# Genie-Kim/PintheMemory

Measured on AMD Instinct MI355X. Metric: train imgs/sec 768x768 bs=8 R50-DeepLabV3+ +mem, higher is better.
Workload: dtype f32

## Files before the change

### include/pinmem_hip.h

```cpp
#ifndef PINMEM_HIP_H
#define PINMEM_HIP_H
#include <stddef.h>
#include <stdint.h>

#ifdef __cplusplus
extern "C" {
#endif

typedef enum pm_status { PM_OK = 0, PM_EINVAL = -1, PM_EWORKSPACE = -2, PM_ELAUNCH = -3, PM_EUNSUPPORTED = -4 } pm_status;

typedef enum pm_dtype { PM_F32 = 0, PM_BF16 = 1 } pm_dtype;
#define PM_TF_ZERO_PAD64 1

typedef struct pm_tensor {
  void* ptr;
  int32_t n, h, w, c;
  int64_t pitch;
  int32_t dtype;
  int32_t flags;
} pm_tensor;

#define PM_ABI_VERSION 400

typedef struct pm_conv_params {
  int32_t struct_size;
  int32_t kh, kw, stride, pad, dil;
  int32_t prec;
  void* wino_v;
  int64_t wino_v_bytes;
  void* wxf;
  int64_t wxf_bytes;
  int32_t wxf_valid;
} pm_conv_params;

typedef struct pm_conv_epilogue {
  int64_t struct_size;
  const float* bias;
  const float* scale;
  const float* shift;
  const float* residual;
  int64_t residual_pitch;
  int32_t relu;
  float* bn_partials;
  int64_t bn_partials_bytes;
} pm_conv_epilogue;

const char* pm_last_error(void);
int pm_version(void);

size_t pm_conv_workspace(const pm_tensor* x, const pm_tensor* y, const pm_conv_params* p, int which );
size_t pm_conv_winograd_v_bytes(const pm_tensor* x, const pm_tensor* y, const pm_conv_params* p);
size_t pm_conv_wxf_bytes(const pm_tensor* x, const pm_tensor* y, const pm_conv_params* p);
size_t pm_conv_wxf_bytes_dgrad(const pm_tensor* dy, const pm_tensor* dx, const pm_conv_params* p);
typedef struct pm_wxf_job {
  const float* w;
  void* wxf;
  int64_t wxf_bytes;
  int32_t cout, kh, kw, cin;
  int32_t dgrad;
  int32_t reserved;
} pm_wxf_job;
int pm_conv_wxf_refresh_bf16(const pm_wxf_job* jobs, int n, void* stream);
int pm_conv_wxf_refresh_f32(const pm_wxf_job* jobs, int n, void* stream);
size_t pm_conv_bn_partials_bytes(const pm_tensor* x, const pm_tensor* y, const pm_conv_params* p);
int pm_conv_fwd(const pm_tensor* x, const float* w_krsc, const pm_tensor* y, const pm_conv_params* p,
                const pm_conv_epilogue* ep, void* ws, size_t ws_bytes, void* stream);
int pm_conv_bwd_data(const pm_tensor* dy, const float* w_krsc, const pm_tensor* dx, const pm_conv_params* p,
                     const pm_tensor* add, void* ws, size_t ws_bytes, void* stream);
int pm_conv_bwd_data_masked(const pm_tensor* dy, const float* w_krsc, const pm_tensor* dx, const pm_conv_params* p,
                            const pm_tensor* add, const uint8_t* add_mask, void* ws, size_t ws_bytes, void* stream);
int pm_conv_bwd_weight(const pm_tensor* x, const pm_tensor* dy, float* dw_krsc, float* dbias, const pm_conv_params* p,
                       void* ws, size_t ws_bytes, void* stream);

typedef struct pm_routing {
  int32_t struct_size;
  int32_t winograd;
  int32_t winograd_fused;
  int32_t conv16;
  int32_t conv16_wide;
  int32_t conv16_persistent;
  int32_t wgrad16;
  int32_t bf16_wgrad;
  int32_t split;
} pm_routing;
int pm_routing_get(pm_routing* out);
int pm_routing_set(const pm_routing* r);


int pm_set_winograd(int mode);
int pm_set_winograd_fused(int on);
int pm_set_conv16(int on);
int pm_set_bf16_wgrad(int on);
int pm_set_wgrad16(int on);
int pm_set_split(int on);

int pm_profile_enable(int on);
int pm_profile_dump(const char* csv_path);
int pm_profile_read(int mode, int bm, int bn, int km, int nst, double* total_ms, double* total_flops, int64_t* launches, int clear);
int pm_profile_read_prec(int mode, int bm, int bn, int km, int nst, int prec, double* total_ms, double* total_flops, int64_t* launches, int clear);
int pm_profile_read_bytes(int mode, int bm, int bn, int km, int nst, int prec, double* total_bytes);

size_t pm_bn_workspace(const pm_tensor* x);
int pm_bn_stats(const pm_tensor* x, float* moments, void* ws, size_t ws_bytes, void* stream);
int pm_bn_stats_finalize(const pm_tensor* x, float eps, float* mean, float* invstd, float* running_mean , float* running_var ,
                         float momentum, void* ws, size_t ws_bytes, void* stream);
int pm_bn_merge(const float* parts, int world, int c, float* moments, void* stream);
int pm_bn_merge_finalize(const float* parts, int world, int c, float eps, float* mean, float* invstd, float* running_mean ,
                         float* running_var , float momentum, void* stream);
int pm_bn_finalize(const float* moments, int c, float eps, float* mean, float* invstd,
                   float* running_mean, float* running_var, float momentum, void* stream);
int pm_bn_apply(const pm_tensor* x, const float* mean, const float* invstd, const float* gamma, const float* beta,
                const pm_tensor* residual , int relu, const pm_tensor* y, void* stream);
int pm_bn_apply_mask(const pm_tensor* x, const float* mean, const float* invstd, const float* gamma, const float* beta,
                     const pm_tensor* residual , int relu, const pm_tensor* y, uint8_t* mask , void* stream);
int pm_bn_bwd_reduce_mask(const pm_tensor* dy, const uint8_t* mask, const pm_tensor* x, const float* mean, const float* invstd,
                          const pm_tensor* gmask , float* sums, void* ws, size_t ws_bytes, void* stream);
int pm_bn_apply_mask_affine(const pm_tensor* x, const float* mean, const float* invstd, const float* gamma, const float* beta,
                            const pm_tensor* r, const float* r_mean, const float* r_invstd, const float* r_gamma, const float* r_beta,
                            int relu, const pm_tensor* y, uint8_t* mask , void* stream);
int pm_bn_bwd_apply_mask(const pm_tensor* dy, const uint8_t* mask, const pm_tensor* x, const float* mean, const float* invstd, const float* gamma,
                         const float* sums, float count, const pm_tensor* dx, void* stream);
int pm_bn_bwd_reduce(const pm_tensor* dy, const pm_tensor* y , const pm_tensor* x, const float* mean, const float* invstd,
                     const float* gamma , const float* beta , int relu, const pm_tensor* gmask ,
                     float* sums, void* ws, size_t ws_bytes, void* stream);
int pm_bn_bwd_apply(const pm_tensor* dy, const pm_tensor* y , const pm_tensor* x, const float* mean, const float* invstd,
                    const float* gamma, const float* beta , const float* sums, float count, int relu, const pm_tensor* dx,
                    const pm_tensor* dres , void* stream);
int pm_bn_partials_finalize(const float* partials, int64_t pixels, int c, float eps, float* mean, float* invstd, float* running_mean ,
                            float* running_var , float momentum, float* moments , void* stream);
int pm_bn_fold(const float* gamma, const float* beta, const float* running_mean, const float* running_var, const float* conv_bias,
               int c, float eps, float* scale, float* shift, void* stream);
int pm_bn_fold_multi(const void* table, const int* cs, const int* offs, int n, int max_c, int total, float eps, float* arena, void* stream);
int pm_relu_bwd(const pm_tensor* dy, const pm_tensor* y, const pm_tensor* dx, void* stream);
int pm_add(const pm_tensor* a, const pm_tensor* b, const pm_tensor* y, void* stream);
int pm_add_n(const pm_tensor* const* xs, int n, const pm_tensor* y, void* stream);
int pm_copy(const pm_tensor* src, const pm_tensor* dst, void* stream);
int pm_scale_shift_act(const pm_tensor* x, const float* scale, const float* shift, const pm_tensor* residual, int relu,
                       const pm_tensor* y, void* stream);

int pm_cast(const pm_tensor* x, const pm_tensor* y, void* stream);

int pm_maxpool3x3s2_fwd(const pm_tensor* x, const pm_tensor* y, uint8_t* argmax, void* stream);
int pm_maxpool3x3s2_bwd(const pm_tensor* dy, const uint8_t* argmax, const pm_tensor* dx, void* stream);
int pm_maxpool3x3s2_bn_relu_fwd(const pm_tensor* x, const float* mean, const float* invstd, const float* gamma, const float* beta, const pm_tensor* y,
                                uint8_t* argmax, void* stream);
int pm_bn_bwd_reduce_pool(const pm_tensor* dy_pooled, const uint8_t* argmax, const pm_tensor* x, const float* mean, const float* invstd, const float* gamma,
                          const float* beta, float* sums, void* ws, size_t ws_bytes, void* stream);
int pm_bn_bwd_apply_pool(const pm_tensor* dy_pooled, const uint8_t* argmax, const pm_tensor* x, const float* mean, const float* invstd, const float* gamma,
                         const float* beta, const float* sums, float count, const pm_tensor* dx, void* stream);
int pm_global_avgpool_fwd(const pm_tensor* x, const pm_tensor* y , void* stream);
int pm_global_avgpool_bwd(const pm_tensor* dy, const pm_tensor* dx, int accumulate, void* stream);

int pm_resize_bilinear_fwd(const pm_tensor* x, const pm_tensor* y, void* stream);
int pm_resize_bilinear_bwd(const pm_tensor* dy, const pm_tensor* dx, int accumulate, void* stream);
size_t pm_resize_bilinear_bwd_workspace(const pm_tensor* dy, const pm_tensor* dx);
int pm_resize_bilinear_bwd_separable(const pm_tensor* dy, const pm_tensor* dx, int accumulate, void* ws, size_t ws_bytes, void* stream);

int pm_resize_bilinear_hp_fwd(const pm_tensor* x, const pm_tensor* y, int flip_w, void* stream);
int pm_softmax_mean_update(const pm_tensor* logits, double* buffer, int counter, void* stream);
int pm_sliding_stitch(const pm_tensor* logits, const int32_t* tiles_xyxy, int ntiles, int H, int W, int flip_w, double* acc, int accumulate, void* stream);
int pm_argmax_f64(const double* buffer, int n, int h, int w, int c, int64_t* out_cls, double* out_prob , void* stream);

int pm_image_u8_to_nhwc4(const uint8_t* img_nhw3, int64_t pixels, const float* mean3, const float* std3, float* out_nhwc4, void* stream);
int pm_labels_u8_to_i64(const uint8_t* lab, int64_t n, int64_t* out, void* stream);

int pm_nchw_to_nhwc(const float* x_nchw, int c_src, const pm_tensor* y, void* stream);
int pm_nhwc_to_nchw(const pm_tensor* x, float* y_nchw, void* stream);
int pm_label_nearest(const int64_t* lab, int n, int H, int W, int64_t* out, int h, int w, void* stream);

size_t pm_upsample_ce_workspace(int n, int H, int W);
int pm_upsample_ce_fwd(const pm_tensor* logits, float inv_temp, const int64_t* labels, int H, int W, float* loss_out,
                       void* ws, size_t ws_bytes, void* stream);
size_t pm_upsample_ce_bwd_workspace(const pm_tensor* logits, int H, int W);
int pm_upsample_ce_bwd(const pm_tensor* logits, float inv_temp, const int64_t* labels, int H, int W, const float* loss_out,
                       const float* gscale, const pm_tensor* dlogits, void* ws, size_t ws_bytes, void* stream);

size_t pm_upsample_ce_field_bytes(const pm_tensor* logits, int H, int W);
int pm_upsample_ce_fwd_field(const pm_tensor* logits, float inv_temp, const int64_t* labels, int H, int W, float* loss_out, float* field,
                             void* ws , size_t ws_bytes, void* stream);
int pm_upsample_ce_bwd_field(const pm_tensor* logits , float inv_temp, int H, int W, const float* loss_out, const float* gscale,
                             const float* field, const pm_tensor* dlogits, void* stream);

size_t pm_upsample_wce_loss_floats(int n);
size_t pm_upsample_wce_workspace(int n, int H, int W);
int pm_upsample_wce_fwd(const pm_tensor* logits, float inv_temp, const int64_t* labels, int H, int W, const float* weights, int64_t weight_stride,
                        int per_image, float* loss_out, void* ws , size_t ws_bytes, void* stream);
int pm_upsample_wce_fwd_field(const pm_tensor* logits, float inv_temp, const int64_t* labels, int H, int W, const float* weights, int64_t weight_stride,
                              int per_image, float* loss_out, float* field, void* ws , size_t ws_bytes, void* stream);
int pm_upsample_wce_bwd_field(const pm_tensor* logits , float inv_temp, int H, int W, int per_image, const float* loss_out,
                              const float* gscale, const float* field, const pm_tensor* dlogits, void* stream);

size_t pm_label_class_weights_workspace(int n);
int pm_label_class_weights(const int64_t* labels, int n, int H, int W, int classes, double upper_bound, int norm, int per_batch, float* weights,
                           void* ws, size_t ws_bytes, void* stream);

size_t pm_upsample_eval_workspace(const pm_tensor* logits, int H, int W);
int pm_upsample_eval(const pm_tensor* logits, float inv_temp, const int64_t* labels, int H, int W, float* loss_out, int64_t* hist, int accumulate,
                     uint8_t* pred , void* ws, size_t ws_bytes, void* stream);

int pm_mem_read_fwd(const pm_tensor* x, const float* mem, int m, const float* gumbel_noise ,
                    const pm_tensor* qr, float* score, float* p_mem, void* stream);
size_t pm_mem_colsoftmax_workspace(int64_t rows, int m);
int pm_mem_colsoftmax(const float* score, const float* noise , int64_t rows, int m, float* p_query,
                      void* ws, size_t ws_bytes, void* stream);
size_t pm_mem_read_fwd_pq_workspace(int64_t rows, int m);
int pm_mem_read_fwd_pq(const pm_tensor* x, const float* mem, int m, const float* gumbel_noise, const float* gumbel_noise_q,
                       const pm_tensor* qr, float* score, float* p_mem, float* p_query, void* ws, size_t ws_bytes, void* stream);
size_t pm_mem_read_bwd_workspace(int64_t rows, int m, int d);
int pm_mem_read_bwd(const pm_tensor* x, const float* mem, int m, const float* p_mem, const pm_tensor* dqr,
                    const float* dscore_extra, const pm_tensor* dx, float* dmem ,
                    void* ws, size_t ws_bytes, void* stream);

size_t pm_mem_write_accum_workspace(const pm_tensor* z, int m);
int pm_mem_write_accum(const pm_tensor* z, const int64_t* labels, int H, int W, int m, int normalize,
                       float* nomden, void* ws, size_t ws_bytes, void* stream);
int pm_mem_write_accum_bwd(const pm_tensor* z, const int64_t* labels, int H, int W, int m, int normalize,
// ... 22 lines not shown
```

### pinthememory_amd/csrc/conv_igemm.hip

```cpp
#include <stdlib.h>
#include <algorithm>
#include <type_traits>
#include <vector>

#include "pm_common.h"

#include "conv_igemm_kernel.h"

namespace {

template <int ZL, bool O16 = false>
__global__ __launch_bounds__(256) void splitk_reduce_vec_kernel(const float* __restrict__ ws, int ksplit, long slab, int M, int Nn,
                                                                float* __restrict__ C, long c_pitch, const float* bias,
                                                                const float* scale, const float* shift, const float* residual,
                                                                long res_pitch, int relu, const unsigned char* res_mask) {
  constexpr int GP = 256 / ZL;
  __shared__ float4 red[ZL > 1 ? ZL : 1][GP];
  const int gl = threadIdx.x % GP, zl = threadIdx.x / GP;
  const long groups = (long)M * Nn / 4;
  for (long g0 = (long)blockIdx.x * GP; g0 < groups; g0 += (long)gridDim.x * GP) {
    const long grp = g0 + gl;
    float4 v = make_float4(0.f, 0.f, 0.f, 0.f);
    if (grp < groups)
#pragma unroll 8
// ... 160 lines not shown
  for (int i = 1; i < 16; ++i) s += sm[i][cl];
  out[c] = s;
}

template <bool O16>
__global__ __launch_bounds__(256) void dgrad_s2_interleave_kernel(const float* __restrict__ tmp, long class_stride, int valid_mask,
                                                                  float* __restrict__ dx, long xp, int N, int H, int W, int C, const float* __restrict__ add,
                                                                  long add_pitch) {
  const int c4n = C / 4;
  const long total = (long)N * H * W * c4n;
  for (long i = (long)blockIdx.x * 256 + threadIdx.x; i < total; i += (long)gridDim.x * 256) {
    const long pix = i / c4n;
    const int c = (int)(i - pix * c4n) * 4;
    const int ix = (int)(pix % W), iy = (int)((pix / W) % H), n = (int)(pix / ((long)W * H));
    const int cy = iy & 1, cx = ix & 1, cls = cy * 2 + cx;
    const int Hc = (H - cy + 1) >> 1, Wc = (W - cx + 1) >> 1;
    float4 v = make_float4(0.f, 0.f, 0.f, 0.f);
    if ((valid_mask >> cls) & 1) v = PM_LD4(tmp + cls * class_stride + ((long)(n * Hc + (iy >> 1)) * Wc + (ix >> 1)) * C + c);
    if constexpr (O16) {
      if (add) {
        const uint2 q = *reinterpret_cast<const uint2*>(reinterpret_cast<const pm_bf16*>(add) + pix * add_pitch + c);
        v.x += __uint_as_float(q.x << 16), v.y += __uint_as_float(q.x & 0xffff0000u), v.z += __uint_as_float(q.y << 16), v.w += __uint_as_float(q.y & 0xffff0000u);
      }
      *reinterpret_cast<uint2*>(reinterpret_cast<pm_bf16*>(dx) + pix * xp + c) = make_uint2(pm_pack_bf16(v.x, v.y), pm_pack_bf16(v.z, v.w));
    } else {
      if (add) {
        const float4 q = PM_LD4(add + pix * add_pitch + c);
        v.x += q.x, v.y += q.y, v.z += q.z, v.w += q.w;
      }
      PM_ST4(dx + pix * xp + c, v);
    }
  }
}

struct S2Class {
  int cy, cx, Hc, Wc, ky0, nky, ksy, kx0, nkx, ksx;
  long M;
};
inline void s2_taps(int c, int pad, int dil, int k, int& k0, int& nk, int& ks) {
  if (dil & 1) {
    k0 = (c + pad) & 1, ks = 2, nk = k0 < k ? (k - k0 + 1) / 2 : 0;
  } else {
    k0 = 0, ks = 1, nk = ((c + pad) & 1) ? 0 : k;
  }
}
inline S2Class s2_class(int cls, const pm_tensor* dx, const pm_conv_params* p) {
  S2Class c;
  c.cy = cls >> 1, c.cx = cls & 1;
  c.Hc = (dx->h - c.cy + 1) >> 1, c.Wc = (dx->w - c.cx + 1) >> 1;
  s2_taps(c.cy, p->pad, p->dil, p->kh, c.ky0, c.nky, c.ksy);
  s2_taps(c.cx, p->pad, p->dil, p->kw, c.kx0, c.nkx, c.ksx);
  c.M = (long)dx->n * c.Hc * c.Wc;
  return c;
}
int s2_interleave(const float* tmp, long class_stride, const bool* valid, const pm_tensor* dx, const pm_tensor* add, hipStream_t st, const char* what) {
  const int valid_mask = valid[0] | (valid[1] << 1) | (valid[2] << 2) | (valid[3] << 3);
  const long total = pm_pixels(dx) * (dx->c / 4);
  auto kernel = pm_is_bf16(dx) ? dgrad_s2_interleave_kernel<true> : dgrad_s2_interleave_kernel<false>;
  hipLaunchKernelGGL(kernel, dim3((int)std::min<long>((total + 255) / 256, 8192)), dim3(256), 0, st, tmp, class_stride, valid_mask, (float*)dx->ptr, (long)dx->pitch,
                     dx->n, dx->h, dx->w, dx->c, add ? (const float*)add->ptr : nullptr, add ? (long)add->pitch : 0l);
  return pm_check_launch(what);
}

struct Plan {
  int bm, bn;
  int tiles_m, tiles_n, ksplit, kper;
  size_t ws_bytes;
};

constexpr long SPLIT_MIN_K = 129;
inline bool split_k_ok(int mode, long K) { return mode == MODE_WGRAD || K >= SPLIT_MIN_K; }
Plan make_plan(int mode, long M, long Nn, long K, bool bf16 = false) {
  Plan best_p{};
  double best = 1e30;
  int bn = Nn > 64 ? 128 : ((Nn > 32 || bf16) ? 64 : 32);
  const bool big = bf16 || (pm_route.split && split_k_ok(mode, K));
  if (mode != MODE_WGRAD && !big && bn == 128) bn = 64;
  const long ksteps = (K + BK - 1) / BK;
  for (int bm = 128; bm >= 64; bm -= 64) {
    if (bm == 64 && bn < 64) continue;
    if (!big && mode != MODE_WGRAD && bn >= 64 && bm == 128) continue;
    if (bm == 64 && mode == MODE_WGRAD && M > 64) continue;
    if (bm == 128 && mode == MODE_WGRAD && M <= 64 && bn >= 64) continue;
    const int tiles_m = pm_cdiv(M, bm), tiles_n = pm_cdiv(Nn, bn);
    const long tiles = (long)tiles_m * tiles_n;
    const double unit_us = 2.0 * (bm / 128.0) * (bn / 128.0) * (bm == 64 ? 1.08 : 1.0);
    const long ks_max = std::max<long>(1, std::min<long>(ksteps / 4, 512));
    for (long ks = 1; ks <= ks_max; ++ks) {
      const long steps_per = (ksteps + ks - 1) / ks;
      if ((ksteps + steps_per - 1) / steps_per != ks) continue;
      const long blocks = tiles * ks;
      const long per_cu = (blocks + 255) / 256;
      double t = (double)per_cu * (double)(steps_per + 2) * unit_us * (per_cu == 1 ? 1.25 : 1.0);
      if (ks > 1) t += 2.0 * (double)ks * (double)M * (double)Nn * 4.0 / 3.0e6 + 6.0;
      if (t < best) {
        best = t;
        best_p.bm = bm, best_p.bn = bn, best_p.tiles_m = tiles_m, best_p.tiles_n = tiles_n;
        best_p.ksplit = (int)ks, best_p.kper = (int)(steps_per * BK);
      }
    }
  }
  best_p.ws_bytes = best_p.ksplit > 1 ? (size_t)best_p.ksplit * M * Nn * sizeof(float) : 0;
  return best_p;
}

template <int MODE, int BM, int BN, int WM, int WN, int KM, int PREC, int NST>
void launch_nst(const ConvK& k, dim3 grid, size_t smem, hipStream_t st) {
  const size_t ep_bytes = (size_t)4 * 32 * (BN / WN + 4) * sizeof(float);
  if constexpr (MODE == MODE_FWD && PREC != 1 && BN >= 64) {
    if (k.stats) {
      static pm_lds_optin optin;
      (void)optin(reinterpret_cast<const void*>(&conv_igemm_kernel<MODE, BM, BN, WM, WN, KM, PREC, NST, true>), 160 * 1024);
      hipLaunchKernelGGL((conv_igemm_kernel<MODE, BM, BN, WM, WN, KM, PREC, NST, true>), grid, dim3(256), std::max(smem / (NST == 1 ? 2 : 1), ep_bytes), st, k);
      return;
    }
  }
  static pm_lds_optin optin;
  (void)optin(reinterpret_cast<const void*>(&conv_igemm_kernel<MODE, BM, BN, WM, WN, KM, PREC, NST>), 160 * 1024);
  hipLaunchKernelGGL((conv_igemm_kernel<MODE, BM, BN, WM, WN, KM, PREC, NST>), grid, dim3(256), std::max(smem / (NST == 1 ? 2 : 1), ep_bytes), st, k);
}
constexpr int NST1_MAX_STEPS = 64;
constexpr bool has_nst1(int mode, int kmode, int bn) { return mode != MODE_WGRAD && kmode == K_FAST && bn >= 64; }
inline int lds_stages(int mode, int kmode, int bn, int kper) { return has_nst1(mode, kmode, bn) && kper <= NST1_MAX_STEPS * BK ? 1 : 2; }
template <int MODE, int BM, int BN, int WM, int WN, int KM, int PREC>
void launch_prec(const ConvK& k, dim3 grid, size_t smem, hipStream_t st) {
  if constexpr (has_nst1(MODE, KM, BN)) {
    if (lds_stages(MODE, KM, BN, k.kper) == 1) return launch_nst<MODE, BM, BN, WM, WN, KM, PREC, 1>(k, grid, smem, st);
  }
  launch_nst<MODE, BM, BN, WM, WN, KM, PREC, 2>(k, grid, smem, st);
}
template <int MODE, int BM, int BN, int WM, int WN, int KM>
void launch_inst(const ConvK& k, dim3 grid, size_t smem, hipStream_t st) {
  if constexpr (MODE == MODE_FWD && KM == K_FAST && BN >= 64) {
    if (k.prec == 2) return launch_prec<MODE, BM, BN, WM, WN, KM, 2>(k, grid, smem, st);
  }
  if constexpr (MODE == MODE_WGRAD && BN >= 64) {
    if (k.prec == 3) return launch_prec<MODE, BM, BN, WM, WN, KM, 3>(k, grid, smem, st);
    if (k.prec == 4) return launch_prec<MODE, BM, BN, WM, WN, KM, 4>(k, grid, smem, st);
  }
  if (k.prec != 0) launch_prec<MODE, BM, BN, WM, WN, KM, 1>(k, grid, smem, st);
  else launch_prec<MODE, BM, BN, WM, WN, KM, 0>(k, grid, smem, st);
}
template <int MODE, int BM, int BN, int WM, int WN>
void launch_one(const ConvK& k, dim3 grid, size_t smem, hipStream_t st) {
  if (k.kmode == K_SMALL) launch_inst<MODE, BM, BN, WM, WN, K_SMALL>(k, grid, smem, st);
  else if (k.kmode == K_FAST && MODE != MODE_WGRAD) launch_inst<MODE, BM, BN, WM, WN, (MODE != MODE_WGRAD ? K_FAST : K_MID)>(k, grid, smem, st);
  else launch_inst<MODE, BM, BN, WM, WN, K_MID>(k, grid, smem, st);
}

struct ProfRec {
  hipEvent_t a, b;
  int mode, bm, bn, km, prec, nst;
  int M, Nn, K, batch, ksplit;
  double flops;
  double bytes;
};
bool g_prof_on = false;
std::vector<ProfRec> g_prof;
struct ProfScope {
  ProfRec rec{};
  hipStream_t st;
  ProfScope(hipStream_t st_, int mode, int bm, int bn, int km, int prec, int nst, long M, long Nn, long K, int batch, int ksplit, double flops, double bytes = 0.0) : st(st_) {
    if (!g_prof_on) return;
    (void)hipEventCreate(&rec.a), (void)hipEventCreate(&rec.b);
    rec.mode = mode, rec.bm = bm, rec.bn = bn, rec.km = km, rec.prec = prec, rec.nst = nst, rec.M = (int)M, rec.Nn = (int)Nn, rec.K = (int)K, rec.batch = batch, rec.ksplit = ksplit;
    rec.flops = flops, rec.bytes = bytes;
    (void)hipEventRecord(rec.a, st);
  }
  void done() {
    if (!g_prof_on) return;
    (void)hipEventRecord(rec.b, st);
    g_prof.push_back(rec);
  }
};

inline bool split_takes(int mode, const Plan& p, const ConvK& k, int batch) {
  return pm_route.split != 0 && p.bn >= 64 && !k.io16 && (batch > 1 || split_k_ok(mode, k.K));
}

template <int MODE>
int launch(const ConvK& k0, const Plan& p, hipStream_t st, int batch = 1, double flops = -1.0) {
  ConvK k = k0;
  k.tiles_m = p.tiles_m;
  k.tiles_n = p.tiles_n;
  k.ksplit = p.ksplit;
  k.kper = p.kper;
  dim3 grid(p.tiles_m * p.tiles_n, batch, p.ksplit);
  if (batch != 1) k.stage_ep = 0;
  if (k.prec == 0 && split_takes(MODE, p, k, batch)) k.prec = 5;
  {
    const int units = batch * p.ksplit, rem = units & 7, ntile = p.tiles_m * p.tiles_n;
    k.batch_xcd = units >= 8 && (rem == 0 || ((rem == 1 || rem == 2 || rem == 4) && ntile % (8 / rem) == 0));
  }
  const int km = (MODE == MODE_WGRAD && k.kmode == K_FAST) ? K_MID : ((k.prec == 5 && MODE != MODE_WGRAD && k.kmode == K_FAST && k.kh * k.kw == 1 && k.stride == 1 && k.pad == 0 && !k.sub) ? K_PW : k.kmode);
  ProfScope prof(st, MODE, p.bm, p.bn, km, k.prec, lds_stages(MODE, k.kmode, p.bn, k.kper), k.M, k.Nn, k.K, batch, p.ksplit,
                 flops >= 0.0 ? flops : 2.0 * (double)k.M * (double)k.Nn * (double)k.K * batch,
                 (double)batch * ((double)k.a_bytes + (double)k.b_bytes + ((k.io16 && p.ksplit == 1) ? 2.0 : 4.0) * (double)k.M * (double)k.Nn * (double)p.ksplit));
  if constexpr (MODE != MODE_WGRAD) {
    if (pm_route.split && (k.prec == 0 || k.prec == 5) && !k.io16 && batch == 1 && p.ksplit == 1 && !k.stats && k.kh * k.kw == 1 && k.stride == 1 && k.pad == 0 && !k.sub) {
      pm_gemm_pw g;
      g.A = k.A, g.B = k.B, g.C = k.C, g.bias = k.bias, g.scale = k.scale, g.shift = k.shift, g.residual = k.residual, g.res_mask = k.res_mask;
      g.a_pitch = MODE == MODE_FWD ? k.x_pitch : k.y_pitch, g.c_pitch = k.c_pitch, g.res_pitch = k.res_pitch;
      g.b_sn = MODE == MODE_FWD ? k.K : 1, g.b_sk = MODE == MODE_FWD ? 1 : k.Nn;
      g.M = k.M, g.Nn = k.Nn, g.K = k.K, g.relu = k.relu;
      if (pm_pwstream_ok(&g)) {
        prof.rec.bm = 32, prof.rec.bn = 64, prof.rec.km = 4, prof.rec.prec = 5, prof.rec.nst = 0;
        const int e = pm_pwstream_launch(&g, st);
        prof.done();
        return e;
      }
    }
  }
  constexpr bool akc = MODE != MODE_WGRAD, bkc = MODE == MODE_FWD;
  if (k.prec == 5) {
    if (int e = pm_conv_split_launch(MODE, p.bm, p.bn, k, grid.x, grid.y, grid.z, pm_conv_split_stage_bytes(MODE, p.bm, p.bn), st)) return e;
    prof.rec.nst = 1;
    prof.done();
    return pm_check_launch("conv_split");
  }
  const bool tr = MODE == MODE_WGRAD && (k.prec == 3 || k.prec == 4) && p.bn >= 64;
  auto smem = [&](int bm, int bn) {
    if (tr) return (size_t)2 * ((k.prec == 4 ? 2 : 1) * BK * (bm + 32) + (k.prec == 4 ? 2 : 1) * BK * (bn + 32)) * 2;
    return (size_t)2 * ((akc ? bm * LDK : BK * bm) + (bkc ? bn * LDK : BK * bn)) * sizeof(float);
  };
  if (p.bm == 64) {
    if (p.bn == 128) launch_one<MODE, 64, 128, 2, 2>(k, grid, smem(64, 128), st);
    else launch_one<MODE, 64, 64, 2, 2>(k, grid, smem(64, 64), st);
  } else if (p.bn == 128) {
    launch_one<MODE, 128, 128, 2, 2>(k, grid, smem(128, 128), st);
  } else if (p.bn == 64) {
    launch_one<MODE, 128, 64, 2, 2>(k, grid, smem(128, 64), st);
  } else {
    launch_one<MODE, 128, 32, 4, 1>(k, grid, smem(128, 32), st);
  }
  prof.done();
  return pm_check_launch("conv_igemm");
}

int check_common(const pm_tensor* x, const pm_tensor* y, const pm_conv_params* p) {
  PM_REQUIRE(x && y && p && x->ptr && y->ptr, PM_EINVAL, "conv: null tensor");
  PM_REQUIRE(p->struct_size == (int32_t)sizeof(pm_conv_params), PM_EINVAL, "conv: pm_conv_params.struct_size %d != %zu -- caller built against another pinmem_hip.h (library ABI %d)",
             p->struct_size, sizeof(pm_conv_params), PM_ABI_VERSION);
  PM_REQUIRE(p->kh >= 1 && p->kw >= 1 && p->dil >= 1 && p->pad >= 0, PM_EINVAL, "conv: bad geometry");
  PM_REQUIRE(p->stride == 1 || p->stride == 2, PM_EUNSUPPORTED, "conv: stride %d unsupported (1 or 2)", p->stride);
  const int ho = (x->h + 2 * p->pad - p->dil * (p->kh - 1) - 1) / p->stride + 1;
  const int wo = (x->w + 2 * p->pad - p->dil * (p->kw - 1) - 1) / p->stride + 1;
  PM_REQUIRE(ho == y->h && wo == y->w && x->n == y->n, PM_EINVAL, "conv: output %dx%d does not match geometry (%dx%d)", y->h, y->w, ho, wo);
  PM_REQUIRE((x->dtype == PM_F32 || x->dtype == PM_BF16) && (y->dtype == PM_F32 || y->dtype == PM_BF16), PM_EUNSUPPORTED, "conv: dtype %d / %d", x->dtype, y->dtype);
  for (const pm_tensor* t : {x, y}) {
    if (pm_is_bf16(t)) PM_REQUIRE(pm_vec8(t), PM_EINVAL, "conv: bf16 tensors must be 16B aligned with pitch %% 8 == 0 and channels %% 8 == 0");
    else PM_REQUIRE(pm_vec_ok(t), PM_EINVAL, "conv: tensors must be 16B aligned with pitch %% 4 == 0");
  }
  PM_REQUIRE(x->c % 4 == 0, PM_EUNSUPPORTED, "conv: Cin %% 4 != 0 unsupported (pad the input channels)");
  PM_REQUIRE((y->c % 4 == 0) || (p->kh * p->kw == 1), PM_EUNSUPPORTED, "conv: Cout %% 4 != 0 only for 1x1");
  PM_REQUIRE(x->pitch >= x->c && y->pitch >= y->c, PM_EINVAL, "conv: pitch < channels");
  PM_REQUIRE(pm_pixels(x) * x->pitch < (1ll << 29) && pm_pixels(y) * y->pitch < (1ll << 29) && (int64_t)y->c * x->c * p->kh * p->kw < (1ll << 29),
             PM_EUNSUPPORTED, "conv: tensor too large for 32-bit byte offsets (2 GiB per tensor)");
  return PM_OK;
}

void fill_geom(ConvK& k, const pm_tensor* x, const pm_tensor* y, const pm_conv_params* p) {
  k.N = x->n, k.H = x->h, k.W = x->w, k.Cin = x->c, k.x_pitch = x->pitch;
  k.Ho = y->h, k.Wo = y->w, k.Cout = y->c, k.y_pitch = y->pitch;
  k.kh = p->kh, k.kw = p->kw, k.stride = p->stride, k.pad = p->pad, k.dil = p->dil;
  k.sshift = p->stride == 2 ? 1 : 0;
  k.prec = p->prec != 0 ? 1 : 0;
  k.T_eff = p->kh * p->kw, k.tk_w = p->kw, k.ky0 = k.kx0 = 0, k.ksy = k.ksx = 1;
  k.sub = k.sub_cy = k.sub_cx = 0, k.Hc = x->h, k.Wc = x->w;
  k.bias = k.scale = k.shift = k.residual = nullptr;
  k.res_pitch = 0, k.res_mask = nullptr, k.relu = 0, k.stats = nullptr, k.io16 = 0;
  k.stage_ep = 1;
  k.spl_prio = 1;
  k.n_group = 8;
  k.batch_xcd = 0;
  k.a_bs = k.b_bs = k.c_bs = 0;
}

struct WinoPlan {
  bool use;
  pm_wino_geom g;
  int Kp, P;
  size_t v_bytes, m_bytes, u_bytes;
  Plan pl;
};
inline bool wino_wgrad_pays(int cin, int cout) { return (long)cin * cout >= 256 * 256; }
WinoPlan wino_plan(const pm_tensor* xin, int cout, const pm_conv_params* p, bool wgrad = false) {
  WinoPlan wp{};
  if (wgrad && !wino_wgrad_pays(xin->c, cout)) return wp;
  if (pm_route.winograd == 0 || p->kh != 3 || p->kw != 3 || p->stride != 1 || p->pad != p->dil || p->prec != 0) return wp;
  const int cin = xin->c;
  if (cin < 128 || cout < 128 || (cout & 3) || (cin & 3)) return wp;
  int m = 0;
  double best_ratio = 0.6;
  for (int cand = pm_route.winograd; cand >= 2; cand -= 2) {
    const pm_wino_geom g = pm_wino_make_geom(xin->n, xin->h, xin->w, p->dil, cand);
    const double cover = (double)(cand * g.TY * p->dil) * (double)(cand * g.TX * p->dil) / ((double)xin->h * xin->w);
    const double ratio = cover * (cand + 2) * (cand + 2) / (9.0 * cand * cand);
    if (ratio <= best_ratio) best_ratio = ratio, m = cand, wp.g = g;
  }
  if (!m) return wp;
  wp.P = (m + 2) * (m + 2);
  wp.Kp = (cin + BK - 1) / BK * BK;
  if (wp.g.tiles * (long)std::max(wp.Kp, cout) * 4 >= (1ll << 31)) return wp;
  wp.v_bytes = pm_align_up((size_t)wp.P * wp.g.tiles * wp.Kp * sizeof(float), 256);
  wp.m_bytes = pm_align_up((size_t)wp.P * wp.g.tiles * cout * sizeof(float), 256);
  wp.u_bytes = pm_align_up((size_t)wp.P * cout * wp.Kp * sizeof(float), 256);
  wp.pl.bm = 128, wp.pl.bn = 128;
  if (pm_cdiv(cout, 128) * 128 > cout * 1.12 && pm_cdiv(cout, 64) * 64 < pm_cdiv(cout, 128) * 128) wp.pl.bn = 64;
  if (wp.g.tiles <= 4608 && !pm_route.split) wp.pl.bm = 64;
  wp.pl.tiles_m = pm_cdiv(wp.g.tiles, wp.pl.bm), wp.pl.tiles_n = pm_cdiv(cout, wp.pl.bn);
  wp.pl.ksplit = 1, wp.pl.kper = wp.Kp, wp.pl.ws_bytes = 0;
  wp.use = true;
  return wp;
}
inline size_t wino_ws(const WinoPlan& wp) { return wp.v_bytes + wp.m_bytes + wp.u_bytes; }

int wino_conv(const pm_tensor* xin, const float* w, int w_cout, int w_cin, bool dgrad, const pm_tensor* yout, const WinoPlan& wp,
              const pm_conv_epilogue& ep, void* ws, hipStream_t st, float* v_keep = nullptr, float* u_ext = nullptr, bool u_valid = false) {
  float* V = v_keep ? v_keep : (float*)ws;
  float* Mo = (float*)((char*)ws + wp.v_bytes);
  float* U = u_ext ? u_ext : (float*)((char*)ws + wp.v_bytes + wp.m_bytes);
  const int cout = yout->c;
  if (int e = pm_wino_input_xf((const float*)xin->ptr, xin->pitch, xin->c, wp.Kp, wp.g, V, st)) return e;
  if (!(u_ext && u_valid))
    if (int e = pm_wino_filter_xf(w, w_cout, w_cin, wp.Kp, dgrad, wp.g.m, U, st)) return e;
  const pm_tensor xv = {V, 1, 1, (int32_t)wp.g.tiles, wp.Kp, wp.Kp};
  const pm_tensor yv = {Mo, 1, 1, (int32_t)wp.g.tiles, cout, cout};
  const pm_conv_params p1 = {(int32_t)sizeof(pm_conv_params), 1, 1, 1, 0, 1, 0};
  ConvK k;
  fill_geom(k, &xv, &yv, &p1);
  k.A = V, k.B = U, k.C = Mo;
  k.M = (int)wp.g.tiles, k.Nn = cout, k.K = wp.Kp;
  k.a_bytes = (unsigned)(wp.g.tiles * wp.Kp * 4), k.b_bytes = (unsigned)((long)cout * wp.Kp * 4), k.kmode = K_FAST;
  k.c_pitch = cout, k.c_split = 0;
  k.a_bs = wp.g.tiles * wp.Kp, k.b_bs = (long)cout * wp.Kp, k.c_bs = wp.g.tiles * cout;
  if (pm_route.winograd_fused && wp.g.m == 4 && wp.Kp % 16 == 0) {
    ProfScope prof(st, 3, 32, 32, 0, 0, 1, wp.g.tiles, cout, wp.Kp, wp.P, 1, 2.0 * wp.P * (double)wp.g.tiles * cout * xin->c);
    const int e = pm_wino_fused_f4(V, U, cout, wp.Kp, wp.g, (float*)yout->ptr, yout->pitch, ep.bias, ep.scale, ep.shift, ep.residual, ep.residual_pitch, ep.relu, st);
    prof.done();
    return e;
  }
  if (int e = launch<MODE_FWD>(k, wp.pl, st, wp.P, 2.0 * wp.P * (double)wp.g.tiles * cout * xin->c)) return e;
  return pm_wino_output_xf(Mo, cout, wp.g, (float*)yout->ptr, yout->pitch, ep.bias, ep.scale, ep.shift, ep.residual, ep.residual_pitch, ep.relu, st);
}

struct WinoWgradPlan {
  Plan pl;
  size_t slab_bytes;
};
WinoWgradPlan wino_wgrad_plan(const WinoPlan& wp, int cout) {
  WinoWgradPlan q{};
  q.pl.bm = 128, q.pl.bn = 128;
  if (pm_cdiv(wp.Kp, 128) * 128 > wp.Kp * 1.12 && pm_cdiv(wp.Kp, 64) * 64 < pm_cdiv(wp.Kp, 128) * 128) q.pl.bn = 64;
  q.pl.tiles_m = pm_cdiv(cout, 128), q.pl.tiles_n = pm_cdiv(wp.Kp, q.pl.bn);
  const long ksteps = (wp.g.tiles + BK - 1) / BK;
  const long per_split = (long)q.pl.tiles_m * q.pl.tiles_n * wp.P;
  long ks = std::max<long>(1, std::min<long>((768 + per_split / 2) / per_split, ksteps / 8));
  const long steps_per = (ksteps + ks - 1) / ks;
  ks = (ksteps + steps_per - 1) / steps_per;
  q.pl.ksplit = (int)ks, q.pl.kper = (int)(steps_per * BK), q.pl.ws_bytes = 0;
  q.slab_bytes = pm_align_up((size_t)ks * wp.P * cout * wp.Kp * sizeof(float), 256);
  return q;
}
inline size_t wino_wgrad_ws(const WinoPlan& wp, const WinoWgradPlan& q) { return wp.v_bytes + wp.m_bytes + q.slab_bytes; }

int wino_wgrad(const pm_tensor* x, const pm_tensor* dy, float* dw, const WinoPlan& wp, const WinoWgradPlan& q, void* ws, hipStream_t st,
               float* v_kept = nullptr) {
  float* V = v_kept ? v_kept : (float*)ws;
  float* Z = (float*)((char*)ws + wp.v_bytes);
  float* slab = (float*)((char*)ws + wp.v_bytes + wp.m_bytes);
  const int cout = dy->c;
  if (!v_kept)
    if (int e = pm_wino_input_xf((const float*)x->ptr, x->pitch, x->c, wp.Kp, wp.g, V, st)) return e;
  if (int e = pm_wino_dy_xf((const float*)dy->ptr, dy->pitch, cout, wp.g, Z, st)) return e;
  const pm_tensor xv = {V, 1, 1, (int32_t)wp.g.tiles, wp.Kp, wp.Kp};
  const pm_tensor zv = {Z, 1, 1, (int32_t)wp.g.tiles, cout, cout};
  const pm_conv_params p1 = {(int32_t)sizeof(pm_conv_params), 1, 1, 1, 0, 1, 0};
  ConvK k;
  fill_geom(k, &xv, &zv, &p1);
  k.A = Z, k.B = V, k.C = slab;
  k.M = cout, k.Nn = wp.Kp, k.K = (int)wp.g.tiles;
  k.a_bytes = (unsigned)(wp.g.tiles * cout * 4), k.b_bytes = (unsigned)(wp.g.tiles * wp.Kp * 4), k.kmode = K_MID;
  k.c_pitch = wp.Kp, k.c_split = (long)wp.P * cout * wp.Kp;
  k.a_bs = wp.g.tiles * cout, k.b_bs = wp.g.tiles * wp.Kp, k.c_bs = (long)cout * wp.Kp;
  if (int e = launch<MODE_WGRAD>(k, q.pl, st, wp.P, 2.0 * wp.P * (double)wp.g.tiles * cout * x->c)) return e;
  return pm_wino_dw_xf(slab, q.pl.ksplit, cout, x->c, wp.Kp, wp.g.m, dw, st);
}

struct Bf16Plan {
  bool use;
  bool c16;
  pm_conv16 k16;
  bool inplace;
  int Cp;
  long M, Nn, Kf;
  size_t xb_bytes, wb_bytes;
  Plan pl;
};
Bf16Plan bf16_plan(const pm_tensor* xin, const pm_tensor* yout, const pm_conv_params* p) {
  Bf16Plan b{};
  if ((p->prec != 2 && !pm_is_bf16(xin) && !pm_is_bf16(yout)) || xin->c < 32) return b;
  b.Cp = (xin->c + 63) / 64 * 64;
  const long T = (long)p->kh * p->kw;
  b.M = pm_pixels(yout), b.Nn = yout->c, b.Kf = T * b.Cp / 2;
  b.inplace = pm_is_bf16(xin) && (xin->c % 64 == 0 || ((xin->flags & PM_TF_ZERO_PAD64) && xin->pitch >= b.Cp));
  const size_t xb = b.inplace ? (size_t)pm_pixels(xin) * xin->pitch * 2 : (size_t)pm_pixels(xin) * b.Cp * 2, wb = (size_t)yout->c * T * b.Cp * 2;
  if (xb >= (1ull << 31) || wb >= (1ull << 31)) return b;
  b.xb_bytes = b.inplace ? 0 : pm_align_up(xb, 256), b.wb_bytes = pm_align_up(wb, 256);
  b.pl = make_plan(MODE_FWD, b.M, b.Nn, b.Kf, true);
  if (b.pl.bn < 64) return b;
  b.use = true;
  constexpr long C16_MIN_M = 256;
  b.c16 = false;
  if (pm_route.conv16 && b.M >= C16_MIN_M && p->stride >= 1) {
    pm_conv16& k = b.k16;
    k = pm_conv16{};
    k.N = xin->n, k.H = xin->h, k.W = xin->w, k.Ho = yout->h, k.Wo = yout->w;
    k.a_pitch = b.inplace ? xin->pitch : b.Cp, k.Cp = b.Cp;
    k.kh = p->kh, k.kw = p->kw, k.stride = p->stride, k.pad = p->pad, k.dil = p->dil;
    k.M = (int)b.M, k.Nn = (int)b.Nn, k.K = (int)(T * b.Cp), k.ksteps = k.K / 64;
    k.c_pitch = yout->pitch, k.c_f32 = pm_is_bf16(yout) ? 0 : 1;
    pm_conv16_plan(&k);
    b.c16 = pm_route.conv16 == 2 || k.wide || k.bm == 64 || k.ksteps_per == 1 || (b.pl.bm == 64 && k.ksteps >= 16);
  }
  return b;
}
inline size_t bf16_ws(const Bf16Plan& b) {
  return b.xb_bytes + b.wb_bytes + std::max(pm_align_up(b.pl.ws_bytes, 256), b.c16 ? pm_conv16_slab_bytes(&b.k16) : (size_t)0);
}

int conv_bf16(const pm_tensor* xin, const float* w, int w_cout, int w_cin, bool rotate, const pm_tensor* yout, const pm_conv_params* pe, const Bf16Plan& b,
              const pm_conv_epilogue& e0, void* ws, hipStream_t st, char* wb_ext = nullptr, bool wb_valid = false) {
  char* xb = b.inplace ? (char*)xin->ptr : (char*)ws;
  char* wb = wb_ext ? wb_ext : (char*)ws + b.xb_bytes;
  float* slab = (float*)((char*)ws + b.xb_bytes + b.wb_bytes);
  const int T = pe->kh * pe->kw;
  if (!b.inplace) {
    if (pm_is_bf16(xin)) {
      if (int e = pm16_pad_rows((const pm_bf16*)xin->ptr, xin->pitch, xin->c, b.Cp, pm_pixels(xin), (pm_bf16*)xb, st)) return e;
    } else if (int e = pm_bf16_cast_rows((const float*)xin->ptr, xin->pitch, xin->c, b.Cp, pm_pixels(xin), xb, st)) return e;
  }
  if (!(wb_ext && wb_valid))
    if (int e = pm_bf16_cast_weights(w, w_cout, T, w_cin, b.Cp, rotate, wb, st)) return e;
  const long xpitch16 = b.inplace ? xin->pitch : b.Cp;
  if (b.c16) {
    const bool o16 = pm_is_bf16(yout);
    const bool ok = (!e0.bn_partials || o16) &&
                    (o16 ? ((yout->c | yout->pitch | (e0.residual ? e0.residual_pitch : 0)) & 7) == 0 && pm_aligned16(yout->ptr) && pm_aligned16(e0.residual)
                         : !(e0.scale || e0.residual || e0.relu));
    if (ok) {
      pm_conv16 k = b.k16;
      k.A = (const pm_bf16*)xb, k.B = (const pm_bf16*)wb;
      const double fl = 2.0 * (double)b.M * (double)b.Nn * (double)T * (double)xin->c * (g_prof_on ? pm_conv16_executed_fraction(&k) : 1.0);
      ProfScope prof(st, k.wide ? 5 : 4, k.bm, k.bn, pm_conv16w_persistent(&k), 5, k.wide ? 3 : (k.ksteps_per == 1 ? 1 : 2), k.M, k.Nn, k.K / 2, 1, k.ksplit, fl);
      int e;
      if (k.ksplit > 1) {
        k.C = slab;
        e = pm_conv16_launch(&k, st);
      } else {
        k.C = yout->ptr;
        k.bias = e0.bias, k.scale = e0.scale, k.shift = e0.shift, k.residual = e0.residual, k.res_pitch = e0.residual_pitch, k.relu = e0.relu;
        k.stats = o16 ? e0.bn_partials : nullptr;
        e = pm_conv16_launch(&k, st);
      }
      prof.done();
      if (e) return e;
      if (k.ksplit > 1)
        return splitk_reduce(slab, k.ksplit, b.M, b.Nn, (float*)yout->ptr, (long)yout->pitch, e0.bias, e0.scale, e0.shift, e0.residual, (long)e0.residual_pitch, e0.relu,
                             st, o16);
      return PM_OK;
    }
  }
  const pm_tensor xv = {xb, xin->n, xin->h, xin->w, b.Cp / 2, xpitch16 / 2};
  ConvK k;
  fill_geom(k, &xv, yout, pe);
  k.prec = 2;
  k.A = (const float*)xb, k.B = (const float*)wb;
  k.M = (int)b.M, k.Nn = (int)b.Nn, k.K = (int)b.Kf;
  k.a_bytes = (unsigned)((size_t)pm_pixels(xin) * xpitch16 * 2), k.b_bytes = (unsigned)((size_t)yout->c * T * b.Cp * 2), k.kmode = K_FAST;
  const double flops = 2.0 * (double)b.M * (double)b.Nn * (double)T * (double)xin->c;
  k.io16 = pm_is_bf16(yout) ? 1 : 0;
  if (b.pl.ksplit > 1) {
    k.C = slab, k.c_pitch = b.Nn, k.c_split = b.M * b.Nn;
    if (int e = launch<MODE_FWD>(k, b.pl, st, 1, flops)) return e;
// ... 68 lines not shown
  PmS2Classes cl = s.cl;
  for (int cls = 0; cls < 4; ++cls) cl.out[cls] = (char*)ws + s.wb_off[cls];
  if (int e = pm_bf16_cast_weights_s2(w, dy->c, p->kh, p->kw, dx->c, dy->c, &cl, st)) return e;
  float* slab = (float*)((char*)ws + s.slab_off);
  for (int cls = 0; cls < 4; ++cls) {
    if (!s.valid[cls]) continue;
    pm_conv16 k = s.k[cls];
    k.A = (const pm_bf16*)dy->ptr, k.B = (const pm_bf16*)((char*)ws + s.wb_off[cls]);
    void* out = (char*)ws + s.out_off[cls];
    ProfScope prof(st, 4, k.bm, k.bn, 0, 5, k.ksteps_per == 1 ? 1 : 2, k.M, k.Nn, k.K / 2, 1, k.ksplit, 2.0 * (double)k.M * (double)k.Nn * (double)k.K);
    k.C = k.ksplit > 1 ? (void*)slab : out;
    const int e = pm_conv16_launch(&k, st);
    prof.done();
    if (e) return e;
    if (k.ksplit > 1)
      if (int e2 = splitk_reduce(slab, k.ksplit, k.M, k.Nn, (float*)out, (long)dx->c, nullptr, nullptr, nullptr, nullptr, 0l, 0, st, false)) return e2;
  }
  return s2_interleave((const float*)((char*)ws + s.out_off[0]), s.class_stride, s.valid, dx, add, st, "dgrad_s2_interleave(native bf16 classes)");
}

struct Bf16WgradPlan {
  bool use;
  long P, M, Nn, Kf;
  size_t dyt_bytes, xt_bytes;
  Plan pl;
};
Bf16WgradPlan bf16_wgrad_plan(const pm_tensor* x, const pm_tensor* dy, const pm_conv_params* p) {
  Bf16WgradPlan b{};
  if (p->prec != 2 || !pm_route.bf16_wgrad || x->c < 32 || dy->c < 32) return b;
  b.P = pm_pixels(dy);
  if (b.P % 64) return b;
  const long T = (long)p->kh * p->kw;
  b.M = dy->c, b.Nn = T * x->c, b.Kf = b.P / 2;
  const size_t dyt = (size_t)dy->c * b.P * 2, xt = (size_t)T * x->c * b.P * 2;
  if (dyt >= (1ull << 31) || xt >= (1ull << 31)) return b;
  b.dyt_bytes = pm_align_up(dyt, 256), b.xt_bytes = pm_align_up(xt, 256);
  b.pl = make_plan(MODE_FWD, b.M, b.Nn, b.Kf, true);
  if (b.pl.bn < 64) return b;
  b.use = true;
  return b;
}
inline size_t bf16_wgrad_ws(const Bf16WgradPlan& b) { return b.dyt_bytes + b.xt_bytes + pm_align_up(b.pl.ws_bytes, 256); }

int conv_wgrad_bf16(const pm_tensor* x, const pm_tensor* dy, float* dw, const pm_conv_params* p, const Bf16WgradPlan& b, void* ws, hipStream_t st) {
  char* dyt = (char*)ws;
  char* xt = dyt + b.dyt_bytes;
  float* slab = (float*)(xt + b.xt_bytes);
  if (int e = pm_bf16_transpose_taps((const float*)dy->ptr, dy->pitch, dy->c, dy->n, dy->h, dy->w, dy->h, dy->w, 1, 1, 1, 0, 1, dyt, st)) return e;
  if (int e = pm_bf16_transpose_taps((const float*)x->ptr, x->pitch, x->c, x->n, x->h, x->w, dy->h, dy->w, p->kh, p->kw, p->stride, p->pad, p->dil, xt, st)) return e;
  const int Pf = (int)(b.P / 2);
  const pm_tensor av = {dyt, 1, 1, (int32_t)b.M, Pf, Pf};
  const pm_tensor cv = {dw, 1, 1, (int32_t)b.M, (int32_t)b.Nn, b.Nn};
  const pm_conv_params p1 = {(int32_t)sizeof(pm_conv_params), 1, 1, 1, 0, 1, 2};
  ConvK k;
  fill_geom(k, &av, &cv, &p1);
  k.prec = 2;
  k.A = (const float*)dyt, k.B = (const float*)xt;
  k.M = (int)b.M, k.Nn = (int)b.Nn, k.K = (int)b.Kf;
  k.a_bytes = (unsigned)((size_t)b.M * b.P * 2), k.b_bytes = (unsigned)((size_t)b.Nn * b.P * 2), k.kmode = K_FAST;
  const double flops = 2.0 * (double)b.M * (double)b.Nn * (double)b.P;
  if (b.pl.ksplit > 1) {
    k.C = slab, k.c_pitch = b.Nn, k.c_split = b.M * b.Nn;
    if (int e = launch<MODE_FWD>(k, b.pl, st, 1, flops)) return e;
    return splitk_reduce(slab, b.pl.ksplit, b.M, b.Nn, dw, b.Nn, nullptr, nullptr, nullptr, nullptr, 0l, 0, st);
  }
  k.C = dw, k.c_pitch = b.Nn, k.c_split = 0;
  return launch<MODE_FWD>(k, b.pl, st, 1, flops);
}

void gemm_dims(int which, const pm_tensor* x, const pm_tensor* y, const pm_conv_params* p, long& M, long& Nn, long& K) {
  const long T = (long)p->kh * p->kw;
  if (which == MODE_FWD) M = pm_pixels(y), Nn = y->c, K = T * x->c;
  else if (which == MODE_DGRAD) M = pm_pixels(x), Nn = x->c, K = T * y->c;
  else M = y->c, Nn = T * x->c, K = pm_pixels(y);
}

struct S2ParityPlan {
  S2Class c[4];
  Plan pl[4];
  bool valid[4];
  size_t tmp_bytes, slab_bytes;
};
S2ParityPlan s2_parity_plan(const pm_tensor* dy, const pm_tensor* dx, const pm_conv_params* p) {
  S2ParityPlan s{};
  for (int cls = 0; cls < 4; ++cls) {
    const S2Class& c = s.c[cls] = s2_class(cls, dx, p);
    s.tmp_bytes = std::max(s.tmp_bytes, (size_t)c.M * dx->c * sizeof(float));
    s.valid[cls] = c.M > 0 && c.nky * c.nkx > 0;
    if (!s.valid[cls]) continue;
    s.pl[cls] = make_plan(MODE_DGRAD, c.M, dx->c, (long)c.nky * c.nkx * dy->c, p->prec != 0);
    s.slab_bytes = std::max(s.slab_bytes, s.pl[cls].ws_bytes);
  }
  s.tmp_bytes = pm_align_up(s.tmp_bytes, 256);
  return s;
}

struct W16Plan {
  bool use;
  pm_wgrad16 k;
};
W16Plan wgrad16_plan(const pm_tensor* x, const pm_tensor* dy, const pm_conv_params* p, long M, long Nn, long K, int max_ksplit) {
  W16Plan q{};
  pm_wgrad16& w16 = q.k;
  w16.X = (const pm_bf16*)x->ptr, w16.DY = (const pm_bf16*)dy->ptr;
  w16.N = x->n, w16.H = x->h, w16.W = x->w, w16.Ho = dy->h, w16.Wo = dy->w;
  w16.x_pitch = x->pitch, w16.dy_pitch = dy->pitch, w16.Cin = x->c, w16.Cout = dy->c;
  w16.kh = p->kh, w16.kw = p->kw, w16.stride = p->stride, w16.pad = p->pad, w16.dil = p->dil;
  w16.M = (int)M, w16.Nn = (int)Nn, w16.P = (int)K, w16.kper = 64, w16.c_split = M * Nn;
  q.use = K < (1l << 30) && pm_wgrad16_plan(&w16);
  if (!q.use) return q;
  const long tiles = (long)w16.tiles_m * w16.tiles_n, steps = (K + 63) / 64;
  int best_ks = 1;
  double best = 1e30;
  for (int ks = 1; ks <= max_ksplit; ++ks) {
    const long per = (steps + ks - 1) / ks, kse = (steps + per - 1) / per;
    const long rounds = (tiles * kse + 255) / 256;
    const double cost = (double)rounds * (per + 6) + (kse > 1 ? (double)kse * M * Nn * 8.0 / 4e12 / 1.0e-6 : 0.0);
    if (cost < best) best = cost, best_ks = (int)kse;
  }
  const long per = (steps + best_ks - 1) / best_ks;
  w16.kper = (int)per * 64, w16.ksplit = (int)((steps + per - 1) / per);
  return q;
}

enum RouteKind {
  R_DIRECT,
  R_WINO,
  R_BF16,
  R_S2_NATIVE,
  R_S2_PARITY,
  R_WINO_WGRAD,
  R_BF16_WGRAD,
  R_DIRECT_WGRAD,
};
struct ConvRoute {
  RouteKind kind;
  Plan pl;
  WinoPlan wino;
  WinoWgradPlan wino_w;
  Bf16Plan b16;
  pm_conv_params pe;
  S2Native s2n;
  S2ParityPlan s2p;
  Bf16WgradPlan b16w;
  W16Plan w16;
  bool native16;
  size_t ws_bytes;
  size_t class_off, slab_off;
  size_t bias_off;
  size_t x32_off, dy32_off;
  size_t v_keep_bytes;
  size_t wxf_bytes;
  size_t bn_bytes;
};

ConvRoute route_conv(int which, const pm_tensor* x, const pm_tensor* y, const pm_conv_params* p) {
  ConvRoute r{};
  long M, Nn, K;
  gemm_dims(which, x, y, p, M, Nn, K);
  if (which == MODE_FWD) {
    if ((r.wino = wino_plan(x, y->c, p)).use) {
      r.kind = R_WINO, r.ws_bytes = wino_ws(r.wino), r.wxf_bytes = r.wino.u_bytes;
      r.v_keep_bytes = wino_wgrad_pays(x->c, y->c) ? r.wino.v_bytes : 0;
    } else if (p->prec == 2 && (r.b16 = bf16_plan(x, y, p)).use) {
      r.kind = R_BF16, r.pe = *p, r.ws_bytes = bf16_ws(r.b16), r.wxf_bytes = r.b16.wb_bytes;
    } else {
      r.kind = R_DIRECT, r.pl = make_plan(MODE_FWD, M, Nn, K, p->prec != 0), r.ws_bytes = pm_align_up(r.pl.ws_bytes, 256);
    }
    bool bn;
    if (pm_is_bf16(y)) bn = pm_vec8(y) && r.kind == R_BF16 && (r.b16.c16 ? (r.b16.k16.ksplit == 1 && !r.b16.k16.wide) : r.b16.pl.ksplit == 1);
    else if (pm_is_bf16(x) || (y->c & 3) || (y->pitch & 3) || !pm_aligned16(y->ptr)) bn = false;
    else bn = r.kind == R_BF16 ? r.b16.pl.ksplit == 1 : (r.kind == R_DIRECT && p->prec == 0 && r.pl.ksplit == 1 && r.pl.bn >= 64);
    r.bn_bytes = bn ? pm_align_up((size_t)pm_cdiv(pm_pixels(y), 32) * y->c * 2 * sizeof(float), 256) : 0;
  } else if (which == MODE_DGRAD) {
    if (p->stride == 2) {
      if ((r.s2n = s2_native_plan(y, x, p)).ok) {
        r.kind = R_S2_NATIVE, r.ws_bytes = r.s2n.total;
      } else {
        r.kind = R_S2_PARITY, r.s2p = s2_parity_plan(y, x, p);
        r.class_off = 0, r.slab_off = 4 * r.s2p.tmp_bytes;
        r.dy32_off = pm_align_up(r.slab_off + r.s2p.slab_bytes + 256, 256);
        r.ws_bytes = r.dy32_off + upcast_bytes(y);
      }
    } else if (dgrad_bf16_ok(p) && (r.pe = dgrad_as_fwd(p), r.b16 = bf16_plan(y, x, &r.pe)).use) {
      r.kind = R_BF16, r.ws_bytes = bf16_ws(r.b16), r.wxf_bytes = r.b16.wb_bytes;
    } else if ((r.wino = wino_plan(y, x->c, p)).use) {
      r.kind = R_WINO, r.ws_bytes = wino_ws(r.wino);
    } else {
      r.kind = R_DIRECT, r.pl = make_plan(MODE_DGRAD, M, Nn, K, p->prec != 0), r.ws_bytes = pm_align_up(r.pl.ws_bytes, 256);
    }
  } else {
    const bool tier = pm_is_bf16(x) || pm_is_bf16(y);
    r.native16 = pm_is_bf16(x) && pm_is_bf16(y) && y->c >= 32;
    size_t own;
    if (!tier && (r.b16w = bf16_wgrad_plan(x, y, p)).use) {
      r.kind = R_BF16_WGRAD, own = bf16_wgrad_ws(r.b16w);
    } else if (!tier && (r.wino = wino_plan(x, y->c, p, true)).use) {
      r.kind = R_WINO_WGRAD, r.wino_w = wino_wgrad_plan(r.wino, y->c), own = wino_wgrad_ws(r.wino, r.wino_w);
    } else {
      r.kind = R_DIRECT_WGRAD, r.pl = make_plan(MODE_WGRAD, M, Nn, K, p->prec != 0), own = r.pl.ws_bytes;
      if (r.native16) {
        r.pl.kper = (r.pl.kper + 63) / 64 * 64;
        r.pl.ksplit = (int)((K + r.pl.kper - 1) / r.pl.kper);
        r.w16 = wgrad16_plan(x, y, p, M, Nn, K, r.pl.ksplit);
      }
    }
    r.bias_off = pm_align_up(own, 256);
    r.ws_bytes = r.bias_off + pm_align_up((size_t)pm_cdiv(pm_pixels(y), colsum_rows(pm_pixels(y), y->c)) * y->c * sizeof(float), 256) + upcast_bytes(x) + upcast_bytes(y);
    r.x32_off = r.dy32_off = r.ws_bytes;
    if (!r.native16) r.x32_off -= upcast_bytes(x);
    r.dy32_off = r.x32_off - upcast_bytes(y);
  }
  return r;
}

int dgrad_s2_parity(const pm_tensor* dy0, const float* w, const pm_tensor* dx, const pm_conv_params* p, const pm_tensor* add, const ConvRoute& r, void* ws, hipStream_t st) {
  pm_tensor dy32;
  if (int e = upcast(dy0, (char*)ws + r.dy32_off, &dy32, st)) return e;
  const pm_tensor* dy = &dy32;
  float* tmp = (float*)((char*)ws + r.class_off);
  float* slab = (float*)((char*)ws + r.slab_off);
  for (int cls = 0; cls < 4; ++cls) {
    if (!r.s2p.valid[cls]) continue;
    const S2Class& c = r.s2p.c[cls];
    const Plan& pl = r.s2p.pl[cls];
    ConvK k;
    fill_geom(k, dx, dy, p);
    k.A = (const float*)dy->ptr, k.B = w;
    k.M = (int)c.M, k.Nn = dx->c, k.K = c.nky * c.nkx * dy->c;
    k.a_bytes = (unsigned)(pm_pixels(dy) * dy->pitch * 4), k.b_bytes = (unsigned)((long)dy->c * p->kh * p->kw * dx->c * 4);
    k.kmode = dy->c >= BK ? K_MID : K_SMALL;
    k.T_eff = c.nky * c.nkx, k.tk_w = c.nkx, k.ky0 = c.ky0, k.kx0 = c.kx0, k.ksy = c.ksy, k.ksx = c.ksx;
    k.sub = 1, k.sub_cy = c.cy, k.sub_cx = c.cx, k.Hc = c.Hc, k.Wc = c.Wc;
    float* out = (float*)((char*)tmp + cls * r.s2p.tmp_bytes);
    if (pl.ksplit > 1) {
      k.C = slab, k.c_pitch = dx->c, k.c_split = c.M * dx->c;
      if (int e = launch<MODE_DGRAD>(k, pl, st)) return e;
      if (int e = splitk_reduce(slab, pl.ksplit, c.M, dx->c, out, (long)dx->c, nullptr, nullptr, nullptr, nullptr, 0l, 0, st)) return e;
    } else {
      k.C = out, k.c_pitch = dx->c, k.c_split = 0;
      if (int e = launch<MODE_DGRAD>(k, pl, st)) return e;
    }
  }
  return s2_interleave(tmp, (long)(r.s2p.tmp_bytes / sizeof(float)), r.s2p.valid, dx, add, st, "dgrad_s2_interleave");
}

template <int MODE>
int conv_direct(const pm_tensor* x, const pm_tensor* y, const float* w, const pm_conv_params* p, const Plan& pl, const pm_conv_epilogue& e, void* ws, hipStream_t st,
                const unsigned char* res_mask = nullptr) {
  const pm_tensor *xin = MODE == MODE_FWD ? x : y, *out = MODE == MODE_FWD ? y : x;
  long M, Nn, K;
  gemm_dims(MODE, x, y, p, M, Nn, K);
  ConvK k;
  fill_geom(k, x, y, p);
  k.io16 = pm_is_bf16(out) ? 1 : 0;
  k.A = (const float*)xin->ptr, k.B = w;
  k.M = (int)M, k.Nn = (int)Nn, k.K = (int)K;
  k.a_bytes = (unsigned)(pm_pixels(xin) * xin->pitch * 4), k.b_bytes = (unsigned)((long)y->c * p->kh * p->kw * x->c * 4);
  k.kmode = (xin->c % BK == 0 && (MODE == MODE_FWD || p->stride == 1)) ? 0 : (xin->c >= BK ? 1 : 2);
  if (pl.ksplit > 1) {
    k.C = (float*)ws, k.c_pitch = Nn, k.c_split = M * Nn;
    if (int err = launch<MODE>(k, pl, st)) return err;
    return splitk_reduce((const float*)ws, pl.ksplit, M, Nn, (float*)out->ptr, (long)out->pitch, e.bias, e.scale, e.shift, e.residual, (long)e.residual_pitch, e.relu, st, k.io16 != 0,
                         res_mask);
  }
  k.C = (float*)out->ptr, k.c_pitch = out->pitch, k.c_split = 0;
  k.bias = e.bias, k.scale = e.scale, k.shift = e.shift, k.residual = e.residual, k.res_pitch = e.residual_pitch, k.res_mask = res_mask, k.relu = e.relu;
  k.stats = e.bn_partials;
  return launch<MODE>(k, pl, st);
}

int conv_wgrad_direct(const pm_tensor* x, const pm_tensor* dy, float* dw, const pm_conv_params* p, const ConvRoute& r, void* ws, hipStream_t st) {
  long M, Nn, K;
  gemm_dims(MODE_WGRAD, x, dy, p, M, Nn, K);
  if (r.w16.use) {
    pm_wgrad16 w16 = r.w16.k;
    w16.C = w16.ksplit > 1 ? (float*)ws : dw;
    ProfScope prof(st, MODE_WGRAD, w16.bm, w16.bn, 2, 4, 3, M, Nn, K, 1, w16.ksplit, 2.0 * (double)M * (double)Nn * (double)K);
    const int e = pm_wgrad16_launch(&w16, st);
    prof.done();
    if (e || w16.ksplit == 1) return e;
    return splitk_reduce((const float*)ws, w16.ksplit, M, Nn, dw, (long)Nn, nullptr, nullptr, nullptr, nullptr, 0l, 0, st);
  }
  ConvK k;
  fill_geom(k, x, dy, p);
  if (p->prec == 2) k.prec = 3;
  if (r.native16) {
    PM_REQUIRE(x->c % 8 == 0 && dy->c % 8 == 0 && r.pl.bn >= 64, PM_EUNSUPPORTED, "conv_bwd_weight(bf16): channels %% 8 != 0 or a tile narrower than 64");
    k.prec = 4;
  }
  const int esz = r.native16 ? 2 : 4;
  k.A = (const float*)dy->ptr, k.B = (const float*)x->ptr;
  k.M = (int)M, k.Nn = (int)Nn, k.K = (int)K;
  k.a_bytes = (unsigned)(pm_pixels(dy) * dy->pitch * esz), k.b_bytes = (unsigned)(pm_pixels(x) * x->pitch * esz), k.kmode = dy->w >= (r.native16 ? 2 * BK : BK) ? 1 : 2;
  k.C = r.pl.ksplit > 1 ? (float*)ws : dw, k.c_pitch = Nn, k.c_split = r.pl.ksplit > 1 ? M * Nn : 0;
  if (int e = launch<MODE_WGRAD>(k, r.pl, st)) return e;
  if (r.pl.ksplit == 1) return PM_OK;
  return splitk_reduce((const float*)ws, r.pl.ksplit, M, Nn, dw, (long)Nn, nullptr, nullptr, nullptr, nullptr, 0l, 0, st);
}

}

static pm_routing routing_from_env() {
  auto env = [](const char* name, int dflt) { const char* e = getenv(name); return e ? atoi(e) : dflt; };
  return pm_routing{
      (int32_t)sizeof(pm_routing),
      4,
      env("PM_WINO_FUSED", 0),
      env("PM_CONV16", 1),
      env("PM_C16W", 1),
      env("PM_C16P", 1),
      env("PM_WGRAD16", 1),
      0,
      env("PM_SPLIT", 1),
  };
}
const pm_routing pm_route_defaults = routing_from_env();
pm_routing pm_route = pm_route_defaults;
extern "C" int pm_routing_get(pm_routing* out) {
  PM_REQUIRE(out && out->struct_size == (int32_t)sizeof(pm_routing), PM_EINVAL, "pm_routing_get: struct_size %d != %zu (library ABI %d)", out ? out->struct_size : -1,
             sizeof(pm_routing), PM_ABI_VERSION);
  *out = pm_route;
  return PM_OK;
}
extern "C" int pm_routing_set(const pm_routing* r) {
  PM_REQUIRE(r && r->struct_size == (int32_t)sizeof(pm_routing), PM_EINVAL, "pm_routing_set: struct_size %d != %zu (library ABI %d)", r ? r->struct_size : -1, sizeof(pm_routing),
             PM_ABI_VERSION);
  PM_REQUIRE(r->winograd == 0 || r->winograd == 2 || r->winograd == 4, PM_EINVAL, "pm_routing_set: winograd %d (0, 2 or 4)", r->winograd);
  PM_REQUIRE(r->conv16 >= 0 && r->conv16 <= 2 && r->conv16_wide >= 0 && r->conv16_wide <= 3, PM_EINVAL, "pm_routing_set: conv16 %d / conv16_wide %d", r->conv16, r->conv16_wide);
  pm_route = *r;
  return PM_OK;
}
extern "C" int pm_set_winograd(int mode) {
  PM_REQUIRE(mode == 0 || mode == 2 || mode == 4, PM_EINVAL, "pm_set_winograd: mode %d (0 off, 2 F(2x2,3x3), 4 prefer F(4x4,3x3))", mode);
  pm_route.winograd = mode;
  return PM_OK;
}
extern "C" int pm_set_conv16(int on) {
  PM_REQUIRE(on >= 0 && on <= 8, PM_EINVAL, "pm_set_conv16: %d (0 register-staged, 1 per shape, 2 LDS-DMA everywhere / narrow tiles only, 3 LDS-DMA everywhere / wide tiles "
             "wherever the shape allows, 4 per shape without the wide kernel, 5 / 6 = 1 (the streaming 1x1 kernel left the library in round 6), 7 as 3 with the 256 x 256 tile, "
             "8 as 3 with one block per tile instead of the persistent ring)", on);
  pm_route.conv16 = (on == 3 || on == 7 || on == 8) ? 2 : ((on == 4 || on == 5 || on == 6) ? 1 : on);
  pm_route.conv16_wide = (on == 3 || on == 8) ? 2 : (on == 7 ? 3 : ((on == 2 || on == 4) ? 0 : pm_route_defaults.conv16_wide));
  pm_route.conv16_persistent = on == 8 ? 0 : (on == 3 ? 1 : pm_route_defaults.conv16_persistent);
  return PM_OK;
}
extern "C" int pm_set_winograd_fused(int on) {
  pm_route.winograd_fused = on != 0;
  return PM_OK;
}
extern "C" int pm_set_wgrad16(int on) {
  pm_route.wgrad16 = on != 0;
  return PM_OK;
}
extern "C" int pm_set_split(int on) {
  pm_route.split = on ? 1 : 0;
  return PM_OK;
}
extern "C" int pm_set_bf16_wgrad(int on) {
  pm_route.bf16_wgrad = on != 0;
  return PM_OK;
}
extern "C" int pm_profile_enable(int on) {
  g_prof_on = on != 0;
  return PM_OK;
}
extern "C" int pm_profile_read_prec(int mode, int bm, int bn, int km, int nst, int prec, double* total_ms, double* total_flops, int64_t* launches, int clear);
extern "C" int pm_profile_read(int mode, int bm, int bn, int km, int nst, double* total_ms, double* total_flops, int64_t* launches, int clear) {
  return pm_profile_read_prec(mode, bm, bn, km, nst, -1, total_ms, total_flops, launches, clear);
}
extern "C" int pm_profile_read_prec(int mode, int bm, int bn, int km, int nst, int prec, double* total_ms, double* total_flops, int64_t* launches, int clear) {
  double ms = 0.0, fl = 0.0;
  int64_t n = 0;
  for (const ProfRec& r : g_prof) {
    if ((mode >= 0 && r.mode != mode) || (bm >= 0 && r.bm != bm) || (bn >= 0 && r.bn != bn) || (km >= 0 && r.km != km) || (nst >= 0 && r.nst != nst) ||
        (prec >= 0 && r.prec != prec))
      continue;
    float t = 0.f;
    if (hipEventSynchronize(r.b) != hipSuccess || hipEventElapsedTime(&t, r.a, r.b) != hipSuccess) continue;
    ms += t, fl += r.flops, ++n;
  }
  if (clear) {
    for (const ProfRec& r : g_prof) (void)hipEventDestroy(r.a), (void)hipEventDestroy(r.b);
    g_prof.clear();
  }
  if (total_ms) *total_ms = ms;
  if (total_flops) *total_flops = fl;
  if (launches) *launches = n;
  return PM_OK;
}

extern "C" int pm_profile_read_bytes(int mode, int bm, int bn, int km, int nst, int prec, double* total_bytes) {
  double b = 0.0;
  for (const ProfRec& r : g_prof) {
    if ((mode >= 0 && r.mode != mode) || (bm >= 0 && r.bm != bm) || (bn >= 0 && r.bn != bn) || (km >= 0 && r.km != km) || (nst >= 0 && r.nst != nst) ||
        (prec >= 0 && r.prec != prec))
      continue;
    b += r.bytes;
  }
  if (total_bytes) *total_bytes = b;
  return PM_OK;
}

extern "C" int pm_profile_dump(const char* path) {
  PM_REQUIRE(path, PM_EINVAL, "pm_profile_dump: null path");
  FILE* f = fopen(path, "w");
  PM_REQUIRE(f, PM_EINVAL, "pm_profile_dump: cannot open %s", path);
  fprintf(f, "mode,bm,bn,km,nst,prec,M,N,K,batch,ksplit,ms,gflop\n");
  for (const ProfRec& r : g_prof) {
    float t = 0.f;
    if (hipEventSynchronize(r.b) != hipSuccess || hipEventElapsedTime(&t, r.a, r.b) != hipSuccess) continue;
    fprintf(f, "%d,%d,%d,%d,%d,%d,%d,%d,%d,%d,%d,%.5f,%.4f\n", r.mode, r.bm, r.bn, r.km, r.nst, r.prec, r.M, r.Nn, r.K, r.batch, r.ksplit, t, r.flops * 1e-9);
  }
  fclose(f);
  return PM_OK;
}

extern "C" size_t pm_conv_workspace(const pm_tensor* x, const pm_tensor* y, const pm_conv_params* p0, int which) {
  const pm_conv_params tp = tier_params(p0, x, y);
  return route_conv(which, x, y, &tp).ws_bytes;
}
extern "C" size_t pm_conv_winograd_v_bytes(const pm_tensor* x, const pm_tensor* y, const pm_conv_params* p0) {
  if (!x || !y || !p0) return 0;
  const pm_conv_params tp = tier_params(p0, x, y);
  return route_conv(MODE_FWD, x, y, &tp).v_keep_bytes;
}
extern "C" size_t pm_conv_wxf_bytes(const pm_tensor* x, const pm_tensor* y, const pm_conv_params* p0) {
  if (!x || !y || !p0) return 0;
  const pm_conv_params tp = tier_params(p0, x, y);
  return route_conv(MODE_FWD, x, y, &tp).wxf_bytes;
}
extern "C" size_t pm_conv_wxf_bytes_dgrad(const pm_tensor* dy, const pm_tensor* dx, const pm_conv_params* p0) {
  if (!dy || !dx || !p0) return 0;
  const pm_conv_params tp = tier_params(p0, dy, dx);
  return route_conv(MODE_DGRAD, dx, dy, &tp).wxf_bytes;
}
extern "C" size_t pm_conv_bn_partials_bytes(const pm_tensor* x, const pm_tensor* y, const pm_conv_params* p0) {
  if (!x || !y || !p0 || check_common(x, y, p0) != PM_OK) return 0;
  const pm_conv_params tp = tier_params(p0, x, y);
  return route_conv(MODE_FWD, x, y, &tp).bn_bytes;
}

extern "C" int pm_conv_wxf_refresh_f32(const pm_wxf_job* jobs, int n, void* stream) {
  PM_REQUIRE(n >= 0 && (jobs || n == 0), PM_EINVAL, "conv_wxf_refresh_f32: bad job table");
  std::vector<const float*> w(n);
  std::vector<float*> U(n);
  std::vector<int> cout(n), cin(n), kp(n), m(n);
  for (int i = 0; i < n; ++i) {
    const pm_wxf_job& q = jobs[i];
    PM_REQUIRE(q.w && q.wxf && q.cout > 0 && q.cin > 0 && q.kh == 3 && q.kw == 3 && q.dgrad == 0, PM_EINVAL,
               "conv_wxf_refresh_f32: job %d: forward transforms of 3x3 filters only", i);
    PM_REQUIRE(pm_aligned16(q.wxf), PM_EINVAL, "conv_wxf_refresh_f32: job %d: buffer must be 16-byte aligned", i);
    const int Kp = (q.cin + BK - 1) / BK * BK;
    const size_t u4 = pm_align_up((size_t)36 * q.cout * Kp * sizeof(float), 256), u2 = pm_align_up((size_t)16 * q.cout * Kp * sizeof(float), 256);
    PM_REQUIRE((size_t)q.wxf_bytes == u4 || (size_t)q.wxf_bytes == u2, PM_EINVAL, "conv_wxf_refresh_f32: job %d: %ld bytes is neither the F(4x4) nor the F(2x2) transform of %d x %d",
               i, (long)q.wxf_bytes, q.cout, q.cin);
    w[i] = q.w, U[i] = (float*)q.wxf, cout[i] = q.cout, cin[i] = q.cin, kp[i] = Kp, m[i] = (size_t)q.wxf_bytes == u4 ? 4 : 2;
  }
  return pm_wino_filter_xf_multi(w.data(), U.data(), cout.data(), cin.data(), kp.data(), m.data(), n, (hipStream_t)stream);
}

extern "C" int pm_conv_fwd(const pm_tensor* x, const float* w, const pm_tensor* y, const pm_conv_params* p0,
                           const pm_conv_epilogue* ep, void* ws, size_t ws_bytes, void* stream) {
  if (int e = check_common(x, y, p0)) return e;
  const pm_conv_params tp = tier_params(p0, x, y);
  const pm_conv_params* p = &tp;
  PM_REQUIRE(!ep || ep->struct_size == (int64_t)sizeof(pm_conv_epilogue), PM_EINVAL,
             "conv_fwd: pm_conv_epilogue.struct_size %ld != %zu -- caller built against another pinmem_hip.h (library ABI %d)", ep ? (long)ep->struct_size : 0l,
             sizeof(pm_conv_epilogue), PM_ABI_VERSION);
  PM_REQUIRE(w && pm_aligned16(w), PM_EINVAL, "conv_fwd: weight null or unaligned");
  pm_conv_epilogue e0 = {(int64_t)sizeof(pm_conv_epilogue), nullptr, nullptr, nullptr, nullptr, 0, 0};
  if (ep) e0 = *ep;
  PM_REQUIRE((e0.scale == nullptr) == (e0.shift == nullptr), PM_EINVAL, "conv_fwd: scale and shift go together");
  const ConvRoute r = route_conv(MODE_FWD, x, y, p);
  if (e0.bn_partials) {
    PM_REQUIRE(!e0.relu && !e0.residual, PM_EINVAL, "conv_fwd: bn_partials are the statistics of the convolution output (no residual / ReLU)");
    PM_REQUIRE(r.bn_bytes != 0 && (size_t)e0.bn_partials_bytes >= r.bn_bytes, PM_EINVAL, "conv_fwd: this call cannot emit bn_partials (ask pm_conv_bn_partials_bytes): %zu needed", r.bn_bytes);
  }
  PM_REQUIRE(ws_bytes >= r.ws_bytes && (ws || r.ws_bytes == 0), PM_EWORKSPACE, "conv_fwd: workspace %zu < %zu", ws_bytes, r.ws_bytes);
  hipStream_t st = (hipStream_t)stream;
  switch (r.kind) {
    case R_WINO: {
      float* keep = (p->wino_v && (size_t)p->wino_v_bytes >= r.wino.v_bytes) ? (float*)p->wino_v : nullptr;
      float* uext = (p->wxf && (size_t)p->wxf_bytes >= r.wino.u_bytes) ? (float*)p->wxf : nullptr;
      return wino_conv(x, w, y->c, x->c, false, y, r.wino, e0, ws, st, keep, uext, p->wxf_valid != 0);
    }
    case R_BF16: {
      char* wext = (p->wxf && (size_t)p->wxf_bytes >= r.b16.wb_bytes) ? (char*)p->wxf : nullptr;
      return conv_bf16(x, w, y->c, x->c, false, y, &r.pe, r.b16, e0, ws, st, wext, p->wxf_valid != 0);
    }
    default:
      PM_REQUIRE(pm_is_f32(x), PM_EUNSUPPORTED, "conv_fwd: a bf16 input needs at least 32 channels (got %d)", x->c);
      return conv_direct<MODE_FWD>(x, y, w, p, r.pl, e0, ws, st);
  }
}

extern "C" int pm_conv_bwd_data(const pm_tensor* dy, const float* w, const pm_tensor* dx, const pm_conv_params* p0, const pm_tensor* add,
                                void* ws, size_t ws_bytes, void* stream) {
  return pm_conv_bwd_data_masked(dy, w, dx, p0, add, nullptr, ws, ws_bytes, stream);
}

extern "C" int pm_conv_bwd_data_masked(const pm_tensor* dy, const float* w, const pm_tensor* dx, const pm_conv_params* p0, const pm_tensor* add,
                                       const uint8_t* add_mask, void* ws, size_t ws_bytes, void* stream) {
  if (int e = check_common(dx, dy, p0)) return e;
  const pm_conv_params tp = tier_params(p0, dy, dx);
  const pm_conv_params* p = &tp;
  PM_REQUIRE(!add || (add->ptr && pm_same_shape(add, dx) && add->dtype == dx->dtype), PM_EINVAL, "conv_bwd_data: `add` must match dx (shape and dtype)");
  PM_REQUIRE(!add || !pm_is_bf16(add) || pm_vec8(add), PM_EINVAL, "conv_bwd_data: bf16 `add` must be 16B aligned with pitch %% 8 == 0");
  PM_REQUIRE(w && pm_aligned16(w), PM_EINVAL, "conv_bwd_data: weight null or unaligned");
  const ConvRoute r = route_conv(MODE_DGRAD, dx, dy, p);
  PM_REQUIRE(ws_bytes >= r.ws_bytes && (ws || r.ws_bytes == 0), PM_EWORKSPACE, "conv_bwd_data: workspace %zu < %zu", ws_bytes, r.ws_bytes);
  if (add_mask) {
    PM_REQUIRE(add && pm_is_f32(add) && pm_is_f32(dy) && pm_vec4(add) && pm_vec4(dx), PM_EINVAL, "conv_bwd_data: a masked `add` is an fp32 tensor with 16-byte rows and c %% 4 == 0");
    PM_REQUIRE(r.kind == R_DIRECT, PM_EUNSUPPORTED,
               "conv_bwd_data: a masked `add` is served by the fp32 implicit-GEMM route only (this call routes to %s)",
               r.kind == R_WINO ? "Winograd" : (r.kind == R_BF16 ? "the bf16 kernels" : "the stride-2 class kernels"));
  }
  hipStream_t st = (hipStream_t)stream;
  const pm_conv_epilogue e1 = {(int64_t)sizeof(pm_conv_epilogue), nullptr, nullptr, nullptr, add ? (const float*)add->ptr : nullptr, add ? add->pitch : 0, 0};
  switch (r.kind) {
    case R_S2_NATIVE: return dgrad_s2_bf16(dy, w, dx, p, add, r.s2n, ws, st);
    case R_S2_PARITY: return dgrad_s2_parity(dy, w, dx, p, add, r, ws, st);
    case R_BF16: {
      char* wext = (p->wxf && (size_t)p->wxf_bytes >= r.b16.wb_bytes) ? (char*)p->wxf : nullptr;
      return conv_bf16(dy, w, dy->c, dx->c, true, dx, &r.pe, r.b16, e1, ws, st, wext, p->wxf_valid != 0);
    }
    case R_WINO: return wino_conv(dy, w, dy->c, dx->c, true, dx, r.wino, e1, ws, st);
    default:
      PM_REQUIRE(pm_is_f32(dy), PM_EUNSUPPORTED, "conv_bwd_data: a bf16 dy needs at least 32 channels and a stride-1 geometry the forward form covers");
      return conv_direct<MODE_DGRAD>(dx, dy, w, p, r.pl, e1, ws, st, add_mask);
  }
}

extern "C" int pm_conv_bwd_weight(const pm_tensor* x0, const pm_tensor* dy0, float* dw, float* dbias, const pm_conv_params* p0, void* ws,
                                  size_t ws_bytes, void* stream) {
  if (int e = check_common(x0, dy0, p0)) return e;
  const pm_conv_params tp = tier_params(p0, x0, dy0);
  const pm_conv_params* p = &tp;
  PM_REQUIRE(dw && pm_aligned16(dw), PM_EINVAL, "conv_bwd_weight: dw null or unaligned");
  const ConvRoute r = route_conv(MODE_WGRAD, x0, dy0, p);
  PM_REQUIRE(ws && ws_bytes >= r.ws_bytes, PM_EWORKSPACE, "conv_bwd_weight: workspace %zu < %zu", ws_bytes, r.ws_bytes);
  hipStream_t st = (hipStream_t)stream;
  const pm_tensor *x = x0, *dy = dy0;
  pm_tensor x32, dy32;
  if (!r.native16 && pm_is_bf16(x0)) {
    if (int e = upcast(x0, (char*)ws + r.x32_off, &x32, st)) return e;
    x = &x32;
  }
  if (pm_is_bf16(dy0) && (!r.native16 || dbias)) {
    if (int e = upcast(dy0, (char*)ws + r.dy32_off, &dy32, st)) return e;
    if (!r.native16) dy = &dy32;
  }
  int e;
  switch (r.kind) {
    case R_BF16_WGRAD: e = conv_wgrad_bf16(x, dy, dw, p, r.b16w, ws, st); break;
    case R_WINO_WGRAD: e = wino_wgrad(x, dy, dw, r.wino, r.wino_w, ws, st, (p->wino_v && (size_t)p->wino_v_bytes >= r.wino.v_bytes) ? (float*)p->wino_v : nullptr); break;
    default: e = conv_wgrad_direct(x, dy, dw, p, r, ws, st);
  }
  if (e || !dbias) return e;
  const pm_tensor* dyb = pm_is_bf16(dy0) ? &dy32 : dy0;
  const long P = pm_pixels(dyb);
  const int rpb = colsum_rows(P, dyb->c), nb = pm_cdiv(P, rpb);
  float* part = (float*)((char*)ws + r.bias_off);
  if (dyb->pitch == ((dyb->c + 3) & ~3) && dyb->pitch <= 64 && pm_aligned16(dyb->ptr))
    hipLaunchKernelGGL(colsum_partial_narrow_kernel, dim3(nb), dim3(256), 0, st, (const float*)dyb->ptr, (int)(dyb->pitch / 4), P, dyb->c, rpb, part);
  else
    hipLaunchKernelGGL(colsum_partial_kernel, dim3(nb, pm_cdiv(dyb->c, 64)), dim3(256), 0, st, (const float*)dyb->ptr, (long)dyb->pitch, P, dyb->c, rpb, part);
  hipLaunchKernelGGL(colsum_final_kernel, dim3(pm_cdiv(dyb->c, 64)), dim3(1024), 0, st, (const float*)part, nb, dyb->c, dbias);
  return pm_check_launch("conv_bias_grad");
}
```

### pinthememory_amd/csrc/conv_igemm_kernel.h

```cpp
#pragma once
#include <stdint.h>
#include <type_traits>

#include "pm_common.h"

typedef float f32x16 __attribute__((ext_vector_type(16)));
typedef __bf16 bf16x8 __attribute__((ext_vector_type(8)));

struct ConvK {
  const float* A;
  const float* B;
  float* C;
  int N, H, W, Cin;
  int Ho, Wo, Cout;
  long x_pitch, y_pitch;
  int kh, kw, stride, pad, dil, sshift;
  int M, Nn, K;
  int ksplit;
  int kper;
  long c_pitch;
  long c_split;
  long a_bs, b_bs, c_bs;
  int tiles_m, tiles_n;
  unsigned a_bytes, b_bytes;
  int kmode;
  int prec;
  int T_eff, tk_w, ky0, kx0, ksy, ksx;
  int sub, sub_cy, sub_cx, Hc, Wc;
  const float* bias;
  const float* scale;
  const float* shift;
  const float* residual;
  long res_pitch;
  const unsigned char* res_mask;
  int relu;
  float* stats;
  int io16;
  int stage_ep;
  int n_group;
  int batch_xcd;
  int spl_prio;
};

int pm_conv_split_launch(int mode, int bm, int bn, const ConvK& k, unsigned gx, unsigned gy, unsigned gz, size_t smem, hipStream_t st);
size_t pm_conv_split_stage_bytes(int mode, int bm, int bn);

namespace {

enum { MODE_FWD = 0, MODE_DGRAD = 1, MODE_WGRAD = 2 };
constexpr int BK = 32;
constexpr int LDK = 36;


typedef float v4f __attribute__((ext_vector_type(4)));
constexpr int OOB = 0x7fffffff;

__device__ __forceinline__ float4 bload(__amdgpu_buffer_rsrc_t r, int off) {
  const v4f v = __builtin_bit_cast(v4f, __builtin_amdgcn_raw_buffer_load_b128(r, off, 0, 0));
  return make_float4(v.x, v.y, v.z, v.w);
}

__device__ __forceinline__ int xcd_remap(int bid, int nwg) {
  const int q = nwg >> 3, r = nwg & 7, xcd = bid & 7, idx = bid >> 3;
  const int base = xcd < r ? xcd * (q + 1) : r * (q + 1) + (xcd - r) * q;
  return base + idx;
}

enum { K_FAST = 0, K_MID = 1, K_SMALL = 2, K_PW = 3 };

template <int MODE, int BM, int BN, int WM, int WN, int KM, int PREC, int NST, bool STATS = false>
__global__ __launch_bounds__(256, 2) void conv_igemm_kernel(const ConvK a) {
  constexpr bool A_KC = (MODE != MODE_WGRAD);
  constexpr bool B_KC = (MODE == MODE_FWD);
  constexpr bool FAST = (KM == K_FAST || KM == K_PW) && (MODE != MODE_WGRAD);
  constexpr bool PW = (KM == K_PW) && (MODE != MODE_WGRAD);
  constexpr int TM = BM / WM / 32, TN = BN / WN / 32;
  constexpr bool TR = (PREC == 3 || PREC == 4);
  constexpr bool NAT16 = (PREC == 4);
  constexpr bool SPL = (PREC == 5);
  constexpr int LD5 = 52;
  constexpr int KX = NAT16 ? 2 : 1, BKW = BK * KX;
  static_assert(!TR || MODE == MODE_WGRAD, "PREC 3 / 4 are the weight-gradient forms");
  constexpr int LDA_T = BM + 32, LDB_T = BN + 32;
  constexpr int PLANE_A = BK * LDA_T / 2, PLANE_B = BK * LDB_T / 2;
  constexpr int A_FLOATS = SPL ? (A_KC ? BM * LD5 : 3 * PLANE_A) : (A_KC ? BM * LDK : (TR ? BKW * LDA_T / 2 : BK * BM));
  constexpr int B_FLOATS = SPL ? (B_KC ? BN * LD5 : 3 * PLANE_B) : (B_KC ? BN * LDK : (TR ? BKW * LDB_T / 2 : BK * BN));
  constexpr int STAGE = A_FLOATS + B_FLOATS;
  constexpr int A_N = BM / 32, B_N = BN / 32;
  static_assert(WM * WN == 4 && TM >= 1 && TN >= 1 && BK == 32, "bad tile config");

  extern __shared__ __align__(16) float smem[];
  if constexpr (PREC == 5) {
    if (a.spl_prio && (__builtin_amdgcn_s_getreg(0x1804) & 1)) __builtin_amdgcn_s_setprio(2);
  }

  const int t = threadIdx.x;
  const int lane = t & 63, wave = t >> 6;
  const int wm = wave / WN, wn = wave % WN;
  const int half = lane >> 5, l31 = lane & 31;
  const int g = t & 7, r = t >> 3;

  const int ntile = a.tiles_m * a.tiles_n;
  int lid, by, z;
  if (a.batch_xcd) {
    const int L = blockIdx.x + ntile * (blockIdx.y + gridDim.y * blockIdx.z), xcd = L & 7, idx = L >> 3;
    const int units = (int)(gridDim.y * gridDim.z), whole = units >> 3, rem = units & 7;
    int u;
    if (idx < whole * ntile) {
      u = xcd + 8 * (idx / ntile), lid = idx % ntile;
    } else {
      const int share = 8 / rem, per = ntile / share;
      u = whole * 8 + xcd / share, lid = (xcd % share) * per + (idx - whole * ntile);
    }
    by = u % (int)gridDim.y, z = u / (int)gridDim.y;
  } else {
    lid = xcd_remap(blockIdx.x, ntile), by = blockIdx.y, z = blockIdx.z;
  }
  int tile_m, tile_n;
  if (a.n_group > 0 && a.tiles_n > a.n_group) {
    const int gsz = a.tiles_m * a.n_group, grp = lid / gsz, rem = lid - grp * gsz;
    const int gw = min(a.n_group, a.tiles_n - grp * a.n_group);
    tile_m = rem / gw, tile_n = grp * a.n_group + rem % gw;
  } else {
    tile_m = lid / a.tiles_n, tile_n = lid % a.tiles_n;
  }
  const int m0 = tile_m * BM, n0 = tile_n * BN;
  const int k_begin = z * a.kper;
  const int k_end = min(a.K, k_begin + a.kper);
  const int nk = (k_end - k_begin + BKW - 1) / BKW;
  const int T = a.T_eff;
  const int Treal = a.kh * a.kw;

  const __amdgpu_buffer_rsrc_t rA = __builtin_amdgcn_make_buffer_rsrc(const_cast<float*>(a.A + by * a.a_bs), 0, (int)a.a_bytes, 0x00020000);
  const __amdgpu_buffer_rsrc_t rB = __builtin_amdgcn_make_buffer_rsrc(const_cast<float*>(a.B + by * a.b_bs), 0, (int)a.b_bytes, 0x00020000);
  const int xp4 = (int)a.x_pitch * (NAT16 ? 2 : 4), yp4 = (int)a.y_pitch * (NAT16 ? 2 : 4);
  constexpr int A_NL = NAT16 ? (A_N + 1) / 2 : A_N, B_NL = NAT16 ? (B_N + 1) / 2 : B_N;
  constexpr int EPL = NAT16 ? 8 : 4;

  int u_ch = 0, u_tap = 0, u_ky = 0, u_kx = 0;
  int a_ch = 0, a_tap = 0, a_ky = 0, a_kx = 0;
  int b_co = 0, b_tap = 0;
  int p_ox = 0, p_oy = 0, p_img = 0;
  int q_ox = 0, q_oy = 0, q_img = 0;
  int a_base[A_N], a_y0[A_N], a_x0[A_N];
  int a_col4[A_N];
  int b_base[B_N];
  int b_dy[B_N], b_dx[B_N];

  if constexpr (MODE == MODE_FWD || MODE == MODE_DGRAD) {
    const int rh = (MODE == MODE_FWD) ? a.Ho : (a.sub ? a.Hc : a.H), rw = (MODE == MODE_FWD) ? a.Wo : (a.sub ? a.Wc : a.W);
    const int cdim = (MODE == MODE_FWD) ? a.Cin : a.Cout;
    const bool pointwise = FAST && a.kh * a.kw == 1 && a.stride == 1 && a.pad == 0 && !a.sub;
#pragma unroll
    for (int i = 0; i < A_N; ++i) {
      const int m = m0 + r + 32 * i;
      if (PW) {
        a_y0[i] = a_x0[i] = 0;
        a_base[i] = m < a.M ? m * (MODE == MODE_FWD ? xp4 : yp4) + g * 16 : OOB;
      } else if (pointwise) {
        a_y0[i] = a_x0[i] = m < a.M ? 0 : -(1 << 28);
        a_base[i] = m < a.M ? m * (MODE == MODE_FWD ? xp4 : yp4) + (FAST ? g * 16 : 0) : 0;
      } else if (m < a.M) {
        const int img = m / (rh * rw), rem = m - img * (rh * rw);
        const int py = rem / rw, px = rem - py * rw;
        if constexpr (MODE == MODE_FWD) {
          a_y0[i] = py * a.stride - a.pad;
          a_x0[i] = px * a.stride - a.pad;
          a_base[i] = (img * a.H * a.W + a_y0[i] * a.W + a_x0[i]) * xp4 + (FAST ? g * 16 : 0);
        } else {
          a_y0[i] = (a.sub ? 2 * py + a.sub_cy : py) + a.pad;
          a_x0[i] = (a.sub ? 2 * px + a.sub_cx : px) + a.pad;
          a_base[i] = FAST ? ((img * a.Ho + a_y0[i]) * a.Wo + a_x0[i]) * yp4 + g * 16 : img * a.Ho * a.Wo;
        }
      } else {
        a_base[i] = 0;
        a_y0[i] = -(1 << 28);
        a_x0[i] = -(1 << 28);
      }
    }
    if constexpr (FAST) {
      u_tap = __builtin_amdgcn_readfirstlane(k_begin / cdim);
      u_ch = k_begin - u_tap * cdim;
      u_ky = u_tap / a.kw;
      u_kx = u_tap - u_ky * a.kw;
    } else {
      const int k = k_begin + g * 4;
      a_tap = k / cdim;
      a_ch = k - a_tap * cdim;
      a_ky = a_tap / a.tk_w;
      a_kx = a_tap - a_ky * a.tk_w;
    }
  } else {
#pragma unroll
    for (int j = 0; j < A_NL; ++j) {
      const int col = m0 + (g + 8 * j) * EPL;
      a_col4[j] = col < a.Cout ? col * (NAT16 ? 2 : 4) : OOB;
    }
  }
  if constexpr (MODE == MODE_FWD) {
#pragma unroll
    for (int i = 0; i < B_N; ++i) {
      const int row = n0 + r + 32 * i;
      b_base[i] = row < a.Cout ? row * a.K * 4 + g * 16 : OOB;
    }
  } else if constexpr (MODE == MODE_DGRAD) {
#pragma unroll
    for (int j = 0; j < B_N; ++j) {
      const int col = n0 + (g + 8 * j) * 4;
      b_base[j] = col < a.Cin ? col * 4 + (FAST ? r * Treal * a.Cin * 4 : 0) : OOB;
    }
    if constexpr (!FAST) {
      const int k = k_begin + r;
      b_tap = k / a.Cout;
      b_co = k - b_tap * a.Cout;
    }
  } else {
#pragma unroll
    for (int j = 0; j < B_NL; ++j) {
      const int n = n0 + (g + 8 * j) * EPL;
      const int tap = n < a.Nn ? n / a.Cin : 0;
      const int ky = tap / a.kw, kx = tap - ky * a.kw;
      b_dy[j] = ky * a.dil - a.pad;
      b_dx[j] = kx * a.dil - a.pad;
      b_base[j] = n < a.Nn ? (b_dy[j] * a.W + b_dx[j]) * xp4 + (n - tap * a.Cin) * (NAT16 ? 2 : 4) : OOB;
    }
    const int p = k_begin + r;
    p_img = p / (a.Ho * a.Wo);
    const int rem = p - p_img * (a.Ho * a.Wo);
    p_oy = rem / a.Wo;
    p_ox = rem - p_oy * a.Wo;
    if constexpr (KX == 2) {
      const int q = p + 32;
      q_img = q / (a.Ho * a.Wo);
      const int rq = q - q_img * (a.Ho * a.Wo);
      q_oy = rq / a.Wo;
      q_ox = rq - q_oy * a.Wo;
    }
  }

  float4 ra[A_N], rb[B_N];

  auto load_tiles = [&](int kt, int which = 0) {
    const int kbase = k_begin + kt * BKW;
    const bool doA = which != 2, doB = which != 1;
    if constexpr (PW) {
      const unsigned beyond = 0x80000000u;
      const bool tok = u_tap < T;
      if constexpr (MODE == MODE_FWD) {
        const unsigned toff = (unsigned)(u_ch * 4) + (tok ? 0u : beyond), kb4 = kbase < k_end ? (unsigned)(kbase * 4) : beyond;
        if (doA)
#pragma unroll
        for (int i = 0; i < A_N; ++i) ra[i] = bload(rA, (int)((unsigned)a_base[i] + toff));
        if (doB)
#pragma unroll
        for (int i = 0; i < B_N; ++i) rb[i] = bload(rB, (int)((unsigned)b_base[i] + kb4));
      } else {
        const unsigned toff = (unsigned)(u_ch * 4) + (tok ? 0u : beyond), uoff = tok ? (unsigned)((u_ch * Treal + u_tap) * a.Cin * 4) : beyond;
        if (doA)
#pragma unroll
        for (int i = 0; i < A_N; ++i) ra[i] = bload(rA, (int)((unsigned)a_base[i] + toff));
        if (doB)
#pragma unroll
        for (int j = 0; j < B_N; ++j) rb[j] = bload(rB, (int)((unsigned)b_base[j] + uoff));
      }
    } else if constexpr (MODE == MODE_FWD) {
      const int ky = FAST ? u_ky : a_ky, kx = FAST ? u_kx : a_kx, tap = FAST ? u_tap : a_tap, ch = FAST ? u_ch : a_ch;
      const int dy = ky * a.dil, dx = kx * a.dil;
      const int toff = (dy * a.W + dx) * xp4 + ch * 4;
      const bool tok = tap < T;
      if (doA)
#pragma unroll
      for (int i = 0; i < A_N; ++i) {
        const bool ok = ((unsigned)(a_y0[i] + dy) < (unsigned)a.H) & ((unsigned)(a_x0[i] + dx) < (unsigned)a.W) & tok;
        const int off = a_base[i] + toff;
        ra[i] = bload(rA, ok ? off : OOB);
      }
      const bool kok = FAST ? (kbase < k_end) : (kbase + g * 4 < k_end);
      if (doB)
#pragma unroll
      for (int i = 0; i < B_N; ++i) {
        const int off = b_base[i] + kbase * 4;
        rb[i] = bload(rB, (kok & (b_base[i] != OOB)) ? off : OOB);
      }
    } else if constexpr (MODE == MODE_DGRAD) {
      if constexpr (FAST) {
        const int dy = u_ky * a.dil, dx = u_kx * a.dil;
        const int toff = (dy * a.Wo + dx) * yp4 - u_ch * 4;
        const bool tok = u_tap < T;
        if (doA)
#pragma unroll
        for (int i = 0; i < A_N; ++i) {
          const bool ok = ((unsigned)(a_y0[i] - dy) < (unsigned)a.Ho) & ((unsigned)(a_x0[i] - dx) < (unsigned)a.Wo) & tok;
          const int off = a_base[i] - toff;
          ra[i] = bload(rA, ok ? off : OOB);
        }
        const int uoff = (u_ch * Treal + u_tap) * a.Cin * 4;
        if (doB)
#pragma unroll
        for (int j = 0; j < B_N; ++j) {
          const int off = b_base[j] + uoff;
          rb[j] = bload(rB, (tok & (b_base[j] != OOB)) ? off : OOB);
        }
      } else {
        const int dy = (a.ky0 + a.ksy * a_ky) * a.dil, dx = (a.kx0 + a.ksx * a_kx) * a.dil, smask = a.stride - 1;
        const bool kok = a_tap < T;
        if (doA)
#pragma unroll
        for (int i = 0; i < A_N; ++i) {
          const int ty = a_y0[i] - dy, tx = a_x0[i] - dx;
          const int oy = ty >> a.sshift, ox = tx >> a.sshift;
          const bool ok = kok & ((ty | tx) >= 0) & (((ty | tx) & smask) == 0) & (oy < a.Ho) & (ox < a.Wo);
          const int off = (a_base[i] + oy * a.Wo + ox) * yp4 + a_ch * 4;
          ra[i] = bload(rA, ok ? off : OOB);
        }
        const bool rok = (b_tap < T) & (kbase + r < k_end);
        const int b_tky = b_tap / a.tk_w, b_tkx = b_tap - b_tky * a.tk_w;
        const int roff = (b_co * Treal + (a.ky0 + a.ksy * b_tky) * a.kw + a.kx0 + a.ksx * b_tkx) * a.Cin * 4;
        if (doB)
#pragma unroll
        for (int j = 0; j < B_N; ++j) {
          const int off = roff + b_base[j];
          rb[j] = bload(rB, (rok & (b_base[j] != OOB)) ? off : OOB);
        }
      }
    } else {
#pragma unroll
      for (int kk = 0; kk < KX; ++kk) {
        const int p = kbase + r + 32 * kk;
        const bool pok = p < k_end;
        const int poff = p * yp4;
        if (doA)
#pragma unroll
        for (int j = 0; j < A_NL; ++j) {
          const int off = poff + a_col4[j];
          ra[kk * A_NL + j] = bload(rA, (pok & (a_col4[j] != OOB)) ? off : OOB);
        }
        const int by = (kk ? q_oy : p_oy) * a.stride, bx = (kk ? q_ox : p_ox) * a.stride;
        const int rowbase = (((kk ? q_img : p_img) * a.H + by) * a.W + bx) * xp4;
        if (doB)
#pragma unroll
        for (int j = 0; j < B_NL; ++j) {
          const bool ok = pok & (b_base[j] != OOB) & ((unsigned)(by + b_dy[j]) < (unsigned)a.H) & ((unsigned)(bx + b_dx[j]) < (unsigned)a.W);
          const int off = rowbase + b_base[j];
          rb[kk * B_NL + j] = bload(rB, ok ? off : OOB);
        }
      }
    }
  };

  auto advance = [&]() {
    if constexpr (MODE == MODE_FWD || MODE == MODE_DGRAD) {
      const int cdim = (MODE == MODE_FWD) ? a.Cin : a.Cout;
      if constexpr (FAST) {
        u_ch += BK;
        if (u_ch >= cdim) {
          u_ch = 0;
          ++u_tap;
          if (++u_kx == a.kw) u_kx = 0, ++u_ky;
        }
      } else {
        a_ch += BK;
        if constexpr (KM == K_SMALL) {
          while (a_ch >= cdim) {
            a_ch -= cdim;
            ++a_tap;
            if (++a_kx == a.tk_w) a_kx = 0, ++a_ky;
          }
        } else {
          const bool wrap = a_ch >= cdim;
          a_ch -= wrap ? cdim : 0;
          a_tap += wrap ? 1 : 0;
          const bool roww = wrap & (a_kx + 1 == a.tk_w);
          a_kx = roww ? 0 : a_kx + (wrap ? 1 : 0);
          a_ky += roww ? 1 : 0;
        }
        if constexpr (MODE == MODE_DGRAD) {
          b_co += BK;
          if constexpr (KM == K_SMALL) {
            while (b_co >= a.Cout) b_co -= a.Cout, ++b_tap;
          } else {
            const bool wrap = b_co >= a.Cout;
            b_co -= wrap ? a.Cout : 0;
            b_tap += wrap ? 1 : 0;
          }
        }
      }
    } else {
      auto step = [&](int& ox, int& oy, int& img) {
        ox += BKW;
        if constexpr (KM == K_SMALL) {
          while (ox >= a.Wo) {
            ox -= a.Wo;
            if (++oy == a.Ho) oy = 0, ++img;
          }
        } else {
          const bool wrap = ox >= a.Wo;
          ox -= wrap ? a.Wo : 0;
          const bool imgw = wrap & (oy + 1 == a.Ho);
          oy = imgw ? 0 : oy + (wrap ? 1 : 0);
          img += imgw ? 1 : 0;
        }
      };
      step(p_ox, p_oy, p_img);
      if constexpr (KX == 2) step(q_ox, q_oy, q_img);
    }
  };

  auto pack4 = [](const float4& v) {
    typedef __bf16 bf16x4 __attribute__((ext_vector_type(4)));
    bf16x4 o;
    o[0] = (__bf16)v.x, o[1] = (__bf16)v.y, o[2] = (__bf16)v.z, o[3] = (__bf16)v.w;
    return __builtin_bit_cast(float2, o);
  };
  auto split4 = [](const float4& v, float2& h, float2& m, float2& l) {
    const unsigned u0 = __float_as_uint(v.x), u1 = __float_as_uint(v.y), u2 = __float_as_uint(v.z), u3 = __float_as_uint(v.w);
    h.x = __uint_as_float(__builtin_amdgcn_perm(u1, u0, 0x07060302)), h.y = __uint_as_float(__builtin_amdgcn_perm(u3, u2, 0x07060302));
    const float r0 = v.x - __uint_as_float(u0 & 0xffff0000u), r1 = v.y - __uint_as_float(u1 & 0xffff0000u);
    const float r2 = v.z - __uint_as_float(u2 & 0xffff0000u), r3 = v.w - __uint_as_float(u3 & 0xffff0000u);
    const unsigned q0 = __float_as_uint(r0), q1 = __float_as_uint(r1), q2 = __float_as_uint(r2), q3 = __float_as_uint(r3);
    m.x = __uint_as_float(__builtin_amdgcn_perm(q1, q0, 0x07060302)), m.y = __uint_as_float(__builtin_amdgcn_perm(q3, q2, 0x07060302));
    const float s0 = r0 - __uint_as_float(q0 & 0xffff0000u), s1 = r1 - __uint_as_float(q1 & 0xffff0000u);
    const float s2 = r2 - __uint_as_float(q2 & 0xffff0000u), s3 = r3 - __uint_as_float(q3 & 0xffff0000u);
    l.x = __uint_as_float(__builtin_amdgcn_perm(__float_as_uint(s1), __float_as_uint(s0), 0x07060302));
    l.y = __uint_as_float(__builtin_amdgcn_perm(__float_as_uint(s3), __float_as_uint(s2), 0x07060302));
  };
  float2 sa[SPL ? A_N : 1][3], sb[SPL ? B_N : 1][3];
  auto split_a = [&]() {
    if constexpr (SPL) {
#pragma unroll
      for (int i = 0; i < A_N; ++i) split4(ra[i], sa[i][0], sa[i][1], sa[i][2]);
    }
  };
  auto split_b = [&]() {
    if constexpr (SPL) {
#pragma unroll
      for (int i = 0; i < B_N; ++i) split4(rb[i], sb[i][0], sb[i][1], sb[i][2]);
    }
  };
  auto write_planes = [&](int buf) {
    if constexpr (SPL) {
      float* As = smem + buf * STAGE;
      float* Bs = As + A_FLOATS;
#pragma unroll
      for (int i = 0; i < A_N; ++i) {
        if constexpr (A_KC) {
          float* d = As + (r + 32 * i) * LD5 + g * 2;
          *reinterpret_cast<float2*>(d) = sa[i][0], *reinterpret_cast<float2*>(d + 16) = sa[i][1], *reinterpret_cast<float2*>(d + 32) = sa[i][2];
        } else {
          float* d = As + (r * LDA_T + (g + 8 * i) * 4) / 2;
          *reinterpret_cast<float2*>(d) = sa[i][0], *reinterpret_cast<float2*>(d + PLANE_A) = sa[i][1], *reinterpret_cast<float2*>(d + 2 * PLANE_A) = sa[i][2];
        }
      }
#pragma unroll
      for (int i = 0; i < B_N; ++i) {
        if constexpr (B_KC) {
          float* d = Bs + (r + 32 * i) * LD5 + g * 2;
          *reinterpret_cast<float2*>(d) = sb[i][0], *reinterpret_cast<float2*>(d + 16) = sb[i][1], *reinterpret_cast<float2*>(d + 32) = sb[i][2];
        } else {
          float* d = Bs + (r * LDB_T + (g + 8 * i) * 4) / 2;
          *reinterpret_cast<float2*>(d) = sb[i][0], *reinterpret_cast<float2*>(d + PLANE_B) = sb[i][1], *reinterpret_cast<float2*>(d + 2 * PLANE_B) = sb[i][2];
        }
      }
    }
  };
  auto store_tiles = [&](int buf) {
    float* As = smem + buf * STAGE;
    float* Bs = As + A_FLOATS;
    if constexpr (SPL) {
      split_a();
      split_b();
      write_planes(buf);
      return;
    }
    if constexpr (NAT16) {
#pragma unroll
      for (int kk = 0; kk < KX; ++kk) {
#pragma unroll
        for (int i = 0; i < A_NL; ++i)
          *reinterpret_cast<float4*>(reinterpret_cast<char*>(As) + ((r + 32 * kk) * LDA_T + (g + 8 * i) * 8) * 2) = ra[kk * A_NL + i];
#pragma unroll
        for (int i = 0; i < B_NL; ++i)
          *reinterpret_cast<float4*>(reinterpret_cast<char*>(Bs) + ((r + 32 * kk) * LDB_T + (g + 8 * i) * 8) * 2) = rb[kk * B_NL + i];
      }
      return;
    }
#pragma unroll
    for (int i = 0; i < A_NL; ++i) {
      if constexpr (A_KC) *reinterpret_cast<float4*>(As + (r + 32 * i) * LDK + g * 4) = ra[i];
      else if constexpr (NAT16) *reinterpret_cast<float4*>(reinterpret_cast<char*>(As) + (r * LDA_T + (g + 8 * i) * 8) * 2) = ra[i];
      else if constexpr (TR) *reinterpret_cast<float2*>(reinterpret_cast<char*>(As) + (r * LDA_T + (g + 8 * i) * 4) * 2) = pack4(ra[i]);
      else *reinterpret_cast<float4*>(As + r * BM + (g + 8 * i) * 4) = ra[i];
    }
#pragma unroll
    for (int i = 0; i < B_NL; ++i) {
      if constexpr (B_KC) *reinterpret_cast<float4*>(Bs + (r + 32 * i) * LDK + g * 4) = rb[i];
      else if constexpr (NAT16) *reinterpret_cast<float4*>(reinterpret_cast<char*>(Bs) + (r * LDB_T + (g + 8 * i) * 8) * 2) = rb[i];
      else if constexpr (TR) *reinterpret_cast<float2*>(reinterpret_cast<char*>(Bs) + (r * LDB_T + (g + 8 * i) * 4) * 2) = pack4(rb[i]);
      else *reinterpret_cast<float4*>(Bs + r * BN + (g + 8 * i) * 4) = rb[i];
    }
  };

  f32x16 acc[TM][TN];
#pragma unroll
  for (int i = 0; i < TM; ++i)
#pragma unroll
    for (int j = 0; j < TN; ++j)
#pragma unroll
      for (int q = 0; q < 16; ++q) acc[i][j][q] = 0.f;

  auto compute_kg = [&](int buf, int kg) {
    const float* As = smem + buf * STAGE;
    const float* Bs = As + A_FLOATS;
    if constexpr (TR) {
      if (kg & 1) return;
      typedef short s16x4 __attribute__((ext_vector_type(4)));
      typedef short s16x8 __attribute__((ext_vector_type(8)));
      const int krow = (kg >> 1) * 16 + half * 8 + ((lane & 15) >> 2);
      const int cofs = ((lane >> 4) & 1) * 16 + (lane & 3) * 4;
      auto frag = [&](const float* T, int ld, int col0) {
        const short* base = reinterpret_cast<const short*>(T) + krow * ld + col0 + cofs;
        const s16x4 lo = __builtin_amdgcn_ds_read_tr16_b64_v4i16((__attribute__((address_space(3))) s16x4*)(base));
        const s16x4 hi = __builtin_amdgcn_ds_read_tr16_b64_v4i16((__attribute__((address_space(3))) s16x4*)(base + 4 * ld));
        const s16x8 v = {lo[0], lo[1], lo[2], lo[3], hi[0], hi[1], hi[2], hi[3]};
        return __builtin_bit_cast(bf16x8, v);
      };
      bf16x8 fa[TM], fb[TN];
#pragma unroll
      for (int i = 0; i < TM; ++i) fa[i] = frag(As, LDA_T, wm * (BM / WM) + i * 32);
#pragma unroll
      for (int i = 0; i < TN; ++i) fb[i] = frag(Bs, LDB_T, wn * (BN / WN) + i * 32);
#pragma unroll
      for (int i = 0; i < TM; ++i)
#pragma unroll
        for (int n = 0; n < TN; ++n)
          acc[i][n] = __builtin_amdgcn_mfma_f32_32x32x16_bf16(fa[i], fb[n], acc[i][n], 0, 0, 0);
    } else if constexpr (SPL) {
      if (kg & 1) return;
      typedef short s16x4 __attribute__((ext_vector_type(4)));
      typedef short s16x8 __attribute__((ext_vector_type(8)));
      const int krow = (kg >> 1) * 16 + half * 8 + ((lane & 15) >> 2);
      const int cofs = ((lane >> 4) & 1) * 16 + (lane & 3) * 4;
      auto frag_t = [&](const float* T, int ld, int col0) {
        const short* base = reinterpret_cast<const short*>(T) + krow * ld + col0 + cofs;
        const s16x4 lo = __builtin_amdgcn_ds_read_tr16_b64_v4i16((__attribute__((address_space(3))) s16x4*)(base));
        const s16x4 hi = __builtin_amdgcn_ds_read_tr16_b64_v4i16((__attribute__((address_space(3))) s16x4*)(base + 4 * ld));
        const s16x8 v = {lo[0], lo[1], lo[2], lo[3], hi[0], hi[1], hi[2], hi[3]};
        return __builtin_bit_cast(bf16x8, v);
      };
      const int kk = (kg >> 1) * 8 + half * 4;
      bf16x8 fa[3][TM], fb[3][TN];
#pragma unroll
      for (int p = 0; p < 3; ++p) {
#pragma unroll
        for (int i = 0; i < TM; ++i) {
          if constexpr (A_KC) fa[p][i] = __builtin_bit_cast(bf16x8, *reinterpret_cast<const float4*>(As + (wm * (BM / WM) + i * 32 + l31) * LD5 + p * 16 + kk));
          else fa[p][i] = frag_t(As + p * PLANE_A, LDA_T, wm * (BM / WM) + i * 32);
        }
#pragma unroll
        for (int i = 0; i < TN; ++i) {
          if constexpr (B_KC) fb[p][i] = __builtin_bit_cast(bf16x8, *reinterpret_cast<const float4*>(Bs + (wn * (BN / WN) + i * 32 + l31) * LD5 + p * 16 + kk));
          else fb[p][i] = frag_t(Bs + p * PLANE_B, LDB_T, wn * (BN / WN) + i * 32);
        }
      }
#define PM_SPL_PROD(PA, PB)                                                                                  \
  _Pragma("unroll") for (int i = 0; i < TM; ++i) _Pragma("unroll") for (int n = 0; n < TN; ++n) acc[i][n] = \
      __builtin_amdgcn_mfma_f32_32x32x16_bf16(fa[PA][i], fb[PB][n], acc[i][n], 0, 0, 0);
      PM_SPL_PROD(2, 0) PM_SPL_PROD(0, 2) PM_SPL_PROD(1, 1) PM_SPL_PROD(1, 0) PM_SPL_PROD(0, 1) PM_SPL_PROD(0, 0)
#undef PM_SPL_PROD
    } else if constexpr (PREC == 2) {
      static_assert(A_KC && B_KC, "bf16 tiles need k-contiguous operands (forward form)");
      const int kk = kg * 8 + half * 4;
      bf16x8 fa[TM], fb[TN];
#pragma unroll
      for (int i = 0; i < TM; ++i) fa[i] = __builtin_bit_cast(bf16x8, *reinterpret_cast<const float4*>(As + (wm * (BM / WM) + i * 32 + l31) * LDK + kk));
#pragma unroll
      for (int i = 0; i < TN; ++i) fb[i] = __builtin_bit_cast(bf16x8, *reinterpret_cast<const float4*>(Bs + (wn * (BN / WN) + i * 32 + l31) * LDK + kk));
#pragma unroll
      for (int i = 0; i < TM; ++i)
#pragma unroll
        for (int n = 0; n < TN; ++n)
          acc[i][n] = __builtin_amdgcn_mfma_f32_32x32x16_bf16(fa[i], fb[n], acc[i][n], 0, 0, 0);
    } else if constexpr (PREC == 0) {
      const int kk = kg * 8 + half * 4;
      float fa[TM][4], fb[TN][4];
#pragma unroll
      for (int i = 0; i < TM; ++i) {
        const int row = wm * (BM / WM) + i * 32 + l31;
        if constexpr (A_KC) {
          const float4 v = *reinterpret_cast<const float4*>(As + row * LDK + kk);
          fa[i][0] = v.x, fa[i][1] = v.y, fa[i][2] = v.z, fa[i][3] = v.w;
        } else {
#pragma unroll
          for (int j = 0; j < 4; ++j) fa[i][j] = As[(kk + j) * BM + row];
        }
      }
#pragma unroll
      for (int i = 0; i < TN; ++i) {
        const int col = wn * (BN / WN) + i * 32 + l31;
        if constexpr (B_KC) {
          const float4 v = *reinterpret_cast<const float4*>(Bs + col * LDK + kk);
          fb[i][0] = v.x, fb[i][1] = v.y, fb[i][2] = v.z, fb[i][3] = v.w;
        } else {
#pragma unroll
          for (int j = 0; j < 4; ++j) fb[i][j] = Bs[(kk + j) * BN + col];
        }
      }
#pragma unroll
      for (int j = 0; j < 4; ++j)
#pragma unroll
        for (int i = 0; i < TM; ++i)
#pragma unroll
          for (int n = 0; n < TN; ++n)
            acc[i][n] = __builtin_amdgcn_mfma_f32_32x32x2f32(fa[i][j], fb[n][j], acc[i][n], 0, 0, 0);
    } else {
      if (kg & 1) return;
      const int kk = (kg >> 1) * 16 + half * 8;
      bf16x8 fa[TM], fb[TN];
#pragma unroll
      for (int i = 0; i < TM; ++i) {
        const int row = wm * (BM / WM) + i * 32 + l31;
        float v[8];
        if constexpr (A_KC) {
          const float4 p = *reinterpret_cast<const float4*>(As + row * LDK + kk), q = *reinterpret_cast<const float4*>(As + row * LDK + kk + 4);
          v[0] = p.x, v[1] = p.y, v[2] = p.z, v[3] = p.w, v[4] = q.x, v[5] = q.y, v[6] = q.z, v[7] = q.w;
        } else {
#pragma unroll
          for (int j = 0; j < 8; ++j) v[j] = As[(kk + j) * BM + row];
        }
#pragma unroll
        for (int j = 0; j < 8; ++j) fa[i][j] = (__bf16)v[j];
      }
#pragma unroll
      for (int i = 0; i < TN; ++i) {
        const int col = wn * (BN / WN) + i * 32 + l31;
        float v[8];
        if constexpr (B_KC) {
          const float4 p = *reinterpret_cast<const float4*>(Bs + col * LDK + kk), q = *reinterpret_cast<const float4*>(Bs + col * LDK + kk + 4);
          v[0] = p.x, v[1] = p.y, v[2] = p.z, v[3] = p.w, v[4] = q.x, v[5] = q.y, v[6] = q.z, v[7] = q.w;
        } else {
#pragma unroll
          for (int j = 0; j < 8; ++j) v[j] = Bs[(kk + j) * BN + col];
        }
#pragma unroll
        for (int j = 0; j < 8; ++j) fb[i][j] = (__bf16)v[j];
      }
#pragma unroll
      for (int i = 0; i < TM; ++i)
#pragma unroll
        for (int n = 0; n < TN; ++n)
          acc[i][n] = __builtin_amdgcn_mfma_f32_32x32x16_bf16(fa[i], fb[n], acc[i][n], 0, 0, 0);
    }
  };
  auto compute = [&](int buf) {
#pragma unroll
    for (int kg = 0; kg < BKW / 8; ++kg) compute_kg(buf, kg);
  };

  if constexpr (SPL && NST == 1) {
    if (nk > 0) {
      load_tiles(0);
      advance();
      split_a(), split_b();
      write_planes(0);
      __syncthreads();
      load_tiles(1);
      advance();
      constexpr int NDS = 3 * (TM * (A_KC ? 1 : 2) + TN * (B_KC ? 1 : 2));
      constexpr int NMF = 6 * TM * TN;
      for (int kt = 0; kt < nk; ++kt) {
        compute_kg(0, 0);
        split_a();
        load_tiles(kt + 2, 1);
        __builtin_amdgcn_sched_group_barrier(0x100, NDS, 0);
#pragma unroll
        for (int q = 0; q < NMF; ++q) {
          __builtin_amdgcn_sched_group_barrier(0x008, 1, 0);
          __builtin_amdgcn_sched_group_barrier(0x006, 5, 0);
        }
        __builtin_amdgcn_sched_barrier(0);
        compute_kg(0, 2);
        split_b();
        load_tiles(kt + 2, 2);
        __builtin_amdgcn_sched_group_barrier(0x100, NDS, 0);
#pragma unroll
        for (int q = 0; q < NMF; ++q) {
          __builtin_amdgcn_sched_group_barrier(0x008, 1, 0);
          __builtin_amdgcn_sched_group_barrier(0x006, 5, 0);
        }
        __builtin_amdgcn_sched_barrier(0);
        __syncthreads();
        write_planes(0);
        __syncthreads();
        advance();
      }
    }
  } else if constexpr (NST == 1) {
    if (nk > 0) {
      load_tiles(0);
      advance();
      store_tiles(0);
      __syncthreads();
      for (int kt = 0; kt < nk - 1; ++kt) {
        load_tiles(kt + 1);
        __builtin_amdgcn_sched_barrier(0);
        advance();
        compute(0);
        __syncthreads();
        store_tiles(0);
        __syncthreads();
      }
      compute(0);
    }
  } else if (nk > 0) {
    load_tiles(0);
    advance();
    store_tiles(0);
    __syncthreads();
    for (int kt = 0; kt < nk - 1; ++kt) {
      compute_kg(kt & 1, 0);
      load_tiles(kt + 1);
      advance();
      __builtin_amdgcn_sched_group_barrier(0x100, TM + TN + (A_KC ? 0 : 3 * TM) + (B_KC ? 0 : 3 * TN), 0);
#define PM_SG(I)                                                                   \
      if constexpr ((A_NL + B_NL) * KX > I) {                                                \
        __builtin_amdgcn_sched_group_barrier(0x008, 2, 0);   \
        __builtin_amdgcn_sched_group_barrier(0x006, 8, 0);   \
        __builtin_amdgcn_sched_group_barrier(0x020, 1, 0);   \
      }
      PM_SG(0) PM_SG(1) PM_SG(2) PM_SG(3) PM_SG(4) PM_SG(5) PM_SG(6) PM_SG(7)
#undef PM_SG
      __builtin_amdgcn_sched_barrier(0);
#pragma unroll
      for (int kg = 1; kg < BKW / 8; ++kg) compute_kg(kt & 1, kg);
      store_tiles((kt + 1) & 1);
      __syncthreads();
    }
    compute((nk - 1) & 1);
  }

  float* Cb = a.C + by * a.c_bs + (a.ksplit > 1 ? (long)z * a.c_split : 0);
  const bool plain = a.ksplit > 1 || !(a.bias || a.scale || a.residual || a.relu);
  const bool full = m0 + BM <= a.M && n0 + BN <= a.Nn;
  const int rbase = m0 + wm * (BM / WM) + 4 * half, cbase = n0 + wn * (BN / WN) + l31;
  const bool out16 = a.io16 && a.ksplit == 1;
  if (out16 && ((a.c_pitch | a.Nn | (a.residual ? a.res_pitch : 0)) & 7) == 0 &&
      ((reinterpret_cast<uintptr_t>(a.C) | reinterpret_cast<uintptr_t>(a.residual)) & 15) == 0) {
    constexpr int WC = BN / WN, LDC = WC + 4, LPR = WC / 8, RPI = 64 / LPR;
    static_assert(32 % RPI == 0, "row segments must tile the 32-row slab");
    __syncthreads();
    float* Ws = smem + wave * 32 * LDC;
    const int rr0 = lane / LPR, cc = (lane % LPR) * 8;
    const int col = n0 + wn * WC + cc;
    const bool cok = col < a.Nn;
    const bool aff = a.bias || a.scale, res = a.residual != nullptr, relu = a.relu != 0;
    float bi[8], sc[8], sh[8];
#pragma unroll
    for (int e = 0; e < 8; ++e) bi[e] = 0.f, sc[e] = 1.f, sh[e] = 0.f;
    if (aff && cok) {
#pragma unroll
      for (int e = 0; e < 8; ++e) {
        if (a.bias) bi[e] = a.bias[col + e];
        if (a.scale) sc[e] = a.scale[col + e], sh[e] = a.shift[col + e];
      }
    }
    pm_bf16* C16 = reinterpret_cast<pm_bf16*>(a.C) + by * a.c_bs;
    const pm_bf16* R16 = reinterpret_cast<const pm_bf16*>(a.residual);
#pragma unroll
    for (int i = 0; i < TM; ++i) {
#pragma unroll
      for (int n = 0; n < TN; ++n)
#pragma unroll
        for (int q = 0; q < 16; ++q) Ws[((q & 3) + 8 * (q >> 2) + 4 * half) * LDC + n * 32 + l31] = acc[i][n][q];
#pragma unroll
      for (int r0 = 0; r0 < 32; r0 += RPI) {
        const int rr = r0 + rr0;
        const long row = m0 + wm * (BM / WM) + i * 32 + rr;
        const float4 v0 = *reinterpret_cast<const float4*>(Ws + rr * LDC + cc), v1 = *reinterpret_cast<const float4*>(Ws + rr * LDC + cc + 4);
        float v[8] = {v0.x, v0.y, v0.z, v0.w, v1.x, v1.y, v1.z, v1.w};
        if (row < a.M && cok) {
          if (aff) {
#pragma unroll
            for (int e = 0; e < 8; ++e) v[e] = (v[e] + bi[e]) * sc[e] + sh[e];
          }
          if (res) {
            float q[8];
            pm_ld8(R16 + row * a.res_pitch + col, q);
#pragma unroll
            for (int e = 0; e < 8; ++e) v[e] += q[e];
          }
          if (relu) {
#pragma unroll
            for (int e = 0; e < 8; ++e) v[e] = fmaxf(v[e], 0.f);
          }
          pm_st8(C16 + row * a.c_pitch + col, v);
        }
      }
      if constexpr (STATS) {
        if (a.stats) pm_slab_stats16<LDC, LPR, RPI>(Ws, rr0, cc, (long)m0 + wm * (BM / WM) + i * 32, a.M, a.Nn, col, cok, bi, sc, sh, a.stats);
      }
    }
    return;
  }
  if (out16) {
    pm_bf16* C16 = reinterpret_cast<pm_bf16*>(a.C) + by * a.c_bs;
    const pm_bf16* R16 = reinterpret_cast<const pm_bf16*>(a.residual);
#pragma unroll
    for (int i = 0; i < TM; ++i)
#pragma unroll
      for (int n = 0; n < TN; ++n) {
        const int col = cbase + n * 32;
        const bool cok = col < a.Nn;
        float bi = 0.f, sc = 1.f, sh = 0.f;
        if (cok) {
          if (a.bias) bi = a.bias[col];
          if (a.scale) sc = a.scale[col], sh = a.shift[col];
        }
#pragma unroll
        for (int q = 0; q < 16; ++q) {
          const int row = rbase + i * 32 + (q & 3) + 8 * (q >> 2);
          if (row < a.M && cok) {
            float v = (acc[i][n][q] + bi) * sc + sh;
            if (R16) v += pm_bf16_to_f32(R16[(long)row * a.res_pitch + col]);
            if (a.relu) v = fmaxf(v, 0.f);
            C16[(long)row * a.c_pitch + col] = pm_f32_to_bf16(v);
          }
        }
      }
    return;
  }
  const bool vec = a.stage_ep && ((a.c_pitch | a.Nn | (a.residual ? a.res_pitch : 0)) & 3) == 0 &&
                   ((reinterpret_cast<uintptr_t>(Cb) | reinterpret_cast<uintptr_t>(a.residual)) & 15) == 0;
  if (vec) {
    constexpr int WC = BN / WN, LDC = WC + 4, LPR = WC / 4, RPI = 64 / LPR;
    static_assert(32 % RPI == 0, "row segments must tile the 32-row slab");
    __syncthreads();
    float* Ws = smem + wave * 32 * LDC;
    const int rr0 = lane / LPR, cc = (lane % LPR) * 4;
    const int col = n0 + wn * WC + cc;
    const bool cok = col < a.Nn;
    const bool aff = !plain && (a.bias || a.scale), res = !plain && a.residual, relu = !plain && a.relu;
    float bi[4] = {0.f, 0.f, 0.f, 0.f}, sc[4] = {1.f, 1.f, 1.f, 1.f}, sh[4] = {0.f, 0.f, 0.f, 0.f};
    if (aff && cok) {
#pragma unroll
      for (int e = 0; e < 4; ++e) {
// ... 138 lines not shown
```

### pinthememory_amd/csrc/conv_split.hip

```cpp
#include <stdlib.h>
#include <algorithm>

#include "conv_igemm_kernel.h"

namespace {

template <int MODE, int BM, int BN, int KM>
void launch_split(const ConvK& k, dim3 grid, size_t smem, hipStream_t st) {
  const size_t ep_bytes = (size_t)4 * 32 * (BN / 2 + 4) * sizeof(float);
  const size_t bytes = std::max(smem, ep_bytes);
  if constexpr (MODE == MODE_FWD) {
    if (k.stats) {
      static pm_lds_optin optin;
      (void)optin(reinterpret_cast<const void*>(&conv_igemm_kernel<MODE, BM, BN, 2, 2, KM, 5, 1, true>), 160 * 1024);
      hipLaunchKernelGGL((conv_igemm_kernel<MODE, BM, BN, 2, 2, KM, 5, 1, true>), grid, dim3(256), bytes, st, k);
      return;
    }
  }
  static pm_lds_optin optin;
  (void)optin(reinterpret_cast<const void*>(&conv_igemm_kernel<MODE, BM, BN, 2, 2, KM, 5, 1>), 160 * 1024);
  hipLaunchKernelGGL((conv_igemm_kernel<MODE, BM, BN, 2, 2, KM, 5, 1>), grid, dim3(256), bytes, st, k);
}

template <int MODE, int BM, int BN>
void launch_km(const ConvK& k, dim3 grid, size_t smem, hipStream_t st) {
  if (k.kmode == K_SMALL) return launch_split<MODE, BM, BN, K_SMALL>(k, grid, smem, st);
  if constexpr (MODE != MODE_WGRAD) {
    if (k.kmode == K_FAST && k.kh * k.kw == 1 && k.stride == 1 && k.pad == 0 && !k.sub) return launch_split<MODE, BM, BN, K_PW>(k, grid, smem, st);
    if (k.kmode == K_FAST) return launch_split<MODE, BM, BN, K_FAST>(k, grid, smem, st);
  }
  launch_split<MODE, BM, BN, K_MID>(k, grid, smem, st);
}

template <int MODE>
int launch_tile(int bm, int bn, const ConvK& k, dim3 grid, size_t smem, hipStream_t st) {
  if (bm == 128 && bn == 128) launch_km<MODE, 128, 128>(k, grid, smem, st);
  else if (bm == 128 && bn == 64) launch_km<MODE, 128, 64>(k, grid, smem, st);
  else if (bm == 64 && bn == 128) launch_km<MODE, 64, 128>(k, grid, smem, st);
  else if (bm == 64 && bn == 64) launch_km<MODE, 64, 64>(k, grid, smem, st);
  else {
    pm_set_error("conv_split: no %d x %d tile", bm, bn);
    return PM_EUNSUPPORTED;
  }
  return PM_OK;
}

}

size_t pm_conv_split_stage_bytes(int mode, int bm, int bn) {
  const bool akc = mode != MODE_WGRAD, bkc = mode == MODE_FWD;
  const size_t a = akc ? (size_t)bm * 52 * 4 : (size_t)3 * BK * (bm + 32) * 2;
  const size_t b = bkc ? (size_t)bn * 52 * 4 : (size_t)3 * BK * (bn + 32) * 2;
  return a + b;
}

int pm_conv_split_launch(int mode, int bm, int bn, const ConvK& k, unsigned gx, unsigned gy, unsigned gz, size_t smem, hipStream_t st) {
  const dim3 grid(gx, gy, gz);
  if (mode == MODE_FWD) return launch_tile<MODE_FWD>(bm, bn, k, grid, smem, st);
  if (mode == MODE_DGRAD) return launch_tile<MODE_DGRAD>(bm, bn, k, grid, smem, st);
  return launch_tile<MODE_WGRAD>(bm, bn, k, grid, smem, st);
}
```

### pinthememory_amd/hip/kernels.py

```python
import ctypes
from ctypes import byref

import os
import weakref

import torch

from . import lib as L
from .lib import PmConvEpilogue, PmConvParams, check, ptr, stream, tdesc, workspace


def _lib():
    return L.load()


CONV_PREC = 0
ACT_DTYPE = torch.float32


def set_conv_precision(name):
    global CONV_PREC, ACT_DTYPE
    CONV_PREC = {'f32': 0, 'fp32': 0, 'bf16': 2, 'bf16_operands': 2, 'bf16_staged': 1}[name]
    ACT_DTYPE = torch.bfloat16 if name == 'bf16' else torch.float32


def _act_dtype(like):
    return like.dtype if like.dtype in (torch.float32, torch.bfloat16) else torch.float32


def new(shape, like, pitch_pad=False, zero_pad=True, dtype=None):
    n, h, w, c = shape
    dtype = _act_dtype(like) if dtype is None else dtype
    if dtype == torch.bfloat16:
        if c % 64:
            base = torch.empty((n, h, w, (c + 63) // 64 * 64), dtype=dtype, device=like.device)
            base[..., c:].zero_()
            L.register_zero_pad(base, c, base.shape[3])
            return base[..., :c]
        return torch.empty((n, h, w, c), dtype=dtype, device=like.device)
    if c % 4 and pitch_pad:
        cp = (c + 3) // 4 * 4
        alloc = torch.zeros if zero_pad else torch.empty
        return alloc((n, h, w, cp), dtype=torch.float32, device=like.device)[..., :c]
    return torch.empty((n, h, w, c), dtype=torch.float32, device=like.device)


def cast(x, dtype):
    if x.dtype == dtype:
        return x
    y = torch.empty(x.shape, dtype=dtype, device=x.device)
    check(_lib().pm_cast(byref(tdesc(x)), byref(tdesc(y)), stream()), 'pm_cast')
    return y


def conv_out_hw(h, w, k, stride, pad, dil):
    return (h + 2 * pad - dil * (k - 1) - 1) // stride + 1, (w + 2 * pad - dil * (k - 1) - 1) // stride + 1


def krsc(w):
    v = w.permute(0, 2, 3, 1)
    return v if v.is_contiguous() else v.contiguous()


KEEP_WINOGRAD_V = os.environ.get('PM_KEEP_V', '1') == '1'


BN_EPILOGUE = os.environ.get('PM_BN_EPILOGUE', '0') == '1'
BN_EPILOGUE16 = os.environ.get('PM_BN_EPILOGUE16', '0') == '1'
BN_EP16_MIN_BYTES = int(float(os.environ.get('PM_BN_EP16_MIN_MB', '0')) * (1 << 20))
BN_EP_MIN_BYTES = int(float(os.environ.get('PM_BN_EP_MIN_MB', '0')) * (1 << 20))


KEEP_WINOGRAD_U = {'0': False, '1': True}.get(os.environ.get('PM_KEEP_U', ''))

_U_OWNERS = {}
_U_CACHE_MAX = 256
_U_CACHE_BYTES = int(os.environ.get('PM_KEEP_U_MB', '2048')) << 20


def register_filter_owners(params):
    for p in params:
        if isinstance(p, torch.nn.Parameter) and p.is_leaf and p.is_cuda and p.dim() == 4 and p.dtype == torch.float32:
            _U_OWNERS[p.data_ptr()] = weakref.ref(p)


def unregister_filter_owners(params=None):
    ptrs = None if params is None else {p.data_ptr() for p in params}
    for k in [k for k in _U_OWNERS if ptrs is None or k in ptrs]:
        del _U_OWNERS[k]
    _U_CACHE.drop_if(lambda ent: ptrs is None or ent.ptr in ptrs)


def _filter_owner(w_krsc):
    ref = _U_OWNERS.get(w_krsc.data_ptr())
    p = ref() if ref is not None else None
    if p is None:
        if ref is not None:
            del _U_OWNERS[w_krsc.data_ptr()]
        return None
    return p if (p.data_ptr() == w_krsc.data_ptr() and p.numel() == w_krsc.numel() and p.is_leaf) else None


class _KeptFilter:
    __slots__ = ('ptr', 'shape', 'nbytes', 'device', 'prec', 'dgrad', 'owner', 'version', 'buf', 'event', 'stream', 'used')


class _FilterCache(dict):
    def __init__(self):
        self.nbytes = 0
        self.streams = {}

    def _stream(self):
        raw = stream()
        cur = self.streams.get(raw)
        if cur is None:
            cur = self.streams[raw] = L.stream_obj()
        return raw, cur

    def _drop(self, key):
        ent = self.pop(key)
        self.nbytes -= ent.nbytes
        if ent.buf.is_cuda:
            for s in self.streams.values():
                ent.buf.record_stream(s)

    def drop_if(self, pred):
        for key in [k for k, ent in self.items() if pred(ent)]:
            self._drop(key)

    def clear(self):
        self.drop_if(lambda ent: True)

    def lookup(self, p, w_krsc, nbu, dgrad=False):
        if KEEP_WINOGRAD_U is False or not nbu:
            return None
        registered = _filter_owner(w_krsc)
        if registered is None and KEEP_WINOGRAD_U is not True:
            return None
        owner = w_krsc if registered is None else registered
        key = (w_krsc.data_ptr(), tuple(w_krsc.shape), nbu, w_krsc.device.index, p.prec, dgrad)
        ent = self.get(key)
        if ent is not None and ent.owner() is not owner:
            self._drop(key)
            ent = None
        if ent is None:
            self.drop_if(lambda e: e.owner() is None)
            while self and (len(self) >= _U_CACHE_MAX or self.nbytes + nbu > _U_CACHE_BYTES):
                self._drop(next(iter(self)))
            ent = _KeptFilter()
            ent.ptr, ent.shape, ent.nbytes, ent.device, ent.prec, ent.dgrad = key
            ent.owner = (lambda: w_krsc) if registered is None else weakref.ref(registered)
            ent.version, ent.buf, ent.event, ent.stream = -1, torch.empty(nbu // 4, dtype=torch.float32, device=w_krsc.device), None, None
            self.nbytes += nbu
        else:
            del self[key]
        self[key] = ent
        ent.used = True
        version = owner._version
        valid = ent.version == version
        if not valid:
            ent.version = -1
        p.wxf, p.wxf_bytes, p.wxf_valid = ent.buf.data_ptr(), nbu, 1 if valid else 0
        raw, cur = self._stream()
        if valid and ent.event is not None and ent.stream != raw:
            cur.wait_event(ent.event)
        return None if valid else (ent, version)

    def commit(self, *pending):
        raw, cur = self._stream()
        event = cur.record_event()
        for ent, version in pending:
            ent.version, ent.event, ent.stream = version, event, raw

    def forget_events(self):
        for ent in self.values():
            ent.event = ent.stream = None


_U_CACHE = _FilterCache()
clear_filters, forget_filter_events = _U_CACHE.clear, _U_CACHE.forget_events

_REFRESH = {2: ('pm_conv_wxf_refresh_bf16', False), 0: ('pm_conv_wxf_refresh_f32', True)}


def refresh_filters():
    if KEEP_WINOGRAD_U is False or not _U_CACHE or CONV_PREC not in _REFRESH:
        return 0
    entry_point, forward_3x3_only = _REFRESH[CONV_PREC]
    dev = torch.cuda.current_device()
    todo = []
    for ent in _U_CACHE.values():
        if ent.prec != CONV_PREC or ent.device != dev or not ent.used:
            continue
        cout, kh, kw, cin = ent.shape
        if forward_3x3_only and (ent.dgrad or kh != 3 or kw != 3):
            continue
        ent.used = False
        owner = ent.owner()
        if owner is None or owner.data_ptr() != ent.ptr or ent.version == owner._version or not ent.buf.is_cuda:
            continue
        todo.append((ent, owner._version))
    if not todo:
        return 0
    jobs = (L.PmWxfJob * len(todo))()
    for j, (ent, version) in zip(jobs, todo):
        cout, kh, kw, cin = ent.shape
        j.w, j.wxf, j.wxf_bytes, j.cout, j.kh, j.kw, j.cin, j.dgrad = ent.ptr, ent.buf.data_ptr(), ent.nbytes, cout, kh, kw, cin, 1 if ent.dgrad else 0
        ent.version = -1
    check(getattr(_lib(), entry_point)(jobs, len(todo), stream()), entry_point)
    _U_CACHE.commit(*todo)
    return len(todo)


_SIZES = {}
_GEN = [0]


def _sizes(key, fn):
    v = _SIZES.get(key)
    if v is None:
        if len(_SIZES) > 8192:
            _SIZES.clear()
        v = _SIZES[key] = fn()
    return v


_XFORM_COUNT = [0, False]


def filter_transform_count(enable=None):
    if enable is not None:
        _XFORM_COUNT[1] = bool(enable)
    return _XFORM_COUNT[0]


def conv_fwd(x, w_krsc, stride, pad, dil, bias=None, scale=None, shift=None, residual=None, relu=False, out=None, keep_v=None, bn_partials=None, out_dtype=None):
    cout, kh, kw, cin = w_krsc.shape
    n, h, w_, c = x.shape
    assert c == cin, 'conv: Cin mismatch %d vs %d' % (c, cin)
    ho, wo = conv_out_hw(h, w_, kh, stride, pad, dil)
    y = out if out is not None else new((n, ho, wo, cout), x, pitch_pad=True, dtype=out_dtype if out_dtype is not None else ACT_DTYPE)
    assert residual is None or residual.dtype == y.dtype, 'conv_fwd: the fused residual has the dtype of the output'
    xd, yd = tdesc(x), tdesc(y)
    p = L.conv_params(kh, kw, stride, pad, dil, CONV_PREC)
    lib = _lib()
    nbv, nbu, nb, npb = _sizes(('f', x.shape, x.stride(), x.dtype, xd.flags, w_krsc.shape, y.stride(), y.dtype, stride, pad, dil, CONV_PREC, _GEN[0]),
                               lambda: (lib.pm_conv_winograd_v_bytes(byref(xd), byref(yd), byref(p)), lib.pm_conv_wxf_bytes(byref(xd), byref(yd), byref(p)),
                                        lib.pm_conv_workspace(byref(xd), byref(yd), byref(p), 0), lib.pm_conv_bn_partials_bytes(byref(xd), byref(yd), byref(p))))
    if keep_v is not None:
        nbv = nbv if KEEP_WINOGRAD_V else 0
        v = torch.empty(nbv // 4, dtype=torch.float32, device=x.device) if nbv else None
        keep_v.append(v)
        if v is not None:
            p.wino_v, p.wino_v_bytes = v.data_ptr(), nbv
    u_ent = None
    if (kh == 3 and CONV_PREC == 0) or CONV_PREC == 2:
        u_ent = _U_CACHE.lookup(p, w_krsc, nbu)
    if _XFORM_COUNT[1] and p.wxf_valid == 0 and nbu:
        _XFORM_COUNT[0] += 1
    ws = workspace(nb, x.device) if nb else None
    part = None
    if bn_partials is not None:
        ep16 = BN_EPILOGUE16 or (BN_EP16_MIN_BYTES > 0 and y.numel() * 2 >= BN_EP16_MIN_BYTES)
        ep32 = BN_EPILOGUE or (BN_EP_MIN_BYTES > 0 and y.numel() * 4 >= BN_EP_MIN_BYTES)
        npb = npb if ((ep16 if y.dtype == torch.bfloat16 else ep32) and residual is None and not relu and scale is None) else 0
        part = torch.empty(npb // 4, dtype=torch.float32, device=x.device) if npb else None
        bn_partials.append(part)
    ep = None
    if bias is not None or scale is not None or residual is not None or relu or part is not None:
        rd = tdesc(residual) if residual is not None else None
        ep = L.conv_epilogue(ptr(bias), ptr(scale), ptr(shift), rd.ptr if rd else None, rd.pitch if rd else 0, 1 if relu else 0, ptr(part),
                            part.numel() * 4 if part is not None else 0)
    check(lib.pm_conv_fwd(byref(xd), w_krsc.data_ptr(), byref(yd), byref(p), byref(ep) if ep else None, ptr(ws), nb, stream()), 'pm_conv_fwd')
    if u_ent is not None:
        _U_CACHE.commit(u_ent)
    return y


def conv_bwd_data(dy, w_krsc, x_shape, stride, pad, dil, add=None, dtype=None, add_mask=None):
    cout, kh, kw, cin = w_krsc.shape
    dx = new(x_shape, dy, dtype=dtype)
    dyd, dxd = tdesc(dy), tdesc(dx)
    p = L.conv_params(kh, kw, stride, pad, dil, CONV_PREC)
    lib = _lib()
    nb, nbu = _sizes(('d', dy.shape, dy.stride(), dy.dtype, dyd.flags, w_krsc.shape, dx.shape, dx.stride(), dx.dtype, stride, pad, dil, CONV_PREC, _GEN[0]),
                     lambda: (lib.pm_conv_workspace(byref(dxd), byref(dyd), byref(p), 1), lib.pm_conv_wxf_bytes_dgrad(byref(dyd), byref(dxd), byref(p))))
    ws = workspace(nb, dy.device) if nb else None
    ad = tdesc(add) if add is not None else None
    u_ent = _U_CACHE.lookup(p, w_krsc, nbu, dgrad=True) if CONV_PREC == 2 else None
    if add_mask is not None:
        check(lib.pm_conv_bwd_data_masked(byref(dyd), w_krsc.data_ptr(), byref(dxd), byref(p), byref(ad), add_mask.data_ptr(), ptr(ws), nb, stream()), 'pm_conv_bwd_data_masked')
    else:
        check(lib.pm_conv_bwd_data(byref(dyd), w_krsc.data_ptr(), byref(dxd), byref(p), byref(ad) if ad else None, ptr(ws), nb, stream()), 'pm_conv_bwd_data')
    if u_ent is not None:
        _U_CACHE.commit(u_ent)
    return dx


def conv_bwd_weight(x, dy, w_shape_krsc, stride, pad, dil, want_bias=False, wino_v=None, on_stream=None):
    cout, kh, kw, cin = w_shape_krsc
    dw = torch.empty(w_shape_krsc, dtype=torch.float32, device=x.device)
    db = torch.empty(cout, dtype=torch.float32, device=x.device) if want_bias else None
    xd, dyd = tdesc(x), tdesc(dy)
    p = L.conv_params(kh, kw, stride, pad, dil, CONV_PREC)
    if wino_v is not None:
        p.wino_v, p.wino_v_bytes = wino_v.data_ptr(), wino_v.numel() * 4
    lib = _lib()
    nb = _sizes(('w', x.shape, x.stride(), x.dtype, dy.shape, dy.stride(), dy.dtype, w_shape_krsc, stride, pad, dil, CONV_PREC, wino_v is not None, _GEN[0]),
                lambda: lib.pm_conv_workspace(byref(xd), byref(dyd), byref(p), 2))
    raw = stream() if on_stream is None else on_stream.cuda_stream
    ws = workspace(nb, x.device, on_stream)
    check(lib.pm_conv_bwd_weight(byref(xd), byref(dyd), dw.data_ptr(), ptr(db), byref(p), ptr(ws), nb, raw), 'pm_conv_bwd_weight')
    return dw, db


def bn_stats(x):
    c = x.shape[3]
    mom = torch.empty(3 * c, dtype=torch.float32, device=x.device)
    xd = tdesc(x)
    lib = _lib()
    nb = _sizes(('bn', x.shape, x.dtype), lambda: lib.pm_bn_workspace(byref(xd)))
    ws = workspace(nb, x.device)
    check(lib.pm_bn_stats(byref(xd), mom.data_ptr(), ptr(ws), nb, stream()), 'pm_bn_stats')
    return mom


def bn_stats_finalize(x, eps, running_mean=None, running_var=None, momentum=0.1):
    c = x.shape[3]
    mean = torch.empty(c, dtype=torch.float32, device=x.device)
    invstd = torch.empty_like(mean)
    xd = tdesc(x)
    lib = _lib()
    nb = _sizes(('bn', x.shape, x.dtype), lambda: lib.pm_bn_workspace(byref(xd)))
    ws = workspace(nb, x.device)
    check(lib.pm_bn_stats_finalize(byref(xd), eps, mean.data_ptr(), invstd.data_ptr(), ptr(running_mean), ptr(running_var), momentum, ptr(ws), nb, stream()),
          'pm_bn_stats_finalize')
    return mean, invstd


def bn_partials_finalize(part, pixels, c, eps, running_mean=None, running_var=None, momentum=0.1):
    mean = torch.empty(c, dtype=torch.float32, device=part.device)
    invstd = torch.empty_like(mean)
    check(_lib().pm_bn_partials_finalize(part.data_ptr(), pixels, c, eps, mean.data_ptr(), invstd.data_ptr(), ptr(running_mean), ptr(running_var), momentum, None,
                                         stream()), 'pm_bn_partials_finalize')
    return mean, invstd


def bn_partials_moments(part, pixels, c):
    mom = torch.empty(3 * c, dtype=torch.float32, device=part.device)
    check(_lib().pm_bn_partials_finalize(part.data_ptr(), pixels, c, 0.0, None, None, None, None, 0.0, mom.data_ptr(), stream()), 'pm_bn_partials_finalize')
    return mom


def bn_merge(parts, world, c):
    out = torch.empty(3 * c, dtype=torch.float32, device=parts.device)
    check(_lib().pm_bn_merge(parts.data_ptr(), world, c, out.data_ptr(), stream()), 'pm_bn_merge')
    return out


def bn_merge_finalize(parts, world, c, eps, running_mean=None, running_var=None, momentum=0.1):
    mean = torch.empty(c, dtype=torch.float32, device=parts.device)
    invstd = torch.empty_like(mean)
    check(_lib().pm_bn_merge_finalize(parts.data_ptr(), world, c, eps, mean.data_ptr(), invstd.data_ptr(), ptr(running_mean), ptr(running_var), momentum,
                                      stream()), 'pm_bn_merge_finalize')
    return mean, invstd


def bn_finalize(moments, c, eps, running_mean=None, running_var=None, momentum=0.1):
    mean = torch.empty(c, dtype=torch.float32, device=moments.device)
    invstd = torch.empty_like(mean)
    check(_lib().pm_bn_finalize(moments.data_ptr(), c, eps, mean.data_ptr(), invstd.data_ptr(), ptr(running_mean), ptr(running_var), momentum, stream()),
          'pm_bn_finalize')
    return mean, invstd


def bn_fold_multi(table, cs, offs, n, max_c, total, eps):
    arena = torch.empty(2 * total, dtype=torch.float32, device=table.device)
    check(_lib().pm_bn_fold_multi(table.data_ptr(), cs.data_ptr(), offs.data_ptr(), n, max_c, total, eps, arena.data_ptr(), stream()), 'pm_bn_fold_multi')
    return arena


def bn_fold(gamma, beta, running_mean, running_var, eps, conv_bias=None):
    c = gamma.numel()
    scale = torch.empty(c, dtype=torch.float32, device=gamma.device)
    shift = torch.empty_like(scale)
    check(_lib().pm_bn_fold(gamma.data_ptr(), beta.data_ptr(), running_mean.data_ptr(), running_var.data_ptr(), ptr(conv_bias), c, eps, scale.data_ptr(),
                            shift.data_ptr(), stream()), 'pm_bn_fold')
    return scale, shift


def bn_apply(x, mean, invstd, gamma, beta, residual=None, relu=False, out=None, want_mask=False):
    y = out if out is not None else torch.empty_like(x, memory_format=torch.contiguous_format)
    rd = tdesc(residual) if residual is not None else None
    grp = 8 if x.dtype == torch.bfloat16 else 4
    mask = torch.empty((x.shape[0] * x.shape[1] * x.shape[2], x.shape[3] // grp), dtype=torch.uint8, device=x.device) if want_mask else None
    check(_lib().pm_bn_apply_mask(byref(tdesc(x)), mean.data_ptr(), invstd.data_ptr(), gamma.data_ptr(), beta.data_ptr(), byref(rd) if rd else None,
                                  1 if relu else 0, byref(tdesc(y)), ptr(mask), stream()), 'pm_bn_apply_mask')
    return (y, mask) if want_mask else y


def bn_apply_res_affine(x, mean, invstd, gamma, beta, r, r_mean, r_invstd, r_gamma, r_beta, relu=False, want_mask=False):
    y = torch.empty_like(x, memory_format=torch.contiguous_format)
    mask = torch.empty((x.shape[0] * x.shape[1] * x.shape[2], x.shape[3] // 4), dtype=torch.uint8, device=x.device) if want_mask else None
    check(_lib().pm_bn_apply_mask_affine(byref(tdesc(x)), mean.data_ptr(), invstd.data_ptr(), gamma.data_ptr(), beta.data_ptr(), byref(tdesc(r)), r_mean.data_ptr(),
                                         r_invstd.data_ptr(), r_gamma.data_ptr(), r_beta.data_ptr(), 1 if relu else 0, byref(tdesc(y)), ptr(mask), stream()),
          'pm_bn_apply_mask_affine')
    return (y, mask) if want_mask else y


def bn_bwd_apply_mask(dy, mask, x, mean, invstd, gamma, sums, count):
    dx = torch.empty(x.shape, dtype=x.dtype, device=x.device)
    check(_lib().pm_bn_bwd_apply_mask(byref(tdesc(dy)), mask.data_ptr(), byref(tdesc(x)), mean.data_ptr(), invstd.data_ptr(), gamma.data_ptr(), sums.data_ptr(),
                                      float(count), byref(tdesc(dx)), stream()), 'pm_bn_bwd_apply_mask')
    return dx


def bn_bwd_reduce_mask(dy, mask, x, mean, invstd, want_gmask=True, with_count=False):
    c = x.shape[3]
    sums = torch.empty(2 * c + (1 if with_count else 0), dtype=torch.float32, device=x.device)
    if with_count:
        sums[2 * c:].fill_(float(x.shape[0] * x.shape[1] * x.shape[2]))
    xd = tdesc(x)
    lib = _lib()
    nb = _sizes(('bn', x.shape, x.dtype), lambda: lib.pm_bn_workspace(byref(xd)))
    ws = workspace(nb, x.device)
    gm = torch.empty(x.shape, dtype=x.dtype, device=x.device) if want_gmask else None
    gd = tdesc(gm) if want_gmask else None
    check(lib.pm_bn_bwd_reduce_mask(byref(tdesc(dy)), mask.data_ptr(), byref(xd), mean.data_ptr(), invstd.data_ptr(), byref(gd) if gd else None,
                                    sums.data_ptr(), ptr(ws), nb, stream()), 'pm_bn_bwd_reduce_mask')
    return sums, gm


def scale_shift_act(x, scale, shift, residual=None, relu=False):
    y = torch.empty(x.shape, dtype=torch.float32, device=x.device)
    rd = tdesc(residual) if residual is not None else None
    check(_lib().pm_scale_shift_act(byref(tdesc(x)), scale.data_ptr(), shift.data_ptr(), byref(rd) if rd else None, 1 if relu else 0, byref(tdesc(y)), stream()),
          'pm_scale_shift_act')
    return y


def bn_bwd_reduce(dy, y, x, mean, invstd, relu, gamma=None, beta=None, want_gmask=False, with_count=False):
    relu = int(relu)
    c = x.shape[3]
    sums = torch.empty(2 * c + (1 if with_count else 0), dtype=torch.float32, device=x.device)
    if with_count:
        sums[2 * c:].fill_(float(x.shape[0] * x.shape[1] * x.shape[2]))
    xd = tdesc(x)
    lib = _lib()
# ... 496 lines not shown
```

### pinthememory_amd/hip/lib.py

```python
import ctypes
import os
from ctypes import POINTER, byref, c_char_p, c_float, c_int, c_int32, c_int64, c_size_t, c_void_p

import torch

_HERE = os.path.dirname(os.path.dirname(os.path.abspath(__file__)))
LIB_PATH = os.environ.get('PM_LIB') or os.path.join(_HERE, 'libpinmem_hip.so')


class PmTensor(ctypes.Structure):
    _fields_ = [('ptr', c_void_p), ('n', c_int32), ('h', c_int32), ('w', c_int32), ('c', c_int32), ('pitch', c_int64), ('dtype', c_int32), ('flags', c_int32)]


PM_F32, PM_BF16 = 0, 1
PM_TF_ZERO_PAD64 = 1


class PmSgdEntry(ctypes.Structure):
    _fields_ = [('param', c_void_p), ('grad', c_void_p), ('momentum_buffer', c_void_p), ('numel', c_int64)]


class PmWxfJob(ctypes.Structure):
    _fields_ = [('w', c_void_p), ('wxf', c_void_p), ('wxf_bytes', c_int64), ('cout', c_int32), ('kh', c_int32), ('kw', c_int32), ('cin', c_int32),
                ('dgrad', c_int32), ('reserved', c_int32)]


class PmConvParams(ctypes.Structure):
    _fields_ = [('struct_size', c_int32), ('kh', c_int32), ('kw', c_int32), ('stride', c_int32), ('pad', c_int32), ('dil', c_int32), ('prec', c_int32),
                ('wino_v', c_void_p), ('wino_v_bytes', c_int64),
                ('wxf', c_void_p), ('wxf_bytes', c_int64), ('wxf_valid', c_int32)]


class PmRouting(ctypes.Structure):
    _fields_ = [('struct_size', c_int32), ('winograd', c_int32), ('winograd_fused', c_int32), ('conv16', c_int32), ('conv16_wide', c_int32),
                ('conv16_persistent', c_int32), ('wgrad16', c_int32), ('bf16_wgrad', c_int32), ('split', c_int32)]


class PmConvEpilogue(ctypes.Structure):
    _fields_ = [('struct_size', c_int64), ('bias', c_void_p), ('scale', c_void_p), ('shift', c_void_p), ('residual', c_void_p),
                ('residual_pitch', c_int64), ('relu', c_int32), ('bn_partials', c_void_p), ('bn_partials_bytes', c_int64)]


def conv_params(kh, kw, stride, pad, dil, prec=0):
    return PmConvParams(ctypes.sizeof(PmConvParams), kh, kw, stride, pad, dil, prec)


def conv_epilogue(*fields):
    return PmConvEpilogue(ctypes.sizeof(PmConvEpilogue), *fields)


ABI_VERSION = 400


class PinmemError(RuntimeError):
    pass


_T, _P, _E = POINTER(PmTensor), POINTER(PmConvParams), POINTER(PmConvEpilogue)
_vp, _sz, _i, _f, _i64 = c_void_p, c_size_t, c_int, c_float, c_int64

SIGNATURES = {
    'pm_last_error': (c_char_p, []),
    'pm_version': (c_int, []),
    'pm_conv_winograd_v_bytes': (_sz, [_T, _T, _P]),
    'pm_conv_wxf_bytes': (_sz, [_T, _T, _P]),
    'pm_conv_wxf_bytes_dgrad': (_sz, [_T, _T, _P]),
    'pm_conv_wxf_refresh_bf16': (_i, [_vp, _i, _vp]),
    'pm_conv_wxf_refresh_f32': (_i, [_vp, _i, _vp]),
    'pm_conv_workspace': (_sz, [_T, _T, _P, _i]),
    'pm_conv_fwd': (_i, [_T, _vp, _T, _P, _E, _vp, _sz, _vp]),
    'pm_conv_bwd_data': (_i, [_T, _vp, _T, _P, _T, _vp, _sz, _vp]),
    'pm_conv_bwd_data_masked': (_i, [_T, _vp, _T, _P, _T, _vp, _vp, _sz, _vp]),
    'pm_conv_bwd_weight': (_i, [_T, _T, _vp, _vp, _P, _vp, _sz, _vp]),
    'pm_set_winograd': (_i, [_i]),
    'pm_set_winograd_fused': (_i, [_i]),
    'pm_set_conv16': (_i, [_i]),
    'pm_profile_enable': (_i, [_i]),
    'pm_profile_dump': (_i, [ctypes.c_char_p]),
    'pm_profile_read': (_i, [_i, _i, _i, _i, _i, POINTER(ctypes.c_double), POINTER(ctypes.c_double), POINTER(c_int64), _i]),
    'pm_profile_read_prec': (_i, [_i, _i, _i, _i, _i, _i, POINTER(ctypes.c_double), POINTER(ctypes.c_double), POINTER(c_int64), _i]),
    'pm_profile_read_bytes': (_i, [_i, _i, _i, _i, _i, _i, POINTER(ctypes.c_double)]),
    'pm_bn_workspace': (_sz, [_T]),
    'pm_bn_stats': (_i, [_T, _vp, _vp, _sz, _vp]),
    'pm_bn_merge': (_i, [_vp, _i, _i, _vp, _vp]),
    'pm_bn_merge_finalize': (_i, [_vp, _i, _i, _f, _vp, _vp, _vp, _vp, _f, _vp]),
    'pm_bn_finalize': (_i, [_vp, _i, _f, _vp, _vp, _vp, _vp, _f, _vp]),
    'pm_bn_stats_finalize': (_i, [_T, _f, _vp, _vp, _vp, _vp, _f, _vp, _sz, _vp]),
    'pm_bn_fold': (_i, [_vp, _vp, _vp, _vp, _vp, _i, _f, _vp, _vp, _vp]),
    'pm_bn_fold_multi': (_i, [_vp, _vp, _vp, _i, _i, _i, _f, _vp, _vp]),
    'pm_bn_apply': (_i, [_T, _vp, _vp, _vp, _vp, _T, _i, _T, _vp]),
    'pm_bn_apply_mask': (_i, [_T, _vp, _vp, _vp, _vp, _T, _i, _T, _vp, _vp]),
    'pm_bn_bwd_reduce_mask': (_i, [_T, _vp, _T, _vp, _vp, _T, _vp, _vp, _sz, _vp]),
    'pm_bn_apply_mask_affine': (_i, [_T, _vp, _vp, _vp, _vp, _T, _vp, _vp, _vp, _vp, _i, _T, _vp, _vp]),
    'pm_bn_bwd_apply_mask': (_i, [_T, _vp, _T, _vp, _vp, _vp, _vp, _f, _T, _vp]),
    'pm_bn_bwd_reduce': (_i, [_T, _T, _T, _vp, _vp, _vp, _vp, _i, _T, _vp, _vp, _sz, _vp]),
    'pm_bn_bwd_apply': (_i, [_T, _T, _T, _vp, _vp, _vp, _vp, _vp, _f, _i, _T, _T, _vp]),
    'pm_relu_bwd': (_i, [_T, _T, _T, _vp]),
    'pm_add': (_i, [_T, _T, _T, _vp]),
    'pm_add_n': (_i, [POINTER(_T), _i, _T, _vp]),
    'pm_copy': (_i, [_T, _T, _vp]),
    'pm_scale_shift_act': (_i, [_T, _vp, _vp, _T, _i, _T, _vp]),
    'pm_maxpool3x3s2_fwd': (_i, [_T, _T, _vp, _vp]),
    'pm_maxpool3x3s2_bwd': (_i, [_T, _vp, _T, _vp]),
    'pm_maxpool3x3s2_bn_relu_fwd': (_i, [_T, _vp, _vp, _vp, _vp, _T, _vp, _vp]),
    'pm_bn_bwd_reduce_pool': (_i, [_T, _vp, _T, _vp, _vp, _vp, _vp, _vp, _vp, _sz, _vp]),
    'pm_bn_bwd_apply_pool': (_i, [_T, _vp, _T, _vp, _vp, _vp, _vp, _vp, _f, _T, _vp]),
    'pm_global_avgpool_fwd': (_i, [_T, _T, _vp]),
    'pm_global_avgpool_bwd': (_i, [_T, _T, _i, _vp]),
    'pm_resize_bilinear_fwd': (_i, [_T, _T, _vp]),
    'pm_resize_bilinear_bwd': (_i, [_T, _T, _i, _vp]),
    'pm_resize_bilinear_bwd_workspace': (_sz, [_T, _T]),
    'pm_resize_bilinear_bwd_separable': (_i, [_T, _T, _i, _vp, _sz, _vp]),
    'pm_resize_bilinear_hp_fwd': (_i, [_T, _T, _i, _vp]),
    'pm_softmax_mean_update': (_i, [_T, _vp, _i, _vp]),
    'pm_sliding_stitch': (_i, [_T, _vp, _i, _i, _i, _i, _vp, _i, _vp]),
    'pm_argmax_f64': (_i, [_vp, _i, _i, _i, _i, _vp, _vp, _vp]),
    'pm_image_u8_to_nhwc4': (_i, [_vp, _i64, POINTER(c_float), POINTER(c_float), _vp, _vp]),
    'pm_labels_u8_to_i64': (_i, [_vp, _i64, _vp, _vp]),
    'pm_nchw_to_nhwc': (_i, [_vp, _i, _T, _vp]),
    'pm_nhwc_to_nchw': (_i, [_T, _vp, _vp]),
    'pm_label_nearest': (_i, [_vp, _i, _i, _i, _vp, _i, _i, _vp]),
    'pm_upsample_ce_workspace': (_sz, [_i, _i, _i]),
    'pm_upsample_ce_fwd': (_i, [_T, _f, _vp, _i, _i, _vp, _vp, _sz, _vp]),
    'pm_upsample_ce_bwd_workspace': (_sz, [_T, _i, _i]),
    'pm_upsample_ce_bwd': (_i, [_T, _f, _vp, _i, _i, _vp, _vp, _T, _vp, _sz, _vp]),
    'pm_upsample_ce_field_bytes': (_sz, [_T, _i, _i]),
    'pm_upsample_ce_fwd_field': (_i, [_T, _f, _vp, _i, _i, _vp, _vp, _vp, _sz, _vp]),
    'pm_upsample_ce_bwd_field': (_i, [_T, _f, _i, _i, _vp, _vp, _vp, _T, _vp]),
    'pm_upsample_wce_loss_floats': (_sz, [_i]),
    'pm_upsample_wce_workspace': (_sz, [_i, _i, _i]),
    'pm_upsample_wce_fwd': (_i, [_T, _f, _vp, _i, _i, _vp, _i64, _i, _vp, _vp, _sz, _vp]),
    'pm_upsample_wce_fwd_field': (_i, [_T, _f, _vp, _i, _i, _vp, _i64, _i, _vp, _vp, _vp, _sz, _vp]),
    'pm_upsample_wce_bwd_field': (_i, [_T, _f, _i, _i, _i, _vp, _vp, _vp, _T, _vp]),
    'pm_label_class_weights_workspace': (_sz, [_i]),
    'pm_label_class_weights': (_i, [_vp, _i, _i, _i, _i, ctypes.c_double, _i, _i, _vp, _vp, _sz, _vp]),
    'pm_upsample_eval_workspace': (_sz, [_T, _i, _i]),
    'pm_upsample_eval': (_i, [_T, _f, _vp, _i, _i, _vp, _vp, _i, _vp, _vp, _sz, _vp]),
    'pm_mem_read_fwd': (_i, [_T, _vp, _i, _vp, _T, _vp, _vp, _vp]),
    'pm_mem_read_fwd_pq_workspace': (_sz, [_i64, _i]),
    'pm_mem_read_fwd_pq': (_i, [_T, _vp, _i, _vp, _vp, _T, _vp, _vp, _vp, _vp, _sz, _vp]),
    'pm_mem_colsoftmax_workspace': (_sz, [_i64, _i]),
    'pm_mem_colsoftmax': (_i, [_vp, _vp, _i64, _i, _vp, _vp, _sz, _vp]),
    'pm_mem_read_bwd_workspace': (_sz, [_i64, _i, _i]),
    'pm_mem_read_bwd': (_i, [_T, _vp, _i, _vp, _T, _vp, _T, _vp, _vp, _sz, _vp]),
    'pm_mem_write_accum_workspace': (_sz, [_T, _i]),
    'pm_mem_write_accum': (_i, [_T, _vp, _i, _i, _i, _i, _vp, _vp, _sz, _vp]),
    'pm_mem_write_accum_bwd': (_i, [_T, _vp, _i, _i, _i, _i, _vp, _T, _vp]),
    'pm_mem_write_update': (_i, [_vp, _vp, _i, _i, _f, _vp, _vp, _vp]),
    'pm_mem_write_update_bwd': (_i, [_vp, _vp, _i, _i, _f, _vp, _vp, _vp, _vp]),
    'pm_sgd_momentum': (_i, [_vp, _vp, _vp, _i64, _f, _f, _f, _i, _vp]),
    'pm_set_bf16_wgrad': (_i, [_i]),
    'pm_set_wgrad16': (_i, [_i]),
    'pm_set_split': (_i, [_i]),
    'pm_routing_get': (_i, [POINTER(PmRouting)]),
    'pm_routing_set': (_i, [POINTER(PmRouting)]),
    'pm_conv_bn_partials_bytes': (_sz, [_T, _T, POINTER(PmConvParams)]),
    'pm_bn_partials_finalize': (_i, [_vp, _i64, _i, _f, _vp, _vp, _vp, _vp, _f, _vp, _vp]),
    'pm_sgd_momentum_multi': (_i, [_vp, _i, _f, _f, _f, _vp]),
    'pm_sgd_momentum_multi_dev': (_i, [_vp, _i, _f, _vp, _f, _f, _vp]),
    'pm_cast': (_i, [_T, _T, _vp]),
}

_lib = None


def load():
    global _lib
    if _lib is not None:
        return _lib
    if not os.environ.get('PM_LIB'):
        from .. import build as _build
        _build.build()
    lib = ctypes.CDLL(LIB_PATH)
    for name, (res, args) in SIGNATURES.items():
        fn = getattr(lib, name)
        fn.restype, fn.argtypes = res, args
    if lib.pm_version() != ABI_VERSION:
        raise PinmemError('%s reports ABI %d, this binding is written against %d (include/pinmem_hip.h)' % (LIB_PATH, lib.pm_version(), ABI_VERSION))
    _lib = lib
    return lib


def check(code, what=''):
    if code != 0:
        raise PinmemError('%s failed (%d): %s' % (what, code, load().pm_last_error().decode()))


_raw_stream = torch._C._cuda_getCurrentRawStream
_cur_device = torch._C._cuda_getDevice


def stream():
    return _raw_stream(_cur_device())


_ZERO_PAD = {}


def register_zero_pad(base, c, pitch):
    import weakref
    if len(_ZERO_PAD) > 64:
        for k in [k for k, v in _ZERO_PAD.items() if v[0]() is None]:
            del _ZERO_PAD[k]
    _ZERO_PAD[base.data_ptr()] = (weakref.ref(base), c, pitch)


_TD = {}


def tdesc(t):
    key = (t.shape, t.stride(), t.dtype)
    m = _TD.get(key)
    if m is None:
        assert t.dim() == 4 and t.dtype in (torch.float32, torch.bfloat16) and t.is_cuda, 'expected a CUDA fp32 / bf16 NHWC tensor, got %s %s' % (tuple(t.shape), t.dtype)
        n, h, w, c = t.shape
        sn, sh, sw, sc = t.stride()
        pitch = sw if w > 1 else (sh if h > 1 else (sn if n > 1 else c))
        assert (sc == 1 or c == 1) and pitch >= c, 'channels must be innermost: shape %s stride %s' % (tuple(t.shape), t.stride())
        assert (h == 1 or w == 1 or sh == w * pitch) and (n == 1 or h * w == 1 or sn == h * w * pitch), \
            'not an NHWC view: shape %s stride %s' % (tuple(t.shape), t.stride())
        if len(_TD) > 4096:
# ... 40 lines not shown
```

Baseline: 154.8.

## Cache pre-split packed weight planes for the split-precision conv path

Adds a packed 6-byte-per-element weight format (split planes) that is computed once per weight version and cached, so split-precision (prec 5) forward and data-gradient kernels load pre-split B operands instead of splitting fp32 weights on the fly in every tile. A new pack kernel, size queries, ABI fields and a Python cache with lazy refresh after optimizer steps are added. This trades extra weight-memory traffic (1.5x bytes) and cache bookkeeping for fewer per-tile conversion instructions in the kernel's B-load path.

```diff
diff --git a/include/pinmem_hip.h b/include/pinmem_hip.h
--- a/include/pinmem_hip.h
+++ b/include/pinmem_hip.h
@@ -20,7 +20,7 @@
   int32_t flags;
 } pm_tensor;
 
-#define PM_ABI_VERSION 400
+#define PM_ABI_VERSION 410
 
 typedef struct pm_conv_params {
   int32_t struct_size;
@@ -31,6 +31,9 @@
   void* wxf;
   int64_t wxf_bytes;
   int32_t wxf_valid;
+  const void* wsplit;
+  int64_t wsplit_bytes;
+  int32_t wsplit_valid;
 } pm_conv_params;
 
 typedef struct pm_conv_epilogue {
@@ -62,6 +65,14 @@
 } pm_wxf_job;
 int pm_conv_wxf_refresh_bf16(const pm_wxf_job* jobs, int n, void* stream);
 int pm_conv_wxf_refresh_f32(const pm_wxf_job* jobs, int n, void* stream);
+typedef struct pm_split_job {
+  const float* src;
+  void* dst;
+  int64_t count;
+} pm_split_job;
+int pm_split_pack_multi(const pm_split_job* jobs, int n, void* stream);
+size_t pm_conv_wsplit_bytes(const pm_tensor* x, const pm_tensor* y, const pm_conv_params* p, int32_t* src_is_wxf);
+size_t pm_conv_wsplit_bytes_dgrad(const pm_tensor* dy, const pm_tensor* dx, const pm_conv_params* p, int32_t* src_is_wxf);
 size_t pm_conv_bn_partials_bytes(const pm_tensor* x, const pm_tensor* y, const pm_conv_params* p);
 int pm_conv_fwd(const pm_tensor* x, const float* w_krsc, const pm_tensor* y, const pm_conv_params* p,
                 const pm_conv_epilogue* ep, void* ws, size_t ws_bytes, void* stream);
diff --git a/pinthememory_amd/csrc/conv_igemm.hip b/pinthememory_amd/csrc/conv_igemm.hip
--- a/pinthememory_amd/csrc/conv_igemm.hip
+++ b/pinthememory_amd/csrc/conv_igemm.hip
@@ -336,6 +336,7 @@
   hipEvent_t a, b;
   int mode, bm, bn, km, prec, nst;
   int M, Nn, K, batch, ksplit;
+  int wsplit;
   double flops;
   double bytes;
 };
@@ -357,6 +358,10 @@
     g_prof.push_back(rec);
   }
 };
+
+inline bool packed_b_ok(int mode, int kmode, unsigned b_bytes) {
+  return mode != MODE_WGRAD && kmode == K_FAST && (double)b_bytes * 1.5 < 2147483000.0 && (b_bytes & 15u) == 0;
+}
 
 inline bool split_takes(int mode, const Plan& p, const ConvK& k, int batch) {
   return pm_route.split != 0 && p.bn >= 64 && !k.io16 && (batch > 1 || split_k_ok(mode, k.K));
@@ -397,6 +402,8 @@
   }
   constexpr bool akc = MODE != MODE_WGRAD, bkc = MODE == MODE_FWD;
   if (k.prec == 5) {
+    if (!packed_b_ok(MODE, k.kmode, k.b_bytes)) k.Bp = nullptr;
+    prof.rec.wsplit = k.Bp ? 1 : 0;
     if (int e = pm_conv_split_launch(MODE, p.bm, p.bn, k, grid.x, grid.y, grid.z, pm_conv_split_stage_bytes(MODE, p.bm, p.bn), st)) return e;
     prof.rec.nst = 1;
     prof.done();
@@ -458,6 +465,7 @@
   k.n_group = 8;
   k.batch_xcd = 0;
   k.a_bs = k.b_bs = k.c_bs = 0;
+  k.Bp = nullptr;
 }
 
 struct WinoPlan {
@@ -500,7 +508,7 @@
 inline size_t wino_ws(const WinoPlan& wp) { return wp.v_bytes + wp.m_bytes + wp.u_bytes; }
 
 int wino_conv(const pm_tensor* xin, const float* w, int w_cout, int w_cin, bool dgrad, const pm_tensor* yout, const WinoPlan& wp,
-              const pm_conv_epilogue& ep, void* ws, hipStream_t st, float* v_keep = nullptr, float* u_ext = nullptr, bool u_valid = false) {
+              const pm_conv_epilogue& ep, void* ws, hipStream_t st, float* v_keep = nullptr, float* u_ext = nullptr, bool u_valid = false, const void* u_packed = nullptr) {
   float* V = v_keep ? v_keep : (float*)ws;
   float* Mo = (float*)((char*)ws + wp.v_bytes);
   float* U = u_ext ? u_ext : (float*)((char*)ws + wp.v_bytes + wp.m_bytes);
@@ -514,6 +522,7 @@
   ConvK k;
   fill_geom(k, &xv, &yv, &p1);
   k.A = V, k.B = U, k.C = Mo;
+  if (u_ext && u_valid) k.Bp = u_packed;
   k.M = (int)wp.g.tiles, k.Nn = cout, k.K = wp.Kp;
   k.a_bytes = (unsigned)(wp.g.tiles * wp.Kp * 4), k.b_bytes = (unsigned)((long)cout * wp.Kp * 4), k.kmode = K_FAST;
   k.c_pitch = cout, k.c_split = 0;
@@ -888,7 +897,24 @@
   size_t v_keep_bytes;
   size_t wxf_bytes;
   size_t bn_bytes;
+  size_t wsplit_bytes;
+  bool wsplit_from_wxf;
 };
+
+bool direct_takes_packed(int mode, const pm_tensor* x, const pm_tensor* y, const pm_conv_params* p, const Plan& pl, long M, long Nn, long K) {
+  const pm_tensor *xin = mode == MODE_FWD ? x : y, *out = mode == MODE_FWD ? y : x;
+  if (!pm_route.split || p->prec != 0 || pl.bn < 64 || !pm_is_f32(out) || !pm_is_f32(xin) || !split_k_ok(mode, K)) return false;
+  const int kmode = (xin->c % BK == 0 && (mode == MODE_FWD || p->stride == 1)) ? K_FAST : K_MID;
+  if (!packed_b_ok(mode, kmode, (unsigned)((long)y->c * p->kh * p->kw * x->c * 4))) return false;
+  if (pl.ksplit == 1 && p->kh * p->kw == 1 && p->stride == 1 && p->pad == 0) {
+    pm_gemm_pw g{};
+    g.A = (const float*)xin->ptr, g.C = (float*)out->ptr;
+    g.a_pitch = xin->pitch, g.c_pitch = out->pitch;
+    g.M = (int)M, g.Nn = (int)Nn, g.K = (int)K;
+    if (pm_pwstream_ok(&g)) return false;
+  }
+  return true;
+}
 
 ConvRoute route_conv(int which, const pm_tensor* x, const pm_tensor* y, const pm_conv_params* p) {
   ConvRoute r{};
@@ -898,10 +924,13 @@
     if ((r.wino = wino_plan(x, y->c, p)).use) {
       r.kind = R_WINO, r.ws_bytes = wino_ws(r.wino), r.wxf_bytes = r.wino.u_bytes;
       r.v_keep_bytes = wino_wgrad_pays(x->c, y->c) ? r.wino.v_bytes : 0;
+      if (pm_route.split && r.wino.pl.bn >= 64 && !pm_route.winograd_fused && packed_b_ok(MODE_FWD, K_FAST, (unsigned)((long)y->c * r.wino.Kp * 4)))
+        r.wsplit_bytes = r.wino.u_bytes / 2 * 3, r.wsplit_from_wxf = true;
     } else if (p->prec == 2 && (r.b16 = bf16_plan(x, y, p)).use) {
       r.kind = R_BF16, r.pe = *p, r.ws_bytes = bf16_ws(r.b16), r.wxf_bytes = r.b16.wb_bytes;
     } else {
       r.kind = R_DIRECT, r.pl = make_plan(MODE_FWD, M, Nn, K, p->prec != 0), r.ws_bytes = pm_align_up(r.pl.ws_bytes, 256);
+      if (direct_takes_packed(MODE_FWD, x, y, p, r.pl, M, Nn, K)) r.wsplit_bytes = (size_t)y->c * p->kh * p->kw * x->c * 6;
     }
     bool bn;
     if (pm_is_bf16(y)) bn = pm_vec8(y) && r.kind == R_BF16 && (r.b16.c16 ? (r.b16.k16.ksplit == 1 && !r.b16.k16.wide) : r.b16.pl.ksplit == 1);
@@ -924,6 +953,7 @@
       r.kind = R_WINO, r.ws_bytes = wino_ws(r.wino);
     } else {
       r.kind = R_DIRECT, r.pl = make_plan(MODE_DGRAD, M, Nn, K, p->prec != 0), r.ws_bytes = pm_align_up(r.pl.ws_bytes, 256);
+      if (direct_takes_packed(MODE_DGRAD, x, y, p, r.pl, M, Nn, K)) r.wsplit_bytes = (size_t)y->c * p->kh * p->kw * x->c * 6;
     }
   } else {
     const bool tier = pm_is_bf16(x) || pm_is_bf16(y);
@@ -948,6 +978,10 @@
     r.dy32_off = r.x32_off - upcast_bytes(y);
   }
   return r;
+}
+
+inline const void* packed_arg(const pm_conv_params* p, const ConvRoute& r) {
+  return (p->wsplit && p->wsplit_valid != 0 && r.wsplit_bytes != 0 && (size_t)p->wsplit_bytes >= r.wsplit_bytes && pm_aligned16(p->wsplit)) ? p->wsplit : nullptr;
 }
 
 int dgrad_s2_parity(const pm_tensor* dy0, const float* w, const pm_tensor* dx, const pm_conv_params* p, const pm_tensor* add, const ConvRoute& r, void* ws, hipStream_t st) {
@@ -983,14 +1017,14 @@
 
 template <int MODE>
 int conv_direct(const pm_tensor* x, const pm_tensor* y, const float* w, const pm_conv_params* p, const Plan& pl, const pm_conv_epilogue& e, void* ws, hipStream_t st,
-                const unsigned char* res_mask = nullptr) {
+                const unsigned char* res_mask = nullptr, const void* w_packed = nullptr) {
   const pm_tensor *xin = MODE == MODE_FWD ? x : y, *out = MODE == MODE_FWD ? y : x;
   long M, Nn, K;
   gemm_dims(MODE, x, y, p, M, Nn, K);
   ConvK k;
   fill_geom(k, x, y, p);
   k.io16 = pm_is_bf16(out) ? 1 : 0;
-  k.A = (const float*)xin->ptr, k.B = w;
+  k.A = (const float*)xin->ptr, k.B = w, k.Bp = w_packed;
   k.M = (int)M, k.Nn = (int)Nn, k.K = (int)K;
   k.a_bytes = (unsigned)(pm_pixels(xin) * xin->pitch * 4), k.b_bytes = (unsigned)((long)y->c * p->kh * p->kw * x->c * 4);
   k.kmode = (xin->c % BK == 0 && (MODE == MODE_FWD || p->stride == 1)) ? 0 : (xin->c >= BK ? 1 : 2);
@@ -1142,11 +1176,11 @@
   PM_REQUIRE(path, PM_EINVAL, "pm_profile_dump: null path");
   FILE* f = fopen(path, "w");
   PM_REQUIRE(f, PM_EINVAL, "pm_profile_dump: cannot open %s", path);
-  fprintf(f, "mode,bm,bn,km,nst,prec,M,N,K,batch,ksplit,ms,gflop\n");
+  fprintf(f, "mode,bm,bn,km,nst,prec,M,N,K,batch,ksplit,ms,gflop,wsplit\n");
   for (const ProfRec& r : g_prof) {
     float t = 0.f;
     if (hipEventSynchronize(r.b) != hipSuccess || hipEventElapsedTime(&t, r.a, r.b) != hipSuccess) continue;
-    fprintf(f, "%d,%d,%d,%d,%d,%d,%d,%d,%d,%d,%d,%.5f,%.4f\n", r.mode, r.bm, r.bn, r.km, r.nst, r.prec, r.M, r.Nn, r.K, r.batch, r.ksplit, t, r.flops * 1e-9);
+    fprintf(f, "%d,%d,%d,%d,%d,%d,%d,%d,%d,%d,%d,%.5f,%.4f,%d\n", r.mode, r.bm, r.bn, r.km, r.nst, r.prec, r.M, r.Nn, r.K, r.batch, r.ksplit, t, r.flops * 1e-9, r.wsplit);
   }
   fclose(f);
   return PM_OK;
@@ -1170,6 +1204,22 @@
   if (!dy || !dx || !p0) return 0;
   const pm_conv_params tp = tier_params(p0, dy, dx);
   return route_conv(MODE_DGRAD, dx, dy, &tp).wxf_bytes;
+}
+extern "C" size_t pm_conv_wsplit_bytes(const pm_tensor* x, const pm_tensor* y, const pm_conv_params* p0, int32_t* src_is_wxf) {
+  if (src_is_wxf) *src_is_wxf = 0;
+  if (!x || !y || !p0 || check_common(x, y, p0) != PM_OK) return 0;
+  const pm_conv_params tp = tier_params(p0, x, y);
+  const ConvRoute r = route_conv(MODE_FWD, x, y, &tp);
+  if (src_is_wxf) *src_is_wxf = r.wsplit_from_wxf ? 1 : 0;
+  return r.wsplit_bytes;
+}
+extern "C" size_t pm_conv_wsplit_bytes_dgrad(const pm_tensor* dy, const pm_tensor* dx, const pm_conv_params* p0, int32_t* src_is_wxf) {
+  if (src_is_wxf) *src_is_wxf = 0;
+  if (!dy || !dx || !p0 || check_common(dx, dy, p0) != PM_OK) return 0;
+  const pm_conv_params tp = tier_params(p0, dy, dx);
+  const ConvRoute r = route_conv(MODE_DGRAD, dx, dy, &tp);
+  if (src_is_wxf) *src_is_wxf = r.wsplit_from_wxf ? 1 : 0;
+  return r.wsplit_bytes;
 }
 extern "C" size_t pm_conv_bn_partials_bytes(const pm_tensor* x, const pm_tensor* y, const pm_conv_params* p0) {
   if (!x || !y || !p0 || check_common(x, y, p0) != PM_OK) return 0;
@@ -1215,11 +1265,12 @@
   }
   PM_REQUIRE(ws_bytes >= r.ws_bytes && (ws || r.ws_bytes == 0), PM_EWORKSPACE, "conv_fwd: workspace %zu < %zu", ws_bytes, r.ws_bytes);
   hipStream_t st = (hipStream_t)stream;
+  const void* wsp = packed_arg(p, r);
   switch (r.kind) {
     case R_WINO: {
       float* keep = (p->wino_v && (size_t)p->wino_v_bytes >= r.wino.v_bytes) ? (float*)p->wino_v : nullptr;
       float* uext = (p->wxf && (size_t)p->wxf_bytes >= r.wino.u_bytes) ? (float*)p->wxf : nullptr;
-      return wino_conv(x, w, y->c, x->c, false, y, r.wino, e0, ws, st, keep, uext, p->wxf_valid != 0);
+      return wino_conv(x, w, y->c, x->c, false, y, r.wino, e0, ws, st, keep, uext, p->wxf_valid != 0, wsp);
     }
     case R_BF16: {
       char* wext = (p->wxf && (size_t)p->wxf_bytes >= r.b16.wb_bytes) ? (char*)p->wxf : nullptr;
@@ -1227,7 +1278,7 @@
     }
     default:
       PM_REQUIRE(pm_is_f32(x), PM_EUNSUPPORTED, "conv_fwd: a bf16 input needs at least 32 channels (got %d)", x->c);
-      return conv_direct<MODE_FWD>(x, y, w, p, r.pl, e0, ws, st);
+      return conv_direct<MODE_FWD>(x, y, w, p, r.pl, e0, ws, st, nullptr, wsp);
   }
 }
 
@@ -1264,7 +1315,7 @@
     case R_WINO: return wino_conv(dy, w, dy->c, dx->c, true, dx, r.wino, e1, ws, st);
     default:
       PM_REQUIRE(pm_is_f32(dy), PM_EUNSUPPORTED, "conv_bwd_data: a bf16 dy needs at least 32 channels and a stride-1 geometry the forward form covers");
-      return conv_direct<MODE_DGRAD>(dx, dy, w, p, r.pl, e1, ws, st, add_mask);
+      return conv_direct<MODE_DGRAD>(dx, dy, w, p, r.pl, e1, ws, st, add_mask, packed_arg(p, r));
   }
 }
 
diff --git a/pinthememory_amd/csrc/conv_igemm_kernel.h b/pinthememory_amd/csrc/conv_igemm_kernel.h
--- a/pinthememory_amd/csrc/conv_igemm_kernel.h
+++ b/pinthememory_amd/csrc/conv_igemm_kernel.h
@@ -3,6 +3,7 @@
 #include <type_traits>
 
 #include "pm_common.h"
+#include "split_planes.h"
 
 typedef float f32x16 __attribute__((ext_vector_type(16)));
 typedef __bf16 bf16x8 __attribute__((ext_vector_type(8)));
@@ -40,6 +41,7 @@
   int n_group;
   int batch_xcd;
   int spl_prio;
+  const void* Bp;
 };
 
 int pm_conv_split_launch(int mode, int bm, int bn, const ConvK& k, unsigned gx, unsigned gy, unsigned gz, size_t smem, hipStream_t st);
@@ -58,6 +60,11 @@
 __device__ __forceinline__ float4 bload(__amdgpu_buffer_rsrc_t r, int off) {
   const v4f v = __builtin_bit_cast(v4f, __builtin_amdgcn_raw_buffer_load_b128(r, off, 0, 0));
   return make_float4(v.x, v.y, v.z, v.w);
+}
+__device__ __forceinline__ float2 bload8(__amdgpu_buffer_rsrc_t r, int off) {
+  typedef float v2f __attribute__((ext_vector_type(2)));
+  const v2f v = __builtin_bit_cast(v2f, __builtin_amdgcn_raw_buffer_load_b64(r, off, 0, 0));
+  return make_float2(v.x, v.y);
 }
 
 __device__ __forceinline__ int xcd_remap(int bid, int nwg) {
@@ -68,7 +75,7 @@
 
 enum { K_FAST = 0, K_MID = 1, K_SMALL = 2, K_PW = 3 };
 
-template <int MODE, int BM, int BN, int WM, int WN, int KM, int PREC, int NST, bool STATS = false>
+template <int MODE, int BM, int BN, int WM, int WN, int KM, int PREC, int NST, bool STATS = false, bool PACKB = false>
 __global__ __launch_bounds__(256, 2) void conv_igemm_kernel(const ConvK a) {
   constexpr bool A_KC = (MODE != MODE_WGRAD);
   constexpr bool B_KC = (MODE == MODE_FWD);
@@ -80,6 +87,9 @@
   constexpr bool SPL = (PREC == 5);
   constexpr int LD5 = 52;
   constexpr int KX = NAT16 ? 2 : 1, BKW = BK * KX;
+  static_assert(!PACKB || (SPL && FAST && NST == 1), "a packed B operand: the split path's forward / data-gradient forms on a wave-uniform K-state");
+  constexpr int BSZ = PACKB ? 6 : 4;
+  constexpr int BOOB = PACKB ? 0x7fffffe0 : OOB;
   static_assert(!TR || MODE == MODE_WGRAD, "PREC 3 / 4 are the weight-gradient forms");
   constexpr int LDA_T = BM + 32, LDB_T = BN + 32;
   constexpr int PLANE_A = BK * LDA_T / 2, PLANE_B = BK * LDB_T / 2;
@@ -132,7 +142,9 @@
   const int Treal = a.kh * a.kw;
 
   const __amdgpu_buffer_rsrc_t rA = __builtin_amdgcn_make_buffer_rsrc(const_cast<float*>(a.A + by * a.a_bs), 0, (int)a.a_bytes, 0x00020000);
-  const __amdgpu_buffer_rsrc_t rB = __builtin_amdgcn_make_buffer_rsrc(const_cast<float*>(a.B + by * a.b_bs), 0, (int)a.b_bytes, 0x00020000);
+  const __amdgpu_buffer_rsrc_t rB =
+      PACKB ? __builtin_amdgcn_make_buffer_rsrc(const_cast<char*>(static_cast<const char*>(a.Bp)) + by * a.b_bs * BSZ, 0, (int)(a.b_bytes + (a.b_bytes >> 1)), 0x00020000)
+            : __builtin_amdgcn_make_buffer_rsrc(const_cast<float*>(a.B + by * a.b_bs), 0, (int)a.b_bytes, 0x00020000);
   const int xp4 = (int)a.x_pitch * (NAT16 ? 2 : 4), yp4 = (int)a.y_pitch * (NAT16 ? 2 : 4);
   constexpr int A_NL = NAT16 ? (A_N + 1) / 2 : A_N, B_NL = NAT16 ? (B_N + 1) / 2 : B_N;
   constexpr int EPL = NAT16 ? 8 : 4;
@@ -201,13 +213,13 @@
 #pragma unroll
     for (int i = 0; i < B_N; ++i) {
       const int row = n0 + r + 32 * i;
-      b_base[i] = row < a.Cout ? row * a.K * 4 + g * 16 : OOB;
+      b_base[i] = row < a.Cout ? row * a.K * BSZ + g * 4 * BSZ : BOOB;
     }
   } else if constexpr (MODE == MODE_DGRAD) {
 #pragma unroll
     for (int j = 0; j < B_N; ++j) {
       const int col = n0 + (g + 8 * j) * 4;
-      b_base[j] = col < a.Cin ? col * 4 + (FAST ? r * Treal * a.Cin * 4 : 0) : OOB;
+      b_base[j] = col < a.Cin ? col * BSZ + (FAST ? r * Treal * a.Cin * BSZ : 0) : BOOB;
     }
     if constexpr (!FAST) {
       const int k = k_begin + r;
@@ -239,6 +251,15 @@
   }
 
   float4 ra[A_N], rb[B_N];
+  float2 sa[SPL ? A_N : 1][3], sb[SPL ? B_N : 1][3];
+  auto load_b = [&](int i, int off) {
+    if constexpr (PACKB) {
+      const float4 v = bload(rB, off);
+      sb[i][0] = make_float2(v.x, v.y), sb[i][1] = make_float2(v.z, v.w), sb[i][2] = bload8(rB, off + 16);
+    } else {
+      rb[i] = bload(rB, off);
+    }
+  };
 
   auto load_tiles = [&](int kt, int which = 0) {
     const int kbase = k_begin + kt * BKW;
@@ -247,21 +268,21 @@
       const unsigned beyond = 0x80000000u;
       const bool tok = u_tap < T;
       if constexpr (MODE == MODE_FWD) {
-        const unsigned toff = (unsigned)(u_ch * 4) + (tok ? 0u : beyond), kb4 = kbase < k_end ? (unsigned)(kbase * 4) : beyond;
+        const unsigned toff = (unsigned)(u_ch * 4) + (tok ? 0u : beyond), kb4 = kbase < k_end ? (unsigned)(kbase * BSZ) : beyond;
         if (doA)
 #pragma unroll
         for (int i = 0; i < A_N; ++i) ra[i] = bload(rA, (int)((unsigned)a_base[i] + toff));
         if (doB)
 #pragma unroll
-        for (int i = 0; i < B_N; ++i) rb[i] = bload(rB, (int)((unsigned)b_base[i] + kb4));
+        for (int i = 0; i < B_N; ++i) load_b(i, (int)((unsigned)b_base[i] + kb4));
       } else {
-        const unsigned toff = (unsigned)(u_ch * 4) + (tok ? 0u : beyond), uoff = tok ? (unsigned)((u_ch * Treal + u_tap) * a.Cin * 4) : beyond;
+        const unsigned toff = (unsigned)(u_ch * 4) + (tok ? 0u : beyond), uoff = tok ? (unsigned)((u_ch * Treal + u_tap) * a.Cin * BSZ) : beyond;
         if (doA)
 #pragma unroll
         for (int i = 0; i < A_N; ++i) ra[i] = bload(rA, (int)((unsigned)a_base[i] + toff));
         if (doB)
 #pragma unroll
-        for (int j = 0; j < B_N; ++j) rb[j] = bload(rB, (int)((unsigned)b_base[j] + uoff));
+        for (int j = 0; j < B_N; ++j) load_b(j, (int)((unsigned)b_base[j] + uoff));
       }
     } else if constexpr (MODE == MODE_FWD) {
       const int ky = FAST ? u_ky : a_ky, kx = FAST ? u_kx : a_kx, tap = FAST ? u_tap : a_tap, ch = FAST ? u_ch : a_ch;
@@ -279,8 +300,8 @@
       if (doB)
 #pragma unroll
       for (int i = 0; i < B_N; ++i) {
-        const int off = b_base[i] + kbase * 4;
-        rb[i] = bload(rB, (kok & (b_base[i] != OOB)) ? off : OOB);
+        const int off = b_base[i] + kbase * BSZ;
+        load_b(i, (kok & (b_base[i] != BOOB)) ? off : BOOB);
       }
     } else if constexpr (MODE == MODE_DGRAD) {
       if constexpr (FAST) {
@@ -294,12 +315,12 @@
           const int off = a_base[i] - toff;
           ra[i] = bload(rA, ok ? off : OOB);
         }
-        const int uoff = (u_ch * Treal + u_tap) * a.Cin * 4;
+        const int uoff = (u_ch * Treal + u_tap) * a.Cin * BSZ;
         if (doB)
 #pragma unroll
         for (int j = 0; j < B_N; ++j) {
           const int off = b_base[j] + uoff;
-          rb[j] = bload(rB, (tok & (b_base[j] != OOB)) ? off : OOB);
+          load_b(j, (tok & (b_base[j] != BOOB)) ? off : BOOB);
         }
       } else {
         const int dy = (a.ky0 + a.ksy * a_ky) * a.dil, dx = (a.kx0 + a.ksx * a_kx) * a.dil, smask = a.stride - 1;
@@ -412,19 +433,7 @@
     o[0] = (__bf16)v.x, o[1] = (__bf16)v.y, o[2] = (__bf16)v.z, o[3] = (__bf16)v.w;
     return __builtin_bit_cast(float2, o);
   };
-  auto split4 = [](const float4& v, float2& h, float2& m, float2& l) {
-    const unsigned u0 = __float_as_uint(v.x), u1 = __float_as_uint(v.y), u2 = __float_as_uint(v.z), u3 = __float_as_uint(v.w);
-    h.x = __uint_as_float(__builtin_amdgcn_perm(u1, u0, 0x07060302)), h.y = __uint_as_float(__builtin_amdgcn_perm(u3, u2, 0x07060302));
-    const float r0 = v.x - __uint_as_float(u0 & 0xffff0000u), r1 = v.y - __uint_as_float(u1 & 0xffff0000u);
-    const float r2 = v.z - __uint_as_float(u2 & 0xffff0000u), r3 = v.w - __uint_as_float(u3 & 0xffff0000u);
-    const unsigned q0 = __float_as_uint(r0), q1 = __float_as_uint(r1), q2 = __float_as_uint(r2), q3 = __float_as_uint(r3);
-    m.x = __uint_as_float(__builtin_amdgcn_perm(q1, q0, 0x07060302)), m.y = __uint_as_float(__builtin_amdgcn_perm(q3, q2, 0x07060302));
-    const float s0 = r0 - __uint_as_float(q0 & 0xffff0000u), s1 = r1 - __uint_as_float(q1 & 0xffff0000u);
-    const float s2 = r2 - __uint_as_float(q2 & 0xffff0000u), s3 = r3 - __uint_as_float(q3 & 0xffff0000u);
-    l.x = __uint_as_float(__builtin_amdgcn_perm(__float_as_uint(s1), __float_as_uint(s0), 0x07060302));
-    l.y = __uint_as_float(__builtin_amdgcn_perm(__float_as_uint(s3), __float_as_uint(s2), 0x07060302));
-  };
-  float2 sa[SPL ? A_N : 1][3], sb[SPL ? B_N : 1][3];
+  auto split4 = [](const float4& v, float2& h, float2& m, float2& l) { pm_split4(v, h, m, l); };
   auto split_a = [&]() {
     if constexpr (SPL) {
 #pragma unroll
@@ -432,7 +441,7 @@
     }
   };
   auto split_b = [&]() {
-    if constexpr (SPL) {
+    if constexpr (SPL && !PACKB) {
 #pragma unroll
       for (int i = 0; i < B_N; ++i) split4(rb[i], sb[i][0], sb[i][1], sb[i][2]);
     }
@@ -679,8 +688,10 @@
         }
         __builtin_amdgcn_sched_barrier(0);
         compute_kg(0, 2);
-        split_b();
-        load_tiles(kt + 2, 2);
+        if constexpr (!PACKB) {
+          split_b();
+          load_tiles(kt + 2, 2);
+        }
         __builtin_amdgcn_sched_group_barrier(0x100, NDS, 0);
 #pragma unroll
         for (int q = 0; q < NMF; ++q) {
@@ -690,6 +701,7 @@
         __builtin_amdgcn_sched_barrier(0);
         __syncthreads();
         write_planes(0);
+        if constexpr (PACKB) load_tiles(kt + 2, 2);
         __syncthreads();
         advance();
       }
diff --git a/pinthememory_amd/csrc/conv_split.hip b/pinthememory_amd/csrc/conv_split.hip
--- a/pinthememory_amd/csrc/conv_split.hip
+++ b/pinthememory_amd/csrc/conv_split.hip
@@ -5,21 +5,30 @@
 
 namespace {
 
+template <int MODE, int BM, int BN, int KM, bool ST, bool PK>
+void launch_inst(const ConvK& k, dim3 grid, size_t bytes, hipStream_t st) {
+  static pm_lds_optin optin;
+  (void)optin(reinterpret_cast<const void*>(&conv_igemm_kernel<MODE, BM, BN, 2, 2, KM, 5, 1, ST, PK>), 160 * 1024);
+  hipLaunchKernelGGL((conv_igemm_kernel<MODE, BM, BN, 2, 2, KM, 5, 1, ST, PK>), grid, dim3(256), bytes, st, k);
+}
+
 template <int MODE, int BM, int BN, int KM>
 void launch_split(const ConvK& k, dim3 grid, size_t smem, hipStream_t st) {
   const size_t ep_bytes = (size_t)4 * 32 * (BN / 2 + 4) * sizeof(float);
   const size_t bytes = std::max(smem, ep_bytes);
-  if constexpr (MODE == MODE_FWD) {
-    if (k.stats) {
-      static pm_lds_optin optin;
-      (void)optin(reinterpret_cast<const void*>(&conv_igemm_kernel<MODE, BM, BN, 2, 2, KM, 5, 1, true>), 160 * 1024);
-      hipLaunchKernelGGL((conv_igemm_kernel<MODE, BM, BN, 2, 2, KM, 5, 1, true>), grid, dim3(256), bytes, st, k);
-      return;
+  const bool stats = MODE == MODE_FWD && k.stats;
+  if constexpr (MODE != MODE_WGRAD && (KM == K_FAST || KM == K_PW)) {
+    if (k.Bp) {
+      if constexpr (MODE == MODE_FWD) {
+        if (stats) return launch_inst<MODE, BM, BN, KM, true, true>(k, grid, bytes, st);
+      }
+      return launch_inst<MODE, BM, BN, KM, false, true>(k, grid, bytes, st);
     }
   }
-  static pm_lds_optin optin;
-  (void)optin(reinterpret_cast<const void*>(&conv_igemm_kernel<MODE, BM, BN, 2, 2, KM, 5, 1>), 160 * 1024);
-  hipLaunchKernelGGL((conv_igemm_kernel<MODE, BM, BN, 2, 2, KM, 5, 1>), grid, dim3(256), bytes, st, k);
+  if constexpr (MODE == MODE_FWD) {
+    if (stats) return launch_inst<MODE, BM, BN, KM, true, false>(k, grid, bytes, st);
+  }
+  launch_inst<MODE, BM, BN, KM, false, false>(k, grid, bytes, st);
 }
 
 template <int MODE, int BM, int BN>
@@ -45,6 +54,34 @@
   return PM_OK;
 }
 
+constexpr int SP_BATCH = 96;
+constexpr int SP_GROUPS = 1024;
+struct SplitPackJobs {
+  const float* src[SP_BATCH];
+  char* dst[SP_BATCH];
+  long groups[SP_BATCH];
+  int start[SP_BATCH + 1];
+  int n;
+};
+__global__ __launch_bounds__(256) void split_pack_multi_kernel(const SplitPackJobs t) {
+  int j = 0;
+  while (j + 1 < t.n && (int)blockIdx.x >= t.start[j + 1]) ++j;
+  const long g0 = (long)((int)blockIdx.x - t.start[j]) * SP_GROUPS + threadIdx.x;
+  const float* src = t.src[j];
+  char* dst = t.dst[j];
+  const long ng = t.groups[j];
+#pragma unroll
+  for (int i = 0; i < SP_GROUPS / 256; ++i) {
+    const long gi = g0 + i * 256;
+    if (gi < ng) {
+      float2 h, m, l;
+      pm_split4(*reinterpret_cast<const float4*>(src + gi * 4), h, m, l);
+      float2* d = reinterpret_cast<float2*>(dst + gi * PM_SPLIT_GROUP_BYTES);
+      d[0] = h, d[1] = m, d[2] = l;
+    }
+  }
+}
+
 }
 
 size_t pm_conv_split_stage_bytes(int mode, int bm, int bn) {
@@ -60,3 +97,28 @@
   if (mode == MODE_DGRAD) return launch_tile<MODE_DGRAD>(bm, bn, k, grid, smem, st);
   return launch_tile<MODE_WGRAD>(bm, bn, k, grid, smem, st);
 }
+
+extern "C" int pm_split_pack_multi(const pm_split_job* jobs, int n, void* stream) {
+  PM_REQUIRE(n >= 0 && (jobs || n == 0), PM_EINVAL, "split_pack_multi: bad job table");
+  for (int i = 0; i < n; ++i) {
+    PM_REQUIRE(jobs[i].src && jobs[i].dst && jobs[i].count >= 0 && jobs[i].count % 4 == 0, PM_EINVAL, "split_pack_multi: job %d: null buffer or a float count (%ld) that is no multiple of 4",
+               i, (long)jobs[i].count);
+    PM_REQUIRE(pm_aligned16(jobs[i].src) && pm_aligned16(jobs[i].dst), PM_EINVAL, "split_pack_multi: job %d: buffers must be 16-byte aligned", i);
+  }
+  for (int i0 = 0; i0 < n; i0 += SP_BATCH) {
+    SplitPackJobs t{};
+    t.n = std::min(SP_BATCH, n - i0);
+    long blocks = 0;
+    for (int i = 0; i < t.n; ++i) {
+      t.src[i] = jobs[i0 + i].src, t.dst[i] = static_cast<char*>(jobs[i0 + i].dst), t.groups[i] = jobs[i0 + i].count / 4;
+      t.start[i] = (int)blocks;
+      blocks += (t.groups[i] + SP_GROUPS - 1) / SP_GROUPS;
+    }
+    t.start[t.n] = (int)blocks;
+    PM_REQUIRE(blocks < (1l << 31), PM_EUNSUPPORTED, "split_pack_multi: job table too large for one grid");
+    if (blocks == 0) continue;
+    hipLaunchKernelGGL(split_pack_multi_kernel, dim3((unsigned)blocks), dim3(256), 0, (hipStream_t)stream, t);
+    if (int e = pm_check_launch("split_pack_multi")) return e;
+  }
+  return PM_OK;
+}
diff --git a/pinthememory_amd/csrc/split_planes.h b/pinthememory_amd/csrc/split_planes.h
--- /dev/null
+++ b/pinthememory_amd/csrc/split_planes.h
@@ -0,0 +1,17 @@
+#pragma once
+#include <hip/hip_runtime.h>
+
+__device__ __forceinline__ void pm_split4(const float4& v, float2& h, float2& m, float2& l) {
+  const unsigned u0 = __float_as_uint(v.x), u1 = __float_as_uint(v.y), u2 = __float_as_uint(v.z), u3 = __float_as_uint(v.w);
+  h.x = __uint_as_float(__builtin_amdgcn_perm(u1, u0, 0x07060302)), h.y = __uint_as_float(__builtin_amdgcn_perm(u3, u2, 0x07060302));
+  const float r0 = v.x - __uint_as_float(u0 & 0xffff0000u), r1 = v.y - __uint_as_float(u1 & 0xffff0000u);
+  const float r2 = v.z - __uint_as_float(u2 & 0xffff0000u), r3 = v.w - __uint_as_float(u3 & 0xffff0000u);
+  const unsigned q0 = __float_as_uint(r0), q1 = __float_as_uint(r1), q2 = __float_as_uint(r2), q3 = __float_as_uint(r3);
+  m.x = __uint_as_float(__builtin_amdgcn_perm(q1, q0, 0x07060302)), m.y = __uint_as_float(__builtin_amdgcn_perm(q3, q2, 0x07060302));
+  const float s0 = r0 - __uint_as_float(q0 & 0xffff0000u), s1 = r1 - __uint_as_float(q1 & 0xffff0000u);
+  const float s2 = r2 - __uint_as_float(q2 & 0xffff0000u), s3 = r3 - __uint_as_float(q3 & 0xffff0000u);
+  l.x = __uint_as_float(__builtin_amdgcn_perm(__float_as_uint(s1), __float_as_uint(s0), 0x07060302));
+  l.y = __uint_as_float(__builtin_amdgcn_perm(__float_as_uint(s3), __float_as_uint(s2), 0x07060302));
+}
+
+constexpr int PM_SPLIT_GROUP_BYTES = 24;
diff --git a/pinthememory_amd/hip/kernels.py b/pinthememory_amd/hip/kernels.py
--- a/pinthememory_amd/hip/kernels.py
+++ b/pinthememory_amd/hip/kernels.py
@@ -88,7 +88,8 @@
     ptrs = None if params is None else {p.data_ptr() for p in params}
     for k in [k for k in _U_OWNERS if ptrs is None or k in ptrs]:
         del _U_OWNERS[k]
-    _U_CACHE.drop_if(lambda ent: ptrs is None or ent.ptr in ptrs)
+    for cache in (_U_CACHE, _P_CACHE):
+        cache.drop_if(lambda ent: ptrs is None or ent.ptr in ptrs)
 
 
 def _filter_owner(w_krsc):
@@ -102,7 +103,7 @@
 
 
 class _KeptFilter:
-    __slots__ = ('ptr', 'shape', 'nbytes', 'device', 'prec', 'dgrad', 'owner', 'version', 'buf', 'event', 'stream', 'used')
+    __slots__ = ('ptr', 'shape', 'nbytes', 'device', 'prec', 'dgrad', 'owner', 'version', 'buf', 'event', 'stream', 'used', 'src')
 
 
 class _FilterCache(dict):
@@ -131,7 +132,7 @@
     def clear(self):
         self.drop_if(lambda ent: True)
 
-    def lookup(self, p, w_krsc, nbu, dgrad=False):
+    def lookup(self, p, w_krsc, nbu, dgrad=False, fields=('wxf', 'wxf_bytes', 'wxf_valid')):
         if KEEP_WINOGRAD_U is False or not nbu:
             return None
         registered = _filter_owner(w_krsc)
@@ -150,7 +151,7 @@
             ent = _KeptFilter()
             ent.ptr, ent.shape, ent.nbytes, ent.device, ent.prec, ent.dgrad = key
             ent.owner = (lambda: w_krsc) if registered is None else weakref.ref(registered)
-            ent.version, ent.buf, ent.event, ent.stream = -1, torch.empty(nbu // 4, dtype=torch.float32, device=w_krsc.device), None, None
+            ent.version, ent.buf, ent.event, ent.stream, ent.src = -1, torch.empty(nbu // 4, dtype=torch.float32, device=w_krsc.device), None, None, None
             self.nbytes += nbu
         else:
             del self[key]
@@ -160,7 +161,8 @@
         valid = ent.version == version
         if not valid:
             ent.version = -1
-        p.wxf, p.wxf_bytes, p.wxf_valid = ent.buf.data_ptr(), nbu, 1 if valid else 0
+        for f, v in zip(fields, (ent.buf.data_ptr(), nbu, 1 if valid else 0)):
+            setattr(p, f, v)
         raw, cur = self._stream()
         if valid and ent.event is not None and ent.stream != raw:
             cur.wait_event(ent.event)
@@ -178,12 +180,95 @@
 
 
 _U_CACHE = _FilterCache()
-clear_filters, forget_filter_events = _U_CACHE.clear, _U_CACHE.forget_events
+
+WSPLIT = os.environ.get('PM_WSPLIT', '1') == '1'
+_P_CACHE = _FilterCache()
+_WSPLIT_FIELDS = ('wsplit', 'wsplit_bytes', 'wsplit_valid')
+
+
+def clear_filters():
+    _U_CACHE.clear()
+    _P_CACHE.clear()
+
+
+def forget_filter_events():
+    _U_CACHE.forget_events()
+    _P_CACHE.forget_events()
+
+
+def split_pack(srcs, dsts=None):
+    one = torch.is_tensor(srcs)
+    srcs = [srcs] if one else list(srcs)
+    for t in srcs:
+        assert t.dtype == torch.float32 and t.is_contiguous() and t.numel() % 4 == 0, 'split_pack: contiguous fp32 tensors of a multiple of four elements'
+    if dsts is None:
+        dsts = [torch.empty(t.numel() * 6, dtype=torch.uint8, device=t.device) for t in srcs]
+    _split_pack_raw([(t.data_ptr(), d.data_ptr(), t.numel()) for t, d in zip(srcs, dsts)])
+    return dsts[0] if one else dsts
+
+
+def _split_pack_raw(table):
+    jobs = (L.PmSplitJob * len(table))()
+    for j, (src, dst, count) in zip(jobs, table):
+        j.src, j.dst, j.count = src, dst, count
+    check(_lib().pm_split_pack_multi(jobs, len(table), stream()), 'pm_split_pack_multi')
+
+
+def _packed_lookup(p, w_krsc, nbp, from_wxf, nbu):
+    if not WSPLIT or not nbp or _filter_owner(w_krsc) is None:
+        return None
+    src = None
+    if from_wxf:
+        src = _U_CACHE.get((w_krsc.data_ptr(), tuple(w_krsc.shape), nbu, w_krsc.device.index, p.prec, False))
+        if src is None or not p.wxf or p.wxf != src.buf.data_ptr():
+            return None
+    pend = _P_CACHE.lookup(p, w_krsc, nbp, dgrad=bool(from_wxf), fields=_WSPLIT_FIELDS)
+    if pend is None:
+        return None
+    ent, version = pend
+    ent.src = src
+    return (ent, version, src.buf.data_ptr(), nbu // 4) if from_wxf else (ent, version, w_krsc.data_ptr(), w_krsc.numel())
+
+
+def _pack_behind(pend):
+    ent, version, src, count = pend
+    _split_pack_raw([(src, ent.buf.data_ptr(), count)])
+    _P_CACHE.commit((ent, version))
 
 _REFRESH = {2: ('pm_conv_wxf_refresh_bf16', False), 0: ('pm_conv_wxf_refresh_f32', True)}
 
 
 def refresh_filters():
+    n = _refresh_transforms()
+    _refresh_packed()
+    return n
+
+
+def _refresh_packed():
+    if not WSPLIT or KEEP_WINOGRAD_U is False or not _P_CACHE or CONV_PREC != 0:
+        return
+    dev = torch.cuda.current_device()
+    todo = []
+    for ent in _P_CACHE.values():
+        if ent.prec != CONV_PREC or ent.device != dev or not ent.used:
+            continue
+        ent.used = False
+        owner = ent.owner()
+        if owner is None or owner.data_ptr() != ent.ptr or ent.version == owner._version or not ent.buf.is_cuda:
+            continue
+        src = ent.src
+        if src is not None and (src.version != owner._version or _U_CACHE.get((ent.ptr, ent.shape, src.nbytes, ent.device, ent.prec, False)) is not src):
+            continue
+        todo.append((ent, owner._version))
+    if not todo:
+        return
+    for ent, _ in todo:
+        ent.version = -1
+    _split_pack_raw([(ent.ptr, ent.buf.data_ptr(), ent.nbytes // 6) if ent.src is None else (ent.src.buf.data_ptr(), ent.buf.data_ptr(), ent.src.nbytes // 4) for ent, _ in todo])
+    _P_CACHE.commit(*todo)
+
+
+def _refresh_transforms():
     if KEEP_WINOGRAD_U is False or not _U_CACHE or CONV_PREC not in _REFRESH:
         return 0
     entry_point, forward_3x3_only = _REFRESH[CONV_PREC]
@@ -225,6 +310,11 @@
     return v
 
 
+def _wsplit_query(fn, ad, bd, p):
+    from_wxf = ctypes.c_int32(0)
+    return fn(byref(ad), byref(bd), byref(p), byref(from_wxf)), from_wxf.value
+
+
 _XFORM_COUNT = [0, False]
 
 
@@ -244,9 +334,10 @@
     xd, yd = tdesc(x), tdesc(y)
     p = L.conv_params(kh, kw, stride, pad, dil, CONV_PREC)
     lib = _lib()
-    nbv, nbu, nb, npb = _sizes(('f', x.shape, x.stride(), x.dtype, xd.flags, w_krsc.shape, y.stride(), y.dtype, stride, pad, dil, CONV_PREC, _GEN[0]),
+    nbv, nbu, nb, npb, nbp = _sizes(('f', x.shape, x.stride(), x.dtype, xd.flags, w_krsc.shape, y.stride(), y.dtype, stride, pad, dil, CONV_PREC, _GEN[0]),
                                lambda: (lib.pm_conv_winograd_v_bytes(byref(xd), byref(yd), byref(p)), lib.pm_conv_wxf_bytes(byref(xd), byref(yd), byref(p)),
-                                        lib.pm_conv_workspace(byref(xd), byref(yd), byref(p), 0), lib.pm_conv_bn_partials_bytes(byref(xd), byref(yd), byref(p))))
+                                        lib.pm_conv_workspace(byref(xd), byref(yd), byref(p), 0), lib.pm_conv_bn_partials_bytes(byref(xd), byref(yd), byref(p)),
+                                        _wsplit_query(lib.pm_conv_wsplit_bytes, xd, yd, p)))
     if keep_v is not None:
         nbv = nbv if KEEP_WINOGRAD_V else 0
         v = torch.empty(nbv // 4, dtype=torch.float32, device=x.device) if nbv else None
@@ -258,6 +349,7 @@
         u_ent = _U_CACHE.lookup(p, w_krsc, nbu)
     if _XFORM_COUNT[1] and p.wxf_valid == 0 and nbu:
         _XFORM_COUNT[0] += 1
+    p_pend = _packed_lookup(p, w_krsc, nbp[0], nbp[1], nbu) if CONV_PREC == 0 else None
     ws = workspace(nb, x.device) if nb else None
     part = None
     if bn_partials is not None:
@@ -274,6 +366,8 @@
     check(lib.pm_conv_fwd(byref(xd), w_krsc.data_ptr(), byref(yd), byref(p), byref(ep) if ep else None, ptr(ws), nb, stream()), 'pm_conv_fwd')
     if u_ent is not None:
         _U_CACHE.commit(u_ent)
+    if p_pend is not None:
+        _pack_behind(p_pend)
     return y
 
 
@@ -283,17 +377,21 @@
     dyd, dxd = tdesc(dy), tdesc(dx)
     p = L.conv_params(kh, kw, stride, pad, dil, CONV_PREC)
     lib = _lib()
-    nb, nbu = _sizes(('d', dy.shape, dy.stride(), dy.dtype, dyd.flags, w_krsc.shape, dx.shape, dx.stride(), dx.dtype, stride, pad, dil, CONV_PREC, _GEN[0]),
-                     lambda: (lib.pm_conv_workspace(byref(dxd), byref(dyd), byref(p), 1), lib.pm_conv_wxf_bytes_dgrad(byref(dyd), byref(dxd), byref(p))))
+    nb, nbu, nbp = _sizes(('d', dy.shape, dy.stride(), dy.dtype, dyd.flags, w_krsc.shape, dx.shape, dx.stride(), dx.dtype, stride, pad, dil, CONV_PREC, _GEN[0]),
+                     lambda: (lib.pm_conv_workspace(byref(dxd), byref(dyd), byref(p), 1), lib.pm_conv_wxf_bytes_dgrad(byref(dyd), byref(dxd), byref(p)),
+                              _wsplit_query(lib.pm_conv_wsplit_bytes_dgrad, dyd, dxd, p)))
     ws = workspace(nb, dy.device) if nb else None
     ad = tdesc(add) if add is not None else None
     u_ent = _U_CACHE.lookup(p, w_krsc, nbu, dgrad=True) if CONV_PREC == 2 else None
+    p_pend = _packed_lookup(p, w_krsc, nbp[0], nbp[1], nbu) if CONV_PREC == 0 else None
     if add_mask is not None:
         check(lib.pm_conv_bwd_data_masked(byref(dyd), w_krsc.data_ptr(), byref(dxd), byref(p), byref(ad), add_mask.data_ptr(), ptr(ws), nb, stream()), 'pm_conv_bwd_data_masked')
     else:
         check(lib.pm_conv_bwd_data(byref(dyd), w_krsc.data_ptr(), byref(dxd), byref(p), byref(ad) if ad else None, ptr(ws), nb, stream()), 'pm_conv_bwd_data')
     if u_ent is not None:
         _U_CACHE.commit(u_ent)
+    if p_pend is not None:
+        _pack_behind(p_pend)
     return dx
 
 
diff --git a/pinthememory_amd/hip/lib.py b/pinthememory_amd/hip/lib.py
--- a/pinthememory_amd/hip/lib.py
+++ b/pinthememory_amd/hip/lib.py
@@ -28,7 +28,12 @@
 class PmConvParams(ctypes.Structure):
     _fields_ = [('struct_size', c_int32), ('kh', c_int32), ('kw', c_int32), ('stride', c_int32), ('pad', c_int32), ('dil', c_int32), ('prec', c_int32),
                 ('wino_v', c_void_p), ('wino_v_bytes', c_int64),
-                ('wxf', c_void_p), ('wxf_bytes', c_int64), ('wxf_valid', c_int32)]
+                ('wxf', c_void_p), ('wxf_bytes', c_int64), ('wxf_valid', c_int32),
+                ('wsplit', c_void_p), ('wsplit_bytes', c_int64), ('wsplit_valid', c_int32)]
+
+
+class PmSplitJob(ctypes.Structure):
+    _fields_ = [('src', c_void_p), ('dst', c_void_p), ('count', c_int64)]
 
 
 class PmRouting(ctypes.Structure):
@@ -49,7 +54,7 @@
     return PmConvEpilogue(ctypes.sizeof(PmConvEpilogue), *fields)
 
 
-ABI_VERSION = 400
+ABI_VERSION = 410
 
 
 class PinmemError(RuntimeError):
@@ -67,6 +72,9 @@
     'pm_conv_wxf_bytes_dgrad': (_sz, [_T, _T, _P]),
     'pm_conv_wxf_refresh_bf16': (_i, [_vp, _i, _vp]),
     'pm_conv_wxf_refresh_f32': (_i, [_vp, _i, _vp]),
+    'pm_split_pack_multi': (_i, [_vp, _i, _vp]),
+    'pm_conv_wsplit_bytes': (_sz, [_T, _T, _P, POINTER(c_int32)]),
+    'pm_conv_wsplit_bytes_dgrad': (_sz, [_T, _T, _P, POINTER(c_int32)]),
     'pm_conv_workspace': (_sz, [_T, _T, _P, _i]),
     'pm_conv_fwd': (_i, [_T, _vp, _T, _P, _E, _vp, _sz, _vp]),
     'pm_conv_bwd_data': (_i, [_T, _vp, _T, _P, _T, _vp, _sz, _vp]),
```

Result: slower. 152.8 (-1.3%).
